# ymxlzgy/commonscenes

Hardware: AMD Instinct MI355X
Metric: DDIM denoise steps/sec (32 objects, 16^3 latent) (higher is better)
Workload: dtype f32 (operands as fp16 hi+lo pairs, fp32 accumulate)

## Files before the change

commonscenes_amd/build.py:

```python
from __future__ import annotations

import os
import shutil
import subprocess
import sys
from pathlib import Path

PKG_DIR = Path(__file__).resolve().parent
CSRC = PKG_DIR / "csrc"
LIB_NAME = "libcommonscenes_hip.so"
LIB_PATH = PKG_DIR / LIB_NAME
SOURCES = ["cs_plan.hip", "cs_gemm.hip", "cs_gemm_f16x3.hip", "cs_gemm_kw.hip", "cs_mesh.hip", "cs_scene.hip", "cs_constraints.hip", "cs_metrics.hip", "cs_pairwise.hip", "cs_norm.hip", "cs_attention.hip", "cs_attention_f16x3.hip", "cs_ops.hip", "cs_unet.hip", "cs_vqvae.hip", "cs_vqenc.hip"]
HEADERS = [CSRC / "cs_common.h", CSRC / "cs_f16x3.h", CSRC / "cs_mc_tables.h", CSRC / "cs_driver.h", CSRC / "cs_vq.h", PKG_DIR.parent / "include" / "commonscenes_hip.h"]
ARCH = "gfx950"
FLAGS = ["-O3", "-std=c++17", "-fPIC", "-ffp-contract=off", f"--offload-arch={ARCH}", "-Wall",
         "-Wno-unused-function"]


def _hipcc() -> str:
    for cand in (os.environ.get("HIPCC"), shutil.which("hipcc"), "/opt/rocm/bin/hipcc"):
        if cand and Path(cand).exists():
            return cand
    raise RuntimeError("hipcc not found: cannot build libcommonscenes_hip.so")


def _flagstr() -> str:
    return " ".join([*FLAGS, *os.environ.get("CS_EXTRA_HIPCC_FLAGS", "").split()])


def _deps(src: Path, seen=None) -> set:
    import re
    seen = set() if seen is None else seen
    src = src.resolve()
    if src in seen or not src.exists():
        return seen
    seen.add(src)
    for m in re.finditer(r'^\s*#\s*include\s+"([^"]+)"', src.read_text(), re.M):
        _deps(src.parent / m.group(1), seen)
    return seen


def needs_build() -> bool:
    if not LIB_PATH.exists():
        return True
    stamp = PKG_DIR / "build" / "flags.txt"
    if stamp.exists() and stamp.read_text() != _flagstr():
        return True
    t = LIB_PATH.stat().st_mtime
    deps = [CSRC / s for s in SOURCES] + HEADERS
    return any(d.stat().st_mtime > t for d in deps)


def build_native(force: bool = False, verbose: bool = True) -> Path:
    if not force and not needs_build():
        return LIB_PATH
    hipcc = _hipcc()
    extra = os.environ.get("CS_EXTRA_HIPCC_FLAGS", "").split()
    objdir = PKG_DIR / "build"
    objdir.mkdir(exist_ok=True)
    import time
    t0 = time.time()
    procs = []
    objs = []
    stamp = objdir / "flags.txt"
    flagstr = _flagstr()
    same_flags = stamp.exists() and stamp.read_text() == flagstr
    for s in SOURCES:
        obj = objdir / (s.replace(".hip", ".o"))
        objs.append(str(obj))
        newest_dep = max(d.stat().st_mtime for d in _deps(CSRC / s))
        if not force and same_flags and obj.exists() and obj.stat().st_mtime > newest_dep:
            continue
        cmd = [hipcc, *FLAGS, *extra, "-c", str(CSRC / s), "-o", str(obj)]
        if verbose:
            print("[build]", " ".join(cmd), flush=True)
        procs.append((s, subprocess.Popen(cmd, stdout=subprocess.PIPE, stderr=subprocess.STDOUT)))
    for s, p in procs:
        out, _ = p.communicate()
        if p.returncode != 0:
            sys.stderr.write(out.decode())
            raise RuntimeError(f"hipcc failed on {s}")
        if verbose and out.strip():
            print(out.decode())
        os.utime(objdir / (s.replace(".hip", ".o")), (t0, t0))
    stamp.write_text(flagstr)
    tmp = LIB_PATH.with_suffix(".so.tmp")
    cmd = [hipcc, "-shared", "-fPIC", f"--offload-arch={ARCH}", *objs, "-o", str(tmp)]
    if verbose:
        print("[build]", " ".join(cmd), flush=True)
    subprocess.check_call(cmd)
    os.replace(tmp, LIB_PATH)
    os.utime(LIB_PATH, (t0, t0))
    return LIB_PATH


if __name__ == "__main__":
    print(build_native(force="--force" in sys.argv))
```

commonscenes_amd/csrc/cs_gemm.hip:

```cpp
#include <cstdlib>
#include <atomic>
#include <cstring>
#include "cs_f16x3.h"

namespace {

constexpr int BK = 16;

template <int WMB, int WNB, int WAVES_M, int WAVES_N>
__global__ __launch_bounds__(256) void conv_gemm_f32_kernel(const CsConvGemm p, int M,
                                                            int tiles_n, int taps_hw, int kw_) {
  constexpr int BM = 32 * WMB * WAVES_M;
  constexpr int BN = 32 * WNB * WAVES_N;
  constexpr int LDAS = BM + 4;
  constexpr int LDBS = BN + 4;
  constexpr int RPT = (BM + 63) / 64;
  constexpr int BUNITS = BK * BN / 4;
  constexpr int BPT = (BUNITS + 255) / 256;
  constexpr int A_SZ = BK * LDAS;
  constexpr int B_SZ = BK * LDBS;
  __shared__ __attribute__((aligned(16))) float smem[2 * A_SZ + 2 * B_SZ];
  float* As = smem;
  float* Bs = smem + 2 * A_SZ;

// ... 467 lines not shown
    }
    if (opair) {
      h4 hi, lo;
#pragma unroll
      for (int k = 0; k < 4; ++k) {
        const float o = v[k] * p.out_scale;
        oamax = fmaxf(oamax, fabsf(o));
        hi[k] = (_Float16)o;
        lo[k] = (_Float16)(o - (float)hi[k]);
      }
      const u32x2 H = __builtin_bit_cast(u32x2, hi), Lw = __builtin_bit_cast(u32x2, lo);
      const bool odd = cl & 1;
      const u32x2 send = odd ? H : Lw;
      u32x2 recv;
      recv[0] = (unsigned)__builtin_amdgcn_update_dpp(0, (int)send[0], 0xB1, 0xF, 0xF, true);
      recv[1] = (unsigned)__builtin_amdgcn_update_dpp(0, (int)send[1], 0xB1, 0xF, 0xF, true);
      u32x4 r;
      r[0] = odd ? recv[0] : H[0];
      r[1] = odd ? recv[1] : H[1];
      r[2] = odd ? Lw[0] : recv[0];
      r[3] = odd ? Lw[1] : recv[1];
      if (tok) {
        char* row = reinterpret_cast<char*>(p.out + m * p.ldo);
        *reinterpret_cast<u32x4*>(row + (n >> 4) * 64 + ((n & 8) ? 32 : 0) + ((n & 4) ? 16 : 0)) = r;
      }
    } else if (tok) {
      *reinterpret_cast<f32x4*>(p.out + m * p.ldo + n) = v;
    }
  }
  if (opair && p.status && oamax >= 65504.f) atomicOr(p.status, CS_STATUS_F16X3_OVERFLOW);
  if (gstat) {
    double tot[2][4];
#pragma unroll
    for (int which = 0; which < 2; ++which) {
      __syncthreads();
#pragma unroll
      for (int k = 0; k < 4; ++k) sc[tl][cl * 4 + k] = which ? sq[k] : s[k];
      __syncthreads();
      if (tl == 0) {
#pragma unroll
        for (int k = 0; k < 4; ++k) {
          double a = 0.0;
          for (int r2 = 0; r2 < 16; ++r2) a += sc[r2][cl * 4 + k];
          tot[which][k] = a;
        }
      }
    }
    if (tl == 0 && nok) {
      double* o = p.gn_part + ((int64_t)rb * p.gn_ld + n) * 2;
#pragma unroll
      for (int k = 0; k < 4; ++k) {
        o[2 * k] = tot[0][k];
        o[2 * k + 1] = tot[1][k];
      }
    }
  }
}

void tile_dims(int tile, int& bm, int& bn) {
  switch (tile) {
    case 1: bm = 128; bn = 128; break;
    case 2: bm = 128; bn = 224; break;
    case 3: bm = 64; bn = 64; break;
    case 4: bm = 256; bn = 224; break;
    case 6: bm = 256; bn = 128; break;
    case 7: bm = 256; bn = 64; break;
    case 10: bm = 64; bn = 64; break;
    default: bm = 0; bn = 0; break;
  }
}

}

static int auto_tile(const CsConvGemm& p, int M, bool f16x3);
static bool up2_direct_batched(const CsConvGemm& d, int64_t m1, int ncls);
static int up2_batched_tile(const CsConvGemm& d, int64_t m1, int ncls);

extern "C" int cs_conv_gemm_epilogue_caps(const CsConvGemm* d, int32_t* gn_rows, int32_t* pair_ok) {
  if (!d) return CS_EINVAL;
  if (gn_rows) *gn_rows = 0;
  if (pair_ok) *pair_ok = 0;
  const CsConvGemm& p = *d;
  if (p.math != CS_MATH_F16X3 || p.nb <= 0 || p.cout <= 0 || p.dout <= 0 || p.hout <= 0 || p.wout <= 0) return CS_OK;
  const int64_t M64 = (int64_t)p.nb * p.dout * p.hout * p.wout;
  if (M64 > 0x7fffffffLL) return CS_OK;
  const int M = (int)M64;
  auto al16 = [](const void* q) { return ((uintptr_t)q & 15) == 0; };
  const int ocols = p.act == CS_ACT_GEGLU ? p.cout / 2 : p.cout;
  const bool vec = (p.cout % 4 == 0) && (p.ldo % 4 == 0) && al16(p.out) && (!p.bias || al16(p.bias)) &&
                   (!p.scale || (al16(p.scale) && al16(p.shift))) && (!p.rowvec || (p.ldrv % 4 == 0 && al16(p.rowvec))) &&
                   (!p.res || (p.ldr % 4 == 0 && al16(p.res)));
  if (!vec) return CS_OK;
  const bool pair_geom = (ocols % 8 == 0) && (p.ldo % 16 == 0) && (((uintptr_t)p.out & 63) == 0);
  int64_t rps = (int64_t)p.dout * p.hout * p.wout;
  int bm = 0, bn = 0;
  if (p.ud | p.uh | p.uw) {
    const int64_t m1 = (int64_t)p.nb * p.din * p.hin * p.win;
    const int ncls = (p.ud ? 2 : 1) * (p.uh ? 2 : 1) * (p.uw ? 2 : 1);
    if (p.splitk > 1 || !up2_direct_batched(p, m1, ncls)) return CS_OK;
    CsConvGemm q = p;
    q.kd = p.ud ? 2 : 3; q.kh = p.uh ? 2 : 3; q.kw = p.uw ? 2 : 3;
    q.ud = q.uh = q.uw = 0;
    q.dout = p.din; q.hout = p.hin; q.wout = p.win;
    q.tile = 0;
    tile_dims(up2_batched_tile(p, m1, ncls), bm, bn);
    rps = (int64_t)p.din * p.hin * p.win;
    if (!bm || !p.bias) return CS_OK;
    if (p.scale) return CS_OK;
    const int64_t ospan = ((int64_t)bm + 2LL * p.hin * p.win + 2LL * p.win + 2) * ncls;
    if (ospan * p.ldo * 4 >= 0x7FF00000LL) return CS_OK;
    if (gn_rows && rps % bm == 0 && p.act != CS_ACT_GEGLU) *gn_rows = bm;
    return CS_OK;
  }
  if (p.a_format == 3 || p.a_format == 4) {
    const int wr = p.a_format == 4 ? 64 : 32;
    if (gn_rows && rps % wr == 0 && p.act != CS_ACT_GEGLU) *gn_rows = wr;
    if (pair_ok && pair_geom && p.act != CS_ACT_GEGLU) *pair_ok = 1;
    return CS_OK;
  }
  if (p.splitk > 1) {
    if (gn_rows && rps % SKR == 0 && p.act != CS_ACT_GEGLU) *gn_rows = SKR;
    if (pair_ok && pair_geom && p.act != CS_ACT_GEGLU) *pair_ok = 1;
    return CS_OK;
  }
  int tile = p.tile ? p.tile : auto_tile(p, M, true);
  if (tile == 5) return CS_OK;
  tile_dims(tile, bm, bn);
  if (!bm) return CS_OK;
  if (tile == 10) {
    if (!cs_kw_gemm_applicable(p, M)) return CS_OK;
    if (gn_rows && rps % bm == 0) *gn_rows = bm;
    if (pair_ok && pair_geom) *pair_ok = 1;
    return CS_OK;
  }
  const bool piped = (p.res || p.bias || p.rowvec) && !p.scale && (p.act != CS_ACT_GEGLU || p.cout % bn == 0) &&
                     (!p.rowvec || p.rv_rows % bm == 0) &&
                     (int64_t)bm * p.ldo * 4 < 0x7FF00000LL && (!p.res || (int64_t)bm * p.ldr * 4 < 0x7FF00000LL);
  if (!piped) return CS_OK;
  if (gn_rows && rps % bm == 0 && p.act != CS_ACT_GEGLU) *gn_rows = bm;
  if (pair_ok && pair_geom) *pair_ok = 1;
  return CS_OK;
}

extern "C" int cs_conv_gemm_plan(const CsConvGemm* d, int32_t* splitk, int64_t* ws_bytes) {
  if (!d || !splitk) return CS_EINVAL;
  const int64_t M = (int64_t)d->nb * d->dout * d->hout * d->wout;
  if (M <= 0 || d->cout <= 0) return CS_EINVAL;
  const int s = plan_splitk(*d, M);
  *splitk = s;
  if (ws_bytes) *ws_bytes = s > 1 ? (int64_t)s * M * d->cout * 4 : 0;
  return CS_OK;
}

static int64_t kwave_max_tiles() {
  static const int64_t v = [] {
    const char* e = getenv("CS_KWAVE_MAX_TILES");
    return (e && *e) ? atoll(e) : (long long)-1;
  }();
  return v >= 0 ? v : 4LL * device_cus();
}

static int tok_t2_maxk() {
  static const int v = [] {
    const char* e = getenv("CS_TOK_T2_MAXK");
    return (e && *e) ? atoi(e) : 128;
  }();
  return v;
}

static int auto_tile(const CsConvGemm& p, int M, bool f16x3) {
  int tile = 0;
  {
    const int64_t mt = (M + 127) / 128;
    if (f16x3 && p.cout % 224 == 0 && ((M + 255) / 256) * (int64_t)(p.cout / 224) >= 192)
      tile = 4;
    else if (f16x3 && p.cout % 128 == 0 && ((M + 255) / 256) * (int64_t)(p.cout / 128) >= 192)
      tile = 6;
    else if (f16x3 && p.cout <= 64 && (p.cout == 64 || p.cout <= 4) && (M + 255) / 256 >= 192)
      tile = 7;
    else if (p.cout % 224 == 0 && mt * (p.cout / 224) >= 256)
      tile = 2;
    else if (p.cout > 64 && mt * ((p.cout + 127) / 128) >= 256)
      tile = 1;
    else
      tile = 3;
    {
      const bool t512on = cs_debug()->tile512 != 0;
      const bool conv3 = p.kd == 3 && p.kh == 3 && p.kw == 3 && p.sd == 1 && p.sh == 1 && p.sw == 1 &&
                         !(p.ud | p.uh | p.uw) && p.pd == 1 && p.ph == 1 && p.pw == 1;
      const int64_t t512 = (M + 511) / 512;
      if (t512on && conv3 && tile == 7 && p.cout == 64 && p.win <= 64 && t512 >= 512) tile = 8;
      if (t512on && conv3 && tile == 6 && p.win <= 32 && t512 * (p.cout / 128) >= 512) tile = 9;
    }
    if (f16x3 && tile == 4 && p.kd * p.kh * p.kw == 1 && p.act != CS_ACT_GEGLU && !cs_debug()->no_tok_rules) {
      const int64_t t4 = ((M + 255) / 256) * (int64_t)(p.cout / 224);
      const int64_t rounds = (t4 + 255) / 256;
      if (t4 > 256 && rounds * 256 * 4 >= t4 * 5)
        tile = 1;
      else if (p.a_format == 2 && (p.cin + 15) / 16 <= 32)
        tile = 2;
      else if (t4 <= 256 && (p.cin + 15) / 16 <= 84)
        tile = 2;
      else if ((p.cin + 15) / 16 <= tok_t2_maxk())
        tile = 2;
    }
    if (p.act == CS_ACT_GEGLU) tile = 2;
    if (f16x3 && tile == 3 && !cs_debug()->no_kwave && (p.cin + 15) / 16 >= 8 && p.cout % 224 == 0 &&
        cs_kw_gemm_applicable(p, M) && (int64_t)((M + 63) / 64) * ((p.cout + 63) / 64) <= kwave_max_tiles())
      tile = 10;
  }
  return tile;
}

static int sliced_tile(const CsConvGemm& p, int M) {
  if (p.tile == 6 || p.tile == 7) return p.tile;
  const bool slab3 = !cs_debug()->slice_tile2 && p.kd == 3 && p.kh == 3 && p.kw == 3 && p.sd == 1 && p.sh == 1 &&
                     p.sw == 1 && p.pd == 1 && p.ph == 1 && p.pw == 1 && !(p.ud | p.uh | p.uw) && p.din == p.dout &&
                     p.hin == p.hout && p.win == p.wout && p.win <= 32;
  return (split4_large(p, M) || p.tile == 4 || slab3) ? 4 : 2;
}

static int device_cus() {
  static std::atomic<int> cached{-1};
  int v = cached.load(std::memory_order_relaxed);
  if (v >= 0) return v;
  int dev = 0, n = 0;
  if (hipGetDevice(&dev) != hipSuccess || hipDeviceGetAttribute(&n, hipDeviceAttributeMultiprocessorCount, dev) != hipSuccess)
    n = 0;
  (void)hipGetLastError();
  cached.store(n, std::memory_order_relaxed);
  return n;
}

static int fused_reduce_plan(const CsConvGemm& p, int M, int stile) {
  if (!p.splitk_sync || cs_debug()->no_fused_reduce || p.splitk < 2 || (stile != 2 && stile != 4)) return 0;
  if (p.cout % 224 || ((uintptr_t)p.splitk_sync & 3)) return 0;
  const int bm = stile == 4 ? 256 : 128;
  const int64_t tiles = (int64_t)((M + bm - 1) / bm) * (p.cout / 224);
  const int64_t slots = (int64_t)device_cus() * (stile == 4 ? 1 : 2);
  if (tiles * p.splitk > slots || 2 * tiles > p.splitk_sync_words) return 0;
  if ((int64_t)p.splitk * M * p.cout * 4 >= 0xFFE00000LL) return 0;
  int r = 1;
  while (2 * r <= p.splitk && 2 * r <= bm / 16) r *= 2;
  return r;
}

static int wino_tile(int cout) { return cout % 224 == 0 ? 4 : cout % 128 == 0 ? 6 : cout == 64 ? 7 : 0; }

static int wino_variant(const CsConvGemm& p);
static bool wino_ok(const CsConvGemm& p) { return wino_variant(p) != 0; }
static bool wino23_ok(const CsConvGemm& p) {
  const CsDebug* dbg = cs_debug();
  if (dbg->no_wino || p.math != CS_MATH_F16X3 || p.act == CS_ACT_GEGLU) return false;
  if (!(p.kd == 3 && p.kh == 3 && p.kw == 3 && p.sd == 1 && p.sh == 1 && p.sw == 1 && p.pd == 1 && p.ph == 1 && p.pw == 1) ||
      (p.ud | p.uh | p.uw) || p.din != p.dout || p.hin != p.hout || p.win != p.wout)
    return false;
  if ((p.win & 1) || p.win < 4 || p.win / 2 > 32 || !wino_tile(p.cout) || (p.cin & 7) || p.cin < 16) return false;
  if (p.cout % 224 && (int64_t)p.din * p.hin * p.win > 4096) return false;
  const int64_t M = (int64_t)p.nb * p.dout * p.hout * p.wout;
  const int64_t min_rows = dbg->wino_min_rows > 0 ? dbg->wino_min_rows : 1024;
  if (M < min_rows || M > 0x3fffffffLL || (M / 2) % 256) return false;
  if ((512 + 2LL * p.hin * (p.win / 2) + p.win + 32) * p.lda * 4 >= 0x7FF00000LL) return false;
  return true;
}
static int wino_variant(const CsConvGemm& p) {
  if (!wino23_ok(p)) return 0;
  const CsDebug* dbg = cs_debug();
  const int64_t M = (int64_t)p.nb * p.dout * p.hout * p.wout;
  const int64_t min43 = dbg->wino43_min_rows > 0 ? dbg->wino43_min_rows : 2048;
  const int64_t rdec = p.cout % 224 ? (int64_t)p.din * p.hin * p.win : M;
  if (!dbg->no_wino43 && p.win % 4 == 0 && (M / 4) % 256 == 0 && (rdec / 4) % 256 == 0 && rdec >= min43) return 4;
  return 2;
}
static inline int wino_pos(int variant) { return variant + 2; }

struct WinoPlan {
  int slices;
  int units_main;
};
static int wino_splits(const CsConvGemm& p, int variant, double* cost_us = nullptr);

static WinoPlan wino_plan(const CsConvGemm& p, int variant) {
  WinoPlan pl;
  double t_uni = 0;
  pl.slices = wino_splits(p, variant, &t_uni);
  pl.units_main = 0;
  static const bool forced = [] { const char* e = getenv("CS_WINO_SPLITS"); return e && *e && atoi(e) > 0; }();
  if (forced || cs_debug()->no_wino_tail || p.cout % 224) return pl;
  const int64_t M = (int64_t)p.nb * p.dout * p.hout * p.wout;
  const int64_t R = M / variant / 256, tiles_n = p.cout / 224;
  const int64_t units = wino_pos(variant) * tiles_n;
  const int64_t cus = device_cus() > 0 ? device_cus() : 256;
  if (R < 1) return pl;
  const int64_t rounds = units * R / cus;
  if (rounds < 1) return pl;
  const int64_t units_main = rounds * cus / R;
  const int64_t tail_tiles = (units - units_main) * R;
  if (units_main < 1 || tail_tiles < 1) return pl;
  const int64_t nsc = 3LL * ((p.cin + 15) / 16);
  int best = 0;
  for (int sp = 2; sp <= 16 && tail_tiles * sp <= cus; ++sp) {
    const int64_t per = (nsc + sp - 1) / sp;
    if (per < 2 || per * sp * 10 > nsc * 11 || (nsc + per - 1) / per != sp) continue;
    best = sp;
  }
  if (!best) return pl;
  const int64_t per = (nsc + best - 1) / best;
  const double mb_tail = (double)tail_tiles * 256.0 * 224.0 * 4.0 / 1e6;
  double seam = (best - 1) * mb_tail * 0.46;
  if (seam < 2.0 * (best - 1)) seam = 2.0 * (best - 1);
  const double main_rounds = (double)((units_main * R + cus - 1) / cus);
  const double t_tail = main_rounds * ((double)nsc * 3.0 * 0.95 + 10.0) + ((double)per * 3.0 * 0.95 + 10.0) + seam + 5.0;
  if (t_tail < t_uni * 0.97) {
    pl.slices = best;
    pl.units_main = (int)units_main;
  }
  return pl;
}

static int wino_splits(const CsConvGemm& p, int variant, double* cost_us) {
  if (cost_us) *cost_us = 0.0;
  if (p.cout % 224) return 1;
  static const int forced = [] {
    const char* e = getenv("CS_WINO_SPLITS");
    return (e && *e) ? atoi(e) : 0;
  }();
  const int64_t M = (int64_t)p.nb * p.dout * p.hout * p.wout;
  const int64_t tiles = wino_pos(variant) * (M / variant / 256) * (p.cout / 224);
  if (forced > 0) {
    const int64_t nsc0 = 3LL * ((p.cin + 15) / 16), per0 = (nsc0 + forced - 1) / forced;
    if (forced == 1 || (per0 >= 2 && per0 * forced * 10 <= nsc0 * 11 && (nsc0 + per0 - 1) / per0 == forced)) return forced;
  }
  const int64_t cus = device_cus() > 0 ? device_cus() : 256;
  const int64_t nsc = 3LL * ((p.cin + 15) / 16);
  const double mb = (double)wino_pos(variant) / variant * (double)M * p.cout * 4.0 / 1e6;
  int best = 1;
  double best_t = 0;
  for (int sp = 1; sp <= 16; ++sp) {
    const int64_t per = (nsc + sp - 1) / sp;
    if (sp > 1 && (per < 2 || per * sp * 10 > nsc * 11 || (nsc + per - 1) / per != sp)) continue;
    const int64_t rounds = (tiles * sp + cus - 1) / cus;
    double seam = (sp - 1) * mb * 0.46;
    if (sp > 1 && seam < 2.0 * (sp - 1)) seam = 2.0 * (sp - 1);
    const double t = (double)rounds * ((double)per * 3.0 * 0.95 + 10.0) + seam;
    if (sp == 1 || t < best_t * 0.97) {
      best = sp;
      best_t = t;
    }
  }
  if (cost_us) *cost_us = best_t;
  return best;
}

extern "C" int cs_conv_wino_ok(const CsConvGemm* d) { return (d && d->nb > 0 && d->cout > 0) ? wino_variant(*d) : 0; }

static int wino_asked(const CsConvGemm& p) {
  const int v = p.a_format == 4 ? 4 : 2;
  const int best = wino_variant(p);
  return (best == 0 || v > best) ? 0 : v;
}

extern "C" int cs_conv_wino_plan(const CsConvGemm* d, int32_t* splitk, int64_t* ws_bytes) {
  if (!d || !splitk) return CS_EINVAL;
  const int v = wino_asked(*d);
  if (!v) return CS_EINVAL;
  const int sp = wino_plan(*d, v).slices;
  *splitk = sp;
  const int64_t M = (int64_t)d->nb * d->dout * d->hout * d->wout;
  if (ws_bytes) *ws_bytes = (int64_t)sp * wino_pos(v) * (M / v) * d->cout * 4;
  return CS_OK;
}

extern "C" int cs_conv_wino_plan_info(const CsConvGemm* d, int32_t* slices, int32_t* units_main, int32_t* units) {
  if (!d) return CS_EINVAL;
  const int v = wino_asked(*d);
  if (!v) return CS_EINVAL;
  const WinoPlan pl = wino_plan(*d, v);
  if (slices) *slices = pl.slices;
  if (units_main) *units_main = pl.units_main;
  if (units) *units = (int32_t)(wino_pos(v) * ((d->cout + 223) / 224));
  return CS_OK;
}

static int conv_wino(const CsConvGemm& p, int M, hipStream_t s, int phases = 3) {
  auto al16 = [](const void* q) { return ((uintptr_t)q & 15) == 0; };
  const int v = wino_asked(p), np = wino_pos(v);
  if (!v || !p.x_lo || !al16(p.x_lo) || !p.w_lo || !al16(p.w_lo) || (p.lda & 7) || !p.splitk_ws || !al16(p.splitk_ws) ||
      p.a_bound || !(p.acc_scale > 0.f))
    return CS_EINVAL;
  if ((p.ldo & 3) || !al16(p.out) || (p.bias && !al16(p.bias)) || (p.scale && (!al16(p.scale) || !al16(p.shift))) ||
      (p.rowvec && ((p.ldrv & 3) || !al16(p.rowvec))) || (p.res && ((p.ldr & 3) || !al16(p.res))))
    return CS_EINVAL;
  const int sp = p.splitk > 1 ? p.splitk : 1;
  if (sp > 16) return CS_EINVAL;
  CsConvGemm q = p;
  q.nb = np * p.nb;
  q.win = q.wout = p.win / v;
  q.kw = 1;
  q.pw = 0;
  q.a_format = 1;
  q.out = reinterpret_cast<float*>(p.splitk_ws);
  q.ldo = p.cout;
  q.bias = q.scale = q.shift = q.rowvec = q.res = nullptr;
  q.act = CS_ACT_NONE;
  q.gn_part = nullptr;
  q.out_format = 0;
  q.splitk = 0;
  q.tile = wino_tile(p.cout);
  const WinoPlan pl = wino_plan(p, v);
  const bool tail = pl.units_main > 0 && pl.slices == sp;
  const int units = np * (p.cout / 224);
  if (phases & 1) {
    int rc;
    if (tail) {
      rc = cs_conv_gemm_f16x3_dispatch(q, np * (M / v), q.tile, 1, s, 16, np, nullptr, nullptr, nullptr, 0, nullptr, 0, pl.units_main);
      if (rc == CS_OK)
        rc = cs_conv_gemm_f16x3_dispatch(q, np * (M / v), q.tile, sp, s, 16, np, nullptr, nullptr, nullptr, 0, nullptr, pl.units_main,
                                         units - pl.units_main);
    } else {
      rc = cs_conv_gemm_f16x3_dispatch(q, np * (M / v), q.tile, sp, s, 16, np, nullptr, nullptr, nullptr, 0, nullptr);
    }
    if (rc != CS_OK) return rc;
  }
  if (!(phases & 2)) return CS_OK;
  const int tail_unit0 = tail ? pl.units_main : 0x7fffffff;
  const int sp_main = tail ? 1 : sp;
  const int64_t nblk = (int64_t)((M / v + 15) / 16) * ((p.cout + 63) / 64);
  if (nblk > 0x7fffffffLL || (p.gn_part && p.gn_rows != 16 * v)) return CS_EINVAL;
  if (v == 4) {
    CS_LAUNCH(wino_out_kernel<4>, dim3((unsigned)nblk), dim3(256), 0, s, p, reinterpret_cast<const float*>(p.splitk_ws), M, sp_main,
              tail_unit0, sp, 224);
  } else {
    CS_LAUNCH(wino_out_kernel<2>, dim3((unsigned)nblk), dim3(256), 0, s, p, reinterpret_cast<const float*>(p.splitk_ws), M, sp_main,
              tail_unit0, sp, 224);
  }
// ... 537 lines not shown
```

commonscenes_amd/csrc/cs_norm.hip:

```cpp
#include <cstdlib>

#include "cs_common.h"

namespace {

constexpr int GN_MIN_SPLIT_ROWS = 16;
constexpr int GN_MAX_SPLITS = 256;
constexpr int64_t GN_SMALL_BYTES = 16 << 20;
constexpr int64_t GN_SMALL_GROUP = 11264;

__global__ __launch_bounds__(256) void gn_partial_kernel(const float* __restrict__ x, int rows, int c,
                                                         int ldx, int groups, int nsplit, int rps,
                                                         double* __restrict__ partial) {
  extern __shared__ __attribute__((aligned(16))) double sm[];
  const int n = blockIdx.x / nsplit;
  const int split = blockIdx.x % nsplit;
  const int ch4 = c >> 2;
  const int tpr = ch4 < 256 ? ch4 : 256;
  const int rowlanes = 256 / tpr;
  const int tid = threadIdx.x;
  const int rl = tid / tpr;
  const int cl = tid - rl * tpr;
  const int r0 = split * rps;
  const int r1 = min(rows, r0 + rps);
  const float* xb = x + (int64_t)n * rows * ldx;
  if (rl < rowlanes) {
    for (int c4 = cl; c4 < ch4; c4 += tpr) {
      double s0 = 0, s1 = 0, s2 = 0, s3 = 0, q0 = 0, q1 = 0, q2 = 0, q3 = 0;
      for (int r = r0 + rl; r < r1; r += 4 * rowlanes) {
        float4 v[4];
#pragma unroll
        for (int u = 0; u < 4; ++u) {
          const int rr = r + u * rowlanes;
          v[u] = rr < r1 ? *reinterpret_cast<const float4*>(xb + (int64_t)rr * ldx + c4 * 4)
                         : make_float4(0.f, 0.f, 0.f, 0.f);
        }
#pragma unroll
        for (int u = 0; u < 4; ++u) {
          if (r + u * rowlanes < r1) {
            s0 += v[u].x; q0 += (double)v[u].x * v[u].x;
            s1 += v[u].y; q1 += (double)v[u].y * v[u].y;
            s2 += v[u].z; q2 += (double)v[u].z * v[u].z;
            s3 += v[u].w; q3 += (double)v[u].w * v[u].w;
          }
        }
      }
      double* d = sm + ((int64_t)rl * c + c4 * 4) * 2;
      d[0] = s0; d[1] = q0; d[2] = s1; d[3] = q1; d[4] = s2; d[5] = q2; d[6] = s3; d[7] = q3;
    }
  }
  __syncthreads();
  if (tid < groups) {
    const int cpg = c / groups;
    double s = 0, q = 0;
    for (int l = 0; l < rowlanes; ++l)
      for (int k = 0; k < cpg; ++k) {
        const double* d = sm + ((int64_t)l * c + tid * cpg + k) * 2;
        s += d[0];
        q += d[1];
      }
    double* o = partial + (((int64_t)n * nsplit + split) * groups + tid) * 2;
    o[0] = s;
    o[1] = q;
  }
}

__device__ __forceinline__ void gn_bound_max(float* bound, double mean, double var, double count);

__global__ __launch_bounds__(256) void gn_finalize_kernel(const double* __restrict__ partial, int nsplit, int groups,
                                                          double count, float eps, float* __restrict__ stats,
                                                          int total, float* __restrict__ bound = nullptr) {
  const int lane = threadIdx.x & 63;
  const int i = blockIdx.x * 4 + (threadIdx.x >> 6);
  if (i >= total) return;
  const int n = i / groups, g = i - n * groups;
  double s = 0, q = 0;
  for (int k = lane; k < nsplit; k += 64) {
    const double* d = partial + (((int64_t)n * nsplit + k) * groups + g) * 2;
    s += d[0];
    q += d[1];
  }
#pragma unroll
  for (int o = 32; o > 0; o >>= 1) {
    s += __shfl_xor(s, o, 64);
    q += __shfl_xor(q, o, 64);
  }
  if (lane == 0) {
    const double mean = s / count;
    double var = q / count - mean * mean;
    if (var < 0) var = 0;
    stats[2 * i] = (float)mean;
    stats[2 * i + 1] = (float)(1.0 / sqrt(var + (double)eps));
    if (bound) gn_bound_max(bound, mean, var, count);
  }
}

struct GnSegs {
  CsGnSeg s[4];
  int n;
};
__device__ __forceinline__ void gn_group_parts(const GnSegs& sg, int n, int g, int cpg, int lane, int nlanes, double& s,
                                               double& q) {
  s = 0;
  q = 0;
  const int c_lo = g * cpg, c_hi = c_lo + cpg;
#pragma unroll
  for (int si = 0; si < 4; ++si) {
    if (si >= sg.n) break;
    const CsGnSeg& sp = sg.s[si];
    const int lo = max(c_lo, sp.ch0), hi = min(c_hi, sp.ch0 + sp.nch);
    if (hi <= lo) continue;
    const int tps = sp.tiles_per_sample, nt = sp.ncls * tps, items = (hi - lo) * nt;
    const int64_t cls_stride = (int64_t)sp.nb_src * tps;
    const int64_t t0 = (int64_t)(n % sp.nb_src) * tps;
    for (int j = lane; j < items; j += 4 * nlanes) {
      double2 v[4];
#pragma unroll
      for (int u = 0; u < 4; ++u) {
        const int ju = j + u * nlanes;
        v[u] = make_double2(0.0, 0.0);
        if (ju < items) {
          const int k = ju / nt, r = ju - k * nt;
          const int cls = r / tps, t = r - cls * tps;
          v[u] = *reinterpret_cast<const double2*>(sp.part +
                                                   ((cls * cls_stride + t0 + t) * sp.ld + sp.col0 + (lo + k - sp.ch0)) * 2);
        }
      }
#pragma unroll
      for (int u = 0; u < 4; ++u)
        if (j + u * nlanes < items) {
          s += v[u].x;
          q += v[u].y;
        }
    }
  }
}

__device__ __forceinline__ float gn_bound_value(double mean, double var, double count) {
  const double b = fabs(mean) + sqrt(var * (count > 1.0 ? count - 1.0 : 1.0));
  float bf = (float)b;
  if ((double)bf < b) bf = __uint_as_float(__float_as_uint(bf) + 1u);
  return (bf == bf && bf > 0.f) ? bf : 0.f;
}
__device__ __forceinline__ void gn_bound_commit(float* bound, float bf) {
  if (bf > 0.f) atomicMax(reinterpret_cast<unsigned int*>(bound), __float_as_uint(bf));
}
__device__ __forceinline__ void gn_bound_max(float* bound, double mean, double var, double count) {
  gn_bound_commit(bound, gn_bound_value(mean, var, count));
}

constexpr int GN_FIN_WAVES = 16;
template <int WPG>
__global__ __launch_bounds__(64 * GN_FIN_WAVES) void gn_finalize_parts_kernel(const GnSegs sg, int groups, int cpg,
                                                                              double count, float eps,
                                                                              float* __restrict__ stats,
// ... 261 lines not shown
  const int tid = threadIdx.x;
  const int ll = tid / tpr;
  const int cl = tid - ll * tpr;
  if (ll >= linelanes) return;
  const int n = blockIdx.y;
  const int l0 = blockIdx.x * lines_per_block;
  const int l1 = min(lines, l0 + lines_per_block);
  const int w4n = w >> 2;
  const float* xb = x + (int64_t)n * lines * w * ldx;
  const int64_t vrow0 = (int64_t)n * lines * w4n;
  const float* st = stats + (int64_t)n * groups * 2;
  float amax = 0.f;
  for (int cv = cl; cv < chv; cv += tpr) {
    float gg[V], bb[V], mean[V], rstd[V];
#pragma unroll
    for (int k4 = 0; k4 < V / 4; ++k4) {
      const float4 g = *reinterpret_cast<const float4*>(gamma + cv * V + 4 * k4);
      const float4 b = *reinterpret_cast<const float4*>(beta + cv * V + 4 * k4);
      gg[4 * k4] = g.x; gg[4 * k4 + 1] = g.y; gg[4 * k4 + 2] = g.z; gg[4 * k4 + 3] = g.w;
      bb[4 * k4] = b.x; bb[4 * k4 + 1] = b.y; bb[4 * k4 + 2] = b.z; bb[4 * k4 + 3] = b.w;
    }
#pragma unroll
    for (int k = 0; k < V; ++k) {
      const int grp = (ch0 + cv * V + k) / cpg;
      mean[k] = st[grp * 2];
      rstd[k] = st[grp * 2 + 1];
    }
    auto actv = [&](const float* px, bool in, float (&o)[V]) {
      if (!in) {
#pragma unroll
        for (int k = 0; k < V; ++k) o[k] = 0.f;
        return;
      }
#pragma unroll
      for (int k4 = 0; k4 < V / 4; ++k4) {
        const float4 v = *reinterpret_cast<const float4*>(px + 4 * k4);
        const float iv[4] = {v.x, v.y, v.z, v.w};
#pragma unroll
        for (int k = 0; k < 4; ++k)
          o[4 * k4 + k] = cs_act((iv[k] - mean[4 * k4 + k]) * rstd[4 * k4 + k] * gg[4 * k4 + k] + bb[4 * k4 + k], act) * a_scale;
      }
    };
    for (int line = l0 + ll; line < l1; line += linelanes) {
      const float* xl = xb + (int64_t)line * w * ldx + cv * V;
      float d[6][V];
#pragma unroll
      for (int k = 0; k < V; ++k) d[0][k] = 0.f;
      actv(xl, true, d[1]);
      for (int t = 0; t < w4n; ++t) {
#pragma unroll
        for (int j = 2; j < 6; ++j) {
          const int wi = 4 * t - 1 + j;
          actv(xl + (int64_t)wi * ldx, wi < w, d[j]);
        }
        const int64_t off = (vrow0 + (int64_t)line * w4n + t) * ldv + cv * V;
#pragma unroll
        for (int q = 0; q < 6; ++q) {
          hv hi, lo;
#pragma unroll
          for (int k = 0; k < V; ++k) {
            float o;
            if (q == 0) o = 4.f * d[0][k] - 5.f * d[2][k] + d[4][k];
            else if (q == 1) o = (d[4][k] + d[3][k]) - 4.f * (d[1][k] + d[2][k]);
            else if (q == 2) o = 4.f * (d[1][k] - d[2][k]) + (d[4][k] - d[3][k]);
            else if (q == 3) o = 2.f * (d[3][k] - d[1][k]) + (d[4][k] - d[2][k]);
            else if (q == 4) o = 2.f * (d[1][k] - d[3][k]) + (d[4][k] - d[2][k]);
            else o = 4.f * d[1][k] - 5.f * d[3][k] + d[5][k];
            amax = fmaxf(amax, fabsf(o));
            const _Float16 hh = (_Float16)o;
            hi[k] = hh;
            lo[k] = (_Float16)(o - (float)hh);
          }
          *reinterpret_cast<hv*>(vh + q * pos_stride + off) = hi;
          *reinterpret_cast<hv*>(vl + q * pos_stride + off) = lo;
        }
#pragma unroll
        for (int k = 0; k < V; ++k) {
          d[0][k] = d[4][k];
          d[1][k] = d[5][k];
        }
      }
    }
  }
  if (status && amax >= 65504.f) atomicOr(status, CS_STATUS_F16X3_OVERFLOW);
}

template <int MAXV>
__global__ __launch_bounds__(256) void ln_kernel(const float* __restrict__ x,
                                                 const float* __restrict__ gamma,
                                                 const float* __restrict__ beta,
                                                 float* __restrict__ y, int m, int c, int ldx,
                                                 int ldy, float eps) {
  const int lane = threadIdx.x & 63;
  const int wave = threadIdx.x >> 6;
  const int ch4 = c >> 2;
  for (int64_t row = (int64_t)blockIdx.x * 4 + wave; row < m; row += (int64_t)gridDim.x * 4) {
    float4 v[MAXV];
    float s = 0.f;
#pragma unroll
    for (int k = 0; k < MAXV; ++k) {
      const int c4 = lane + 64 * k;
      v[k] = make_float4(0.f, 0.f, 0.f, 0.f);
      if (c4 < ch4) v[k] = *reinterpret_cast<const float4*>(x + row * ldx + c4 * 4);
      s += (v[k].x + v[k].y) + (v[k].z + v[k].w);
    }
    const float mean = wave_sum(s) / (float)c;
    float q = 0.f;
#pragma unroll
    for (int k = 0; k < MAXV; ++k) {
      const int c4 = lane + 64 * k;
      if (c4 < ch4) {
        const float a = v[k].x - mean, b = v[k].y - mean, cc = v[k].z - mean, d = v[k].w - mean;
        q += (a * a + b * b) + (cc * cc + d * d);
      }
    }
    const float var = wave_sum(q) / (float)c;
    const float rstd = 1.0f / sqrtf(var + eps);
#pragma unroll
    for (int k = 0; k < MAXV; ++k) {
      const int c4 = lane + 64 * k;
      if (c4 < ch4) {
        const float4 g = *reinterpret_cast<const float4*>(gamma + c4 * 4);
        const float4 b = *reinterpret_cast<const float4*>(beta + c4 * 4);
        float4 o;
        o.x = (v[k].x - mean) * rstd * g.x + b.x;
        o.y = (v[k].y - mean) * rstd * g.y + b.y;
        o.z = (v[k].z - mean) * rstd * g.z + b.z;
        o.w = (v[k].w - mean) * rstd * g.w + b.w;
        *reinterpret_cast<float4*>(y + row * ldy + c4 * 4) = o;
      }
    }
  }
}

template <int MAXV>
__global__ __launch_bounds__(256) void ln_pair_kernel(const float* __restrict__ x, const float* __restrict__ gamma,
                                                      const float* __restrict__ beta, _Float16* __restrict__ y, int m,
                                                      int c, int ldx, int ldy, float eps, float a_scale,
                                                      int32_t* __restrict__ status) {
  const int lane = threadIdx.x & 63;
  const int wave = threadIdx.x >> 6;
  const int ch4 = c >> 2;
  float amax = 0.f;
  for (int64_t row = (int64_t)blockIdx.x * 4 + wave; row < m; row += (int64_t)gridDim.x * 4) {
    float4 v[MAXV];
    float s = 0.f;
#pragma unroll
    for (int k = 0; k < MAXV; ++k) {
      const int c4 = lane + 64 * k;
      v[k] = make_float4(0.f, 0.f, 0.f, 0.f);
      if (c4 < ch4) v[k] = *reinterpret_cast<const float4*>(x + row * ldx + c4 * 4);
      s += (v[k].x + v[k].y) + (v[k].z + v[k].w);
    }
    const float mean = wave_sum(s) / (float)c;
    float q = 0.f;
#pragma unroll
    for (int k = 0; k < MAXV; ++k) {
      const int c4 = lane + 64 * k;
      if (c4 < ch4) {
        const float a = v[k].x - mean, b = v[k].y - mean, cc = v[k].z - mean, d = v[k].w - mean;
        q += (a * a + b * b) + (cc * cc + d * d);
      }
    }
    const float var = wave_sum(q) / (float)c;
    const float rstd = 1.0f / sqrtf(var + eps);
#pragma unroll
    for (int k = 0; k < MAXV; ++k) {
      const int c4 = lane + 64 * k;
      if (c4 < ch4) {
        const float4 g = *reinterpret_cast<const float4*>(gamma + c4 * 4);
        const float4 b = *reinterpret_cast<const float4*>(beta + c4 * 4);
        const float o[4] = {((v[k].x - mean) * rstd * g.x + b.x) * a_scale, ((v[k].y - mean) * rstd * g.y + b.y) * a_scale,
                            ((v[k].z - mean) * rstd * g.z + b.z) * a_scale, ((v[k].w - mean) * rstd * g.w + b.w) * a_scale};
        h4v hi, lo;
#pragma unroll
        for (int e = 0; e < 4; ++e) {
          amax = fmaxf(amax, fabsf(o[e]));
          const _Float16 h = (_Float16)o[e];
          hi[e] = h;
          lo[e] = (_Float16)(o[e] - (float)h);
        }
        const int cch = c4 >> 2, j = (c4 & 3) * 4;
        _Float16* dst = y + row * (int64_t)ldy * 2 + cch * 32 + (j < 8 ? 0 : 16) + (j & 7);
        *reinterpret_cast<h4v*>(dst) = hi;
        *reinterpret_cast<h4v*>(dst + 8) = lo;
      }
    }
  }
  if (status && amax >= 65504.f) atomicOr(status, CS_STATUS_F16X3_OVERFLOW);
}

__global__ __launch_bounds__(256) void gn_small_kernel(const float* __restrict__ x, const float* __restrict__ gamma,
                                                       const float* __restrict__ beta, float* __restrict__ y,
                                                       float* __restrict__ stats, int rows, int c, int ldx, int ldy,
                                                       int groups, float eps, int act) {
  __shared__ double red[2][256];
  const int n = blockIdx.x / groups, g = blockIdx.x - n * groups;
  const int cpg = c / groups;
  const int tid = threadIdx.x;
  const float* xb = x + (int64_t)n * rows * ldx + g * cpg;
  float* yb = y + (int64_t)n * rows * ldy + g * cpg;
  const int dr = 256 / cpg, dk = 256 - dr * cpg;
  auto next = [&](int& r, int& k) {
    r += dr;
    k += dk;
    if (k >= cpg) {
      k -= cpg;
      ++r;
    }
  };
  double s = 0, q = 0;
  {
    int r = tid / cpg, k = tid - r * cpg;
    while (r < rows) {
      float v[4];
      int rr[4];
#pragma unroll
      for (int u = 0; u < 4; ++u) {
        rr[u] = r;
        v[u] = r < rows ? xb[(int64_t)r * ldx + k] : 0.f;
        next(r, k);
      }
#pragma unroll
      for (int u = 0; u < 4; ++u)
        if (rr[u] < rows) {
          s += v[u];
          q += (double)v[u] * v[u];
        }
    }
  }
  red[0][tid] = s;
  red[1][tid] = q;
  __syncthreads();
#pragma unroll
  for (int o = 128; o > 0; o >>= 1) {
    if (tid < o) {
      red[0][tid] += red[0][tid + o];
      red[1][tid] += red[1][tid + o];
    }
    __syncthreads();
  }
  const double count = (double)rows * cpg;
  const double mean_d = red[0][0] / count;
  double var = red[1][0] / count - mean_d * mean_d;
  if (var < 0) var = 0;
  const float mean = (float)mean_d;
  const float rstd = (float)(1.0 / sqrt(var + (double)eps));
  if (tid == 0 && stats) {
    stats[2 * blockIdx.x] = mean;
    stats[2 * blockIdx.x + 1] = rstd;
  }
  {
    int r = tid / cpg, k = tid - r * cpg;
    while (r < rows) {
      float v[4], ga[4], be[4];
      int rr[4], kk[4];
#pragma unroll
      for (int u = 0; u < 4; ++u) {
        rr[u] = r;
        kk[u] = k;
        if (r < rows) {
          v[u] = xb[(int64_t)r * ldx + k];
          ga[u] = gamma[g * cpg + k];
          be[u] = beta[g * cpg + k];
        }
        next(r, k);
      }
#pragma unroll
      for (int u = 0; u < 4; ++u)
        if (rr[u] < rows) yb[(int64_t)rr[u] * ldy + kk[u]] = cs_act((v[u] - mean) * rstd * ga[u] + be[u], act);
    }
  }
}

__global__ __launch_bounds__(256) void gn_small_parts_kernel(const float* __restrict__ x, const GnSegs sg,
                                                             const float* __restrict__ gamma,
                                                             const float* __restrict__ beta, float* __restrict__ y,
                                                             float* __restrict__ stats, float* __restrict__ bound, int rows,
                                                             int c, int ldx, int ldy, int groups, float eps, int act,
                                                             int rsplit) {
  __shared__ double red[2][256];
  const int sgi = blockIdx.x / rsplit, rs = blockIdx.x - sgi * rsplit;
  const int n = sgi / groups, g = sgi - n * groups;
  const int cpg = c / groups;
  const int tid = threadIdx.x;
  double s, q;
  gn_group_parts(sg, n, g, cpg, tid, 256, s, q);
  red[0][tid] = s;
  red[1][tid] = q;
  __syncthreads();
#pragma unroll
  for (int o = 128; o > 0; o >>= 1) {
    if (tid < o) {
      red[0][tid] += red[0][tid + o];
      red[1][tid] += red[1][tid + o];
    }
    __syncthreads();
  }
  const double count = (double)rows * cpg;
  const double mean_d = red[0][0] / count;
  double var = red[1][0] / count - mean_d * mean_d;
  if (var < 0) var = 0;
  const float mean = (float)mean_d;
  const float rstd = (float)(1.0 / sqrt(var + (double)eps));
  if (tid == 0 && stats && rs == 0) {
    stats[2 * sgi] = mean;
    stats[2 * sgi + 1] = rstd;
  }
  if (tid == 0 && bound && rs == 0) gn_bound_max(bound, mean_d, var, count);
  const int rper = (rows + rsplit - 1) / rsplit;
  const int rbeg = rs * rper, rend = min(rows, rbeg + rper);
  const float* xb = x + (int64_t)n * rows * ldx + g * cpg;
  float* yb = y + (int64_t)n * rows * ldy + g * cpg;
  const int dr = 256 / cpg, dk = 256 - dr * cpg;
  int r = rbeg + tid / cpg, k = tid - (tid / cpg) * cpg;
  rows = rend;
  while (r < rows) {
    float v[4], ga[4], be[4];
    int rr[4], kk[4];
#pragma unroll
    for (int u = 0; u < 4; ++u) {
      rr[u] = r;
      kk[u] = k;
      if (r < rows) {
        v[u] = xb[(int64_t)r * ldx + k];
        ga[u] = gamma[g * cpg + k];
        be[u] = beta[g * cpg + k];
      }
      r += dr;
      k += dk;
      if (k >= cpg) {
        k -= cpg;
        ++r;
      }
    }
#pragma unroll
    for (int u = 0; u < 4; ++u)
      if (rr[u] < rows) yb[(int64_t)rr[u] * ldy + kk[u]] = cs_act((v[u] - mean) * rstd * ga[u] + be[u], act);
  }
}
// ... 319 lines not shown
```

commonscenes_amd/csrc/cs_plan.hip:

```cpp
#include <cmath>
#include <cstdlib>
#include <cstring>
#include <mutex>

#include "cs_common.h"

namespace {

CsDebug g_dbg;
std::once_flag g_once;

bool flag(const char* name) {
  const char* e = getenv(name);
  return e && *e && !(e[0] == '0' && e[1] == 0);
}
long long num(const char* name, long long dflt) {
  const char* e = getenv(name);
  return (e && *e) ? atoll(e) : dflt;
}

void parse_env(CsDebug& d) {
  memset(&d, 0, sizeof(d));
  d.no_split16 = flag("CS_NO_SPLIT16");
  d.split16_min_rows = num("CS_SPLIT16_MIN_ROWS", 8192);
  d.no_pair16 = flag("CS_NO_PAIR16");
  d.no_upfold = flag("CS_NO_UPFOLD");
  d.no_splitk = flag("CS_NO_SPLITK");
  d.no_fused_geglu = flag("CS_NO_FUSED_GEGLU");
  d.no_tapcol = flag("CS_NO_TAPCOL");
  d.tapcol_tile = (int32_t)num("CS_TAPCOL_TILE", 0);
  d.no_cfg_split = flag("CS_NO_CFG_SPLIT");
  d.cfg_split_min_rows = num("CS_CFG_SPLIT_MIN_ROWS", 65536);
  d.concat_copy = flag("CS_CONCAT_COPY");
  d.gn_small_group = num("CS_GN_SMALL_GROUP", 11264);
  d.tile512 = flag("CS_TILE512");
  d.no_pw = flag("CS_NO_PW");
  d.no_slab4 = flag("CS_NO_SLAB4");
  d.no_attn_img = flag("CS_NO_ATTN_IMG");
  d.attn_nw8 = flag("CS_ATTN_NW8");
  d.no_up2_direct = flag("CS_NO_UP2_DIRECT");
  d.no_up2_batch = flag("CS_NO_UP2_BATCH");
  d.plan_pow2 = flag("CS_PLAN_POW2");
  d.slice_tile2 = flag("CS_SLICE_TILE2");
  d.no_gn_parts = flag("CS_NO_GN_PARTS");
  d.no_pair_epilogue = flag("CS_NO_PAIR_EPILOGUE");
  d.no_dyn_scale = flag("CS_NO_DYN_SCALE");
  d.no_tok_rules = flag("CS_NO_TOK_RULES");
  d.no_fused_reduce = flag("CS_NO_FUSED_REDUCE");
  d.no_gn_fold = flag("CS_NO_GN_FOLD");
  d.no_kwave = flag("CS_NO_KWAVE");
  d.no_static_scales = flag("CS_NO_STATIC_SCALES");
  d.no_wino = flag("CS_NO_WINO");
  d.wino_min_rows = (int32_t)num("CS_WINO_MIN_ROWS", 1024);
  d.no_wino43 = flag("CS_NO_WINO43");
  d.wino43_min_rows = (int32_t)num("CS_WINO43_MIN_ROWS", 2048);
  d.no_wino_tail = flag("CS_NO_WINO_TAIL");
}

}

extern "C" const CsDebug* cs_debug(void) {
  std::call_once(g_once, [] { parse_env(g_dbg); });
  return &g_dbg;
}

extern "C" void cs_debug_set(const CsDebug* d) {
  (void)cs_debug();
  if (d)
    g_dbg = *d;
  else
    parse_env(g_dbg);
}

extern "C" float cs_norm_a_scale(float gmax, float bmax, int64_t n) {
  const double bound = (double)gmax * std::sqrt((double)(n > 1 ? n - 1 : 1)) + (double)bmax;
  if (!(bound > 0.0) || !std::isfinite(bound)) return (float)std::ldexp(1.0, 40);
  int ex = 0;
  (void)std::frexp(65000.0 / bound, &ex);
  int k = ex - 1;
  if (k < -8) k = -8;
  if (k > 40) k = 40;
  return (float)std::ldexp(1.0, k);
}

extern "C" float cs_bound_a_scale(float bound) {
  if (!(bound > 0.f) || !std::isfinite(bound)) return (float)std::ldexp(1.0, 40);
  int ex = 0;
  (void)std::frexp(65000.0 / (double)bound, &ex);
  int k = ex - 1;
  if (k < -24) k = -24;
  if (k > 40) k = 40;
  return (float)std::ldexp(1.0, k);
}

extern "C" int cs_attnblock_static_scales(float gmax, float bmax, int64_t n, int c, float w_l2max, float b_absmax, float qk_scale,
                                          float* out4) {
  if (!out4 || n < 1 || c < 1 || !(qk_scale > 0.f) || !(gmax >= 0.f) || !(bmax >= 0.f) || !(w_l2max >= 0.f) || !(b_absmax >= 0.f))
    return CS_EINVAL;
  const double e = (double)gmax * std::sqrt((double)(n > 1 ? n - 1 : 1)) + (double)bmax;
  const double b = (double)w_l2max * std::sqrt((double)c) * e + (double)b_absmax;
  auto S = [](double v) { return cs_bound_a_scale(v < 3.0e38 ? (float)(v * (1.0 + 1e-6)) : 3.0e38f); };
  out4[0] = S(b * (double)qk_scale);
  out4[1] = S(b);
  out4[2] = S(b);
  out4[3] = S(b);
  return CS_OK;
}

extern "C" int cs_transformer_static_scales(const CsTransformerStats* st, int c, int64_t n_tokens, int heads, float gn_gmax,
                                            float gn_bmax, float ctx_max, float* out12) {
  if (!st || !out12 || c <= 0 || heads <= 0 || c % heads || n_tokens <= 0) return CS_EINVAL;
  const double rc = std::sqrt((double)c);
  const double dh = (double)(c / heads);
  const double y1 = (double)st->g1 * rc + (double)st->be1;
  const double bq = (double)st->rq * y1, bk = (double)st->rk * y1, bv = (double)st->rv * y1;
  const double ngrp = (double)n_tokens * (double)(c / 32 > 0 ? c / 32 : 1);
  const double egn = (double)gn_gmax * std::sqrt(ngrp > 1.0 ? ngrp - 1.0 : 1.0) + (double)gn_bmax;
  const double bt0 = (double)st->rpi * rc * egn + (double)st->bpi;
  const double bt1 = (double)st->ro * rc * bv + (double)st->bo + bt0 + (double)(ctx_max > 0.f ? ctx_max : 0.f);
  const double y3 = (double)st->g3 * rc + (double)st->be3;
  const double bgg = ((double)st->rx * y3 + (double)st->bx) * ((double)st->rg * y3 + (double)st->bg);
  const double bt2 = (double)st->r2 * std::sqrt(4.0 * c) * bgg + (double)st->b2 + bt1;
  auto S = [](double b) { return cs_bound_a_scale(b < 3.0e38 ? (float)(b * (1.0 + 1e-6)) : 3.0e38f); };
  out12[0] = S(bq / std::sqrt(dh));
  out12[1] = S(bk);
  out12[2] = S(bv);
  out12[3] = S(bv);
  out12[4] = S(bgg);
  out12[5] = S(bt2);
  out12[6] = (float)bq; out12[7] = (float)bk; out12[8] = (float)bv; out12[9] = (float)bt1; out12[10] = (float)bgg;
  out12[11] = (float)bt2;
  return CS_OK;
}

extern "C" int cs_conv_wants_split16(int64_t m, int cin, int cout, int k, int plain, int math) {
  const CsDebug* d = cs_debug();
  if (d->no_split16 || math != CS_MATH_F16X3 || !plain || k != 3 || (cin & 7)) return 0;
  const int64_t t256 = (m + 255) / 256;
  if (cout % 224 == 0) return t256 * (cout / 224) >= 192 || (d->split16_min_rows > 0 && m >= d->split16_min_rows);
  if (cout % 128 == 0) return t256 * (cout / 128) >= 192;
  return (cout == 64 || cout <= 4) && t256 >= 192;
}

extern "C" int cs_tapcol_tile(int64_t m, int ncolp) {
  const CsDebug* d = cs_debug();
  if (d->tapcol_tile) return d->tapcol_tile;
  if ((m + 255) / 256 < 192) return 0;
  return ncolp <= 64 ? 7 : 6;
}

extern "C" int cs_tapcol_ok(int cout, int cin, int k, int math) {
  return !cs_debug()->no_tapcol && math == CS_MATH_F16X3 && k == 3 && cout <= 4 && (cin & 3) == 0;
}
```

commonscenes_amd/csrc/cs_unet.hip:

```cpp
#include "cs_driver.h"

namespace {

enum Kind { CONV_IN, RES, ATTN, ATTNBLOCK, DOWN, UP };

struct Layer {
  Kind kind;
  int cin, cout;
  int g[8];
  int n[4];
  int emb_lo = 0;
  int ks = 0, ch_h = 0;
  int gsp[2] = {-1, -1};
  int ctx_off = 0;
  bool fused_geglu = false;
  int stat_slot = -1;
  CsTransformerStats ts;
  bool has_ts = false;
  float ctx_max = 0.f;
  int ab_w = -1, ab_b = -1;
  float ab_l2max = 0.f, ab_bmax = 0.f;
};

}
// ... 178 lines not shown
      ds *= 2;
    }
  }
  u.mid.push_back(make_res(u, P + "middle_block.0", ch, ch, ted, emb));
  u.mid.push_back(attn_layer(P + "middle_block.1", ch));
  u.mid.push_back(make_res(u, P + "middle_block.2", ch, ch, ted, emb));
  int oi = 0;
  for (int level = c.n_mult - 1; level >= 0; --level) {
    const int m = c.channel_mult[level];
    for (int i = 0; i <= nres; ++i) {
      const int ich = chans.back();
      chans.pop_back();
      const std::string bp = P + "output_blocks." + std::to_string(oi++);
      std::vector<Layer> layers;
      layers.push_back(make_res(u, bp + ".0", ch + ich, mc * m, ted, emb));
      ch = mc * m;
      if (in_list(c.attention_resolutions, c.n_attn_res, ds))
        layers.push_back(attn_layer(bp + ".1", ch));
      if (level && i == nres) {
        Layer l{};
        l.kind = UP;
        l.cin = l.cout = ch;
        l.g[0] = add_layer_gemm(u, bp + "." + std::to_string(layers.size()) + ".conv", ch, ch, 3, true, 0,
                                c.dims == 3 ? 3 : 7);
        layers.push_back(l);
        ds /= 2;
      }
      u.out.push_back(layers);
    }
  }
  if (c.use_spatial_transformer && !cs_debug()->no_cfg_split) {
    size_t n_prefix = 0;
    while (n_prefix < u.inp.size() && !has_attn(u.inp[n_prefix])) ++n_prefix;
    for (size_t j = 0; j < u.out.size(); ++j) {
      const size_t src = u.inp.size() - 1 - j;
      Layer& l = u.out[j][0];
      if (src >= n_prefix || l.kind != RES || l.g[2] < 0) continue;
      const int ch_s = u.inp[src].back().cout, C = l.cin, ch_h = C - ch_s, cpg = C / 32;
      if (C % 32) continue;
      int ks = 0;
      for (int k = (ch_h + 15) / 16 * 16; k < C; k += 16)
        if ((k / cpg) * cpg >= ch_h) {
          ks = k;
          break;
        }
      if (!ks || (C - ks) % 16) continue;
      const int gi = l.g[0];
      const int wp = u.gemms[gi].w[0].param, bp = u.gemms[gi].b.empty() ? -1 : u.gemms[gi].b[0].param;
      const int k = u.gemms[gi].k;
      l.gsp[0] = add_gemm_cin_range(u, wp, bp, l.cout, C, k, 0, ks);
      l.gsp[1] = add_gemm_cin_range(u, wp, -1, l.cout, C, k, ks, C);
      l.ks = ks;
      l.ch_h = ch_h;
    }
  }
  u.split_min_rows = cs_debug()->cfg_split_min_rows;
  u.ch_final = ch;
  u.n_out = add_norm(u, P + "out.0", ch);
  u.g_out = add_layer_gemm(u, P + "out.2", c.out_channels, mc, 3, true, 0, 0, true);
  u.g_emb_all = add_gemm(u, emb.w, emb.b, emb.total, ted, 0);
  u.emb_total = emb.total;

  int nblk = 0, nab = 0;
  for_each_layer(u, [&](const Layer& l) {
    nblk += l.kind == ATTN;
    nab += l.kind == ATTNBLOCK;
  });
  u.extra_slots = (c.math == CS_MATH_F16X3) ? 34 * nblk + 4 * nab : 0;
  layout_arena(u);
  if (u.extra_slots) {
    int k = 0, k2 = 0;
    for_each_layer(u, [&](Layer& l) {
      if (l.kind == ATTN) l.stat_slot = u.extra_slot0 + 34 * k++;
      if (l.kind == ATTNBLOCK) l.stat_slot = u.extra_slot0 + 34 * nblk + 4 * k2++;
    });
  }
  return CS_OK;
}

struct Exec : ExecBase {
  const cs_unet& u;
  Exec(const cs_unet& u_, const void* arena_, void* ws_, int64_t ws_bytes_, bool dry_, hipStream_t st_)
      : ExecBase(u_, arena_, ws_, ws_bytes_, dry_, st_), u(u_) {}
  int64_t in_bound_off = -1;

  Act res_block(const Layer& l, const Act& x, const Buf& semb) {
    const int rows = x.d * x.h * x.w;
    const bool own_skip = l.g[2] >= 0;
    int64_t xb = -1;
    Buf hn = groupnorm(x.b, l.n[0], x.nb, 1e-5f, CS_ACT_SILU, 32, l.g[0], own_skip ? &xb : nullptr, x.d, x.h, x.w);
    Buf h1 = gemm(hn, l.g[0], x.nb, x.d, x.h, x.w, GemmOpts().row_vector(at(semb, l.emb_lo), semb.c, rows).stats());
    release(hn);
    Buf hn2 = groupnorm(h1, l.n[1], x.nb, 1e-5f, CS_ACT_SILU, 32, l.g[1], nullptr, x.d, x.h, x.w);
    release(h1);
    Buf skip;
    if (own_skip) skip = gemm(x.b, l.g[2], x.nb, x.d, x.h, x.w, GemmOpts().bound(xb));
    Act o = x;
    const Buf& sk = own_skip ? skip : x.b;
    o.b = gemm(hn2, l.g[1], x.nb, x.d, x.h, x.w, GemmOpts().residual(sk, sk.c).stats());
    release(hn2);
    release(skip);
    return o;
  }

  Act res_block_split(const Layer& l, const Act& x, const Act& sk, const Buf& semb) {
    const int rows = x.d * x.h * x.w, C = x.b.c, ks = l.ks, cs = C - ks, off = ks - l.ch_h, cpg = C / 32;
    const int nb = x.nb, nbs = sk.nb, ch_s = sk.b.c, cout = l.cout;
    Act o = x;
    if (nbs <= 0 || nb % nbs || ch_s != C - l.ch_h) {
      chk(CS_EINVAL);
      return o;
    }
    const Norm& n0 = pl.norms[l.n[0]];
    GnStats s = gn_stats_alloc(x.b, nb, 32, true);
    gn_stats_run(x.b, nb, 1e-5f, 32, s);
    release(s.wsb);
    auto gn_range = [&](const float* xp, int ldx, int nbr, int64_t sample0, int ch0, int c, int conv_gi, int wn) {
      Buf y = gn_out(n0, (int64_t)nbr * rows, c, nbr, cpg, wn, conv_gi, (int64_t)nbs * rows);
      gn_emit(xp, ldx, at(s.stats, sample0 * 32 * 2), n0, y, nbr, rows, x.d, x.h, x.w, 32, cpg, ch0, CS_ACT_SILU);
      return y;
    };
    const int wn_h = wants_wino(l.gsp[0], nbs, x.d, x.h, x.w), wn_s = wants_wino(l.gsp[1], nbs, x.d, x.h, x.w);
    Buf a_h;
    if (!wn_h) a_h = gn_range(at(x.b), C, nb, 0, 0, ks, l.gsp[0], 0);
    Buf a_s = gn_range(at(sk.b, off), ch_s, nbs, 0, ks, cs, l.gsp[1], wn_s);
    Buf y_s = alloc(sk.b.rows, cout);
    if (ok()) gemm_view(view(a_s), l.gsp[1], nbs, x.d, x.h, x.w, at(y_s), cout);
    release(a_s);
    Buf h1 = alloc(x.b.rows, cout);
    for (int g = 0; g < nb / nbs && ok(); ++g) {
      const int64_t s0 = (int64_t)g * nbs, r0 = s0 * rows;
      GemmOpts opt;
      opt.row_vector(at(semb, s0 * semb.c + l.emb_lo), semb.c, rows).residual(y_s, cout);
      if (wn_h) {
        Buf a_g = gn_range(at(x.b, r0 * C), C, nbs, s0, 0, ks, l.gsp[0], wn_h);
        if (ok()) gemm_view(view(a_g), l.gsp[0], nbs, x.d, x.h, x.w, at(h1, r0 * cout), cout, opt);
        release(a_g);
      } else {
        gemm_view(view(a_h, r0), l.gsp[0], nbs, x.d, x.h, x.w, at(h1, r0 * cout), cout, opt);
      }
    }
    release(s.stats);
    release(a_h);
    release(y_s);
    Buf skc = gemm(x.b, l.g[2], nb, x.d, x.h, x.w, GemmOpts().bound(s.bound));
    Buf hn2 = groupnorm(h1, l.n[1], nb, 1e-5f, CS_ACT_SILU, 32, l.g[1], nullptr, x.d, x.h, x.w);
    release(h1);
    o.b = gemm(hn2, l.g[1], nb, x.d, x.h, x.w, GemmOpts().residual(skc, cout).stats());
    release(hn2);
    release(skc);
    return o;
  }

  Act attn_block(const Layer& l, const Act& x, const float* ctxvec) {
    const int c = l.cin, heads = u.cfg.num_heads, dh = c / heads;
    const int n = x.d * x.h * x.w;
    const int64_t rows = (int64_t)x.nb * n;
    Buf xn = groupnorm(x.b, l.n[0], x.nb, 1e-6f, CS_ACT_NONE);
    Buf t0 = linear(xn, l.g[0]);
    release(xn);
    Buf n1 = layernorm(t0, l.n[1]);
    Buf qkv = linear(n1, l.g[1]);
    release(n1);
    Buf a = alloc(rows, c);
    float ss[12];
    const Norm& gnn = pl.norms[l.n[0]];
    const bool stat = l.has_ts && u.cfg.math == CS_MATH_F16X3 && !cs_debug()->no_static_scales && ctxvec &&
                      cs_transformer_static_scales(&l.ts, c, n, heads, gnn.gmax, gnn.bmax, l.ctx_max, ss) == CS_OK;
    self_attention(qkv, a, x.nb, n, heads, dh, c, (float)std::pow((double)dh, -0.5), stat ? ss : nullptr);
    if (stat) a.a_scale = ss[3];
    release(qkv);
    Buf t1 = linear(a, l.g[2], GemmOpts().row_vector(ctxvec ? ctxvec + l.ctx_off : nullptr, u.ctx_total, n).residual(t0, c));
    release(a);
    release(t0);
    Buf n3 = layernorm(t1, l.n[3]);
    Buf gg;
    const float pairs = u.cfg.math == CS_MATH_F16X3 ? 16.f : 0.f;
    const float pair_gg = (pairs > 0.f && stat) ? ss[4] : pairs, pair_t2 = (pairs > 0.f && stat) ? ss[5] : pairs;
    if (l.fused_geglu) {
      gg = linear(n3, l.g[5], GemmOpts().activation(CS_ACT_GEGLU).pair(pair_gg));
    } else {
      Buf ff = linear(n3, l.g[5]);
      gg = alloc(rows, 4 * c);
      if (ok() && !dry) chk(cs_geglu(p(ff), p(gg), (int)rows, 4 * c, 8 * c, 4 * c, st));
      release(ff);
    }
    if (stat && !gg.pair) gg.a_scale = ss[4];
    release(n3);
    Buf t2 = linear(gg, l.g[6], GemmOpts().residual(t1, c).pair(pair_t2));
    if (stat && !t2.pair) t2.a_scale = ss[5];
    release(gg);
    release(t1);
    Act o = x;
    o.b = gemm(t2, l.g[7], x.nb, n, 1, 1, GemmOpts().residual(x.b, c).stats());
    release(t2);
    return o;
  }

  Act attnblock(const Layer& l, const Act& x) {
    const int c = l.cin, heads = u.cfg.num_heads, dh = c / heads;
    const int n = x.d * x.h * x.w;
    const int64_t rows = (int64_t)x.nb * n;
    Buf xn = groupnorm(x.b, l.n[0], x.nb, 1e-5f, CS_ACT_NONE);
    Buf qkv = linear(xn, l.g[0]);
    release(xn);
    Buf a = alloc(rows, c);
    float ss[4];
    const float qks = (float)std::pow((double)dh, -0.5);
    const bool stat = attnblock_scales(l.n[0], (int64_t)n * (c / 32), c, l.ab_l2max, l.ab_bmax, qks, ss);
    self_attention(qkv, a, x.nb, n, heads, dh, c, qks, stat ? ss : nullptr);
    if (stat) a.a_scale = ss[3];
    release(qkv);
    Act o = x;
    o.b = gemm(a, l.g[1], x.nb, n, 1, 1, GemmOpts().residual(x.b, c).stats());
    release(a);
    return o;
  }

  Act run(const std::vector<Layer>& layers, Act h, const Buf& semb, const float* ctxvec, bool keep_in,
          const Act* split_skip = nullptr) {
    bool owned = !keep_in;
    for (const Layer& l : layers) {
      Act o;
      if (l.kind == RES && l.ks > 0 && split_skip && &l == &layers[0]) {
        o = res_block_split(l, h, *split_skip, semb);
        if (owned) release(h.b);
        h = o;
        owned = true;
        continue;
      }
      switch (l.kind) {
        case CONV_IN:
          o = h;
          o.b = gemm(h.b, l.g[0], h.nb, h.d, h.h, h.w, GemmOpts().stats().bound(in_bound_off));
          break;
        case RES:
          o = res_block(l, h, semb);
          break;
        case ATTN:
          o = attn_block(l, h, ctxvec);
          break;
        case ATTNBLOCK:
          o = attnblock(l, h);
          break;
        case DOWN: {
          const int sd = u.cfg.dims == 3 ? 1 : 2;
          o = h;
          o.b = gemm(h.b, l.g[0], h.nb, h.d, h.h, h.w, GemmOpts().stride(2, sd).stats().bound(range_bound(h.b, h.nb)));
          o.d = h.d / sd;
          o.h = h.h / 2;
          o.w = h.w / 2;
          break;
        }
        case UP: {
          const int ud = u.cfg.dims == 3 ? 0 : 1;
          o = h;
          o.b = gemm(h.b, l.g[0], h.nb, h.d, h.h, h.w, GemmOpts().upsample(1, ud).stats().bound(range_bound(h.b, h.nb)));
          o.d = h.d << ud;
          o.h = h.h * 2;
          o.w = h.w * 2;
          break;
        }
      }
      if (owned) release(h.b);
      h = o;
      owned = true;
    }
    return h;
  }

  Buf duplicate(const Buf& a) {
    Buf o = alloc(2 * a.rows, a.c);
    if (a.nseg == 1 && a.seg[0].valid()) {
      o.seg[0] = dup_stat(a.seg[0]);
      o.nseg = o.seg[0].valid() ? 1 : 0;
    }
    if (ok() && !dry) {
      const size_t bytes = (size_t)a.rows * a.c * 4;
      if (hipMemcpyAsync(p(o), p(a), bytes, hipMemcpyDeviceToDevice, st) != hipSuccess ||
          hipMemcpyAsync((char*)p(o) + bytes, p(a), bytes, hipMemcpyDeviceToDevice, st) != hipSuccess)
        chk(CS_EINVAL);
    }
    return o;
  }
};

int forward(Exec& e, const float* x_ncdhw, const int64_t* t, const float* ctxvec, float* eps_ncdhw, int nbx,
            int cfg_pairs) {
  const cs_unet& u = e.u;
  const CsUnetConfig& c = u.cfg;
  const int S = c.d * c.h * c.w;
  e.sync_begin();
  e.amax_begin(64);
  Buf temb = e.alloc(nbx, c.model_channels);
  if (e.ok() && !e.dry) e.chk(cs_timestep_embedding(t, e.p(temb), nbx, c.model_channels, 10000.0f, e.st));
  Buf e1 = e.linear(temb, u.g_te0, GemmOpts().activation(CS_ACT_SILU));
  e.release(temb);
  Buf e2 = e.linear(e1, u.g_te2, GemmOpts().activation(CS_ACT_SILU));
  e.release(e1);
  Buf semb = e.linear(e2, u.g_emb_all);
  e.release(e2);
  Act h;
  h.nb = nbx; h.d = c.d; h.h = c.h; h.w = c.w;
  h.b = e.alloc((int64_t)nbx * S, u.cpad_in);
  if (e.ok() && !e.dry) e.chk(cs_nchw_to_ndhwc(x_ncdhw, e.p(h.b), nbx, c.in_channels, S, u.cpad_in, e.st));
  e.in_bound_off = e.amax_slot();
  if (e.in_bound_off >= 0 && e.ok() && !e.dry)
    e.chk(cs_absmax(e.p(h.b), (int64_t)nbx * S * u.cpad_in, e.bound_ptr(e.in_bound_off), e.st));
  bool shared = cfg_pairs != 0;
  auto split = [&](bool h_retained) {
    Buf h2 = e.duplicate(h.b);
    if (!h_retained) e.release(h.b);
    h.b = h2;
    h.nb *= 2;
    Buf s2 = e.duplicate(semb);
    e.release(semb);
    semb = s2;
    shared = false;
  };
  std::vector<Act> hs;
  bool first = true;
  for (const auto& layers : u.inp) {
    bool keep = !first;
    if (shared && has_attn(layers)) {
      split(!first);
      keep = false;
    }
    h = e.run(layers, h, semb, ctxvec, keep);
    hs.push_back(h);
    first = false;
    if (!e.ok()) return e.rc;
  }
  bool keep_mid = true;
  if (shared) {
    split(true);
    keep_mid = false;
  }
  h = e.run(u.mid, h, semb, ctxvec, keep_mid);
  for (const auto& layers : u.out) {
    Act sk = hs.back();
    hs.pop_back();
    Act cat = h;
    cat.b = e.alloc(h.b.rows, h.b.c + sk.b.c);
    if (e.ok() && !e.dry) {
      e.chk(cs_copy_rows(e.p(h.b), e.p(cat.b), h.b.rows, h.b.c, h.b.c, cat.b.c, e.st));
      const int groups = h.nb / sk.nb;
      if (groups * sk.nb != h.nb) e.chk(CS_EINVAL);
      for (int g = 0; g < groups && e.ok(); ++g)
        e.chk(cs_copy_rows(e.p(sk.b), e.p(cat.b) + (int64_t)g * sk.b.rows * cat.b.c + h.b.c, sk.b.rows, sk.b.c,
                           sk.b.c, cat.b.c, e.st));
    }
    cat.b.nseg = 0;
    if (h.b.nseg == 1 && sk.b.nseg == 1 && h.b.seg[0].valid() && sk.b.seg[0].valid()) {
      cat.b.seg[0] = h.b.seg[0];
      cat.b.seg[1] = sk.b.seg[0];
      cat.b.nseg = 2;
      h.b.seg[0] = Stat();
      sk.b.seg[0] = Stat();
      h.b.nseg = sk.b.nseg = 0;
    }
    e.release(h.b);
    if (layers[0].kind == RES && layers[0].ks > 0 && cat.b.rows >= u.split_min_rows) {
      h = e.run(layers, cat, semb, ctxvec, false, &sk);
      e.release(sk.b);
    } else {
      e.release(sk.b);
      h = e.run(layers, cat, semb, ctxvec, false);
    }
    if (!e.ok()) return e.rc;
  }
  Buf hn = e.groupnorm(h.b, u.n_out, h.nb, 1e-5f, CS_ACT_SILU, 32, u.g_out);
  e.release(h.b);
  Buf eps = e.gemm(hn, u.g_out, h.nb, h.d, h.h, h.w);
  e.release(hn);
  if (e.ok() && !e.dry) e.chk(cs_ndhwc_to_nchw(e.p(eps), eps_ncdhw, h.nb, c.out_channels, S, eps.c, e.st));
  e.release(eps);
  e.release(semb);
  e.release(e.amax_arena);
  return e.rc;
}

}

extern "C" int cs_unet_create(const CsUnetConfig* cfg, cs_unet** out) {
  if (!cfg || !out) return CS_EINVAL;
  cs_unet* u = new (std::nothrow) cs_unet();
  if (!u) return CS_ENOMEM;
  u->cfg = *cfg;
  u->math = cfg->math;
  const int rc = build(*u);
  if (rc != CS_OK) {
    delete u;
    return rc;
  }
  *out = u;
  return CS_OK;
}

extern "C" void cs_unet_destroy(cs_unet* u) { delete u; }

extern "C" int cs_unet_param_count(const cs_unet* u) { return u ? (int)u->params.size() : 0; }

extern "C" int cs_unet_param_info(const cs_unet* u, int i, const char** name, int64_t shape5[5], int* ndim,
                                  int64_t* raw_offset_bytes) {
  return plan_param_info(u, i, name, shape5, ndim, raw_offset_bytes);
}

extern "C" int64_t cs_unet_raw_bytes(const cs_unet* u) { return u ? u->raw_bytes : 0; }
extern "C" int64_t cs_unet_arena_bytes(const cs_unet* u) { return u ? u->arena_bytes : 0; }
extern "C" int64_t cs_unet_context_floats(const cs_unet* u) { return u ? u->ctx_total : 0; }

extern "C" int cs_unet_pack(cs_unet* u, const void* raw_dev, void* arena_dev, cs_stream_t stream) {
  const int rc = pack_plan(u, raw_dev, arena_dev, stream);
  if (rc != CS_OK || !u || u->math != CS_MATH_F16X3) return rc;
  hipStream_t st = (hipStream_t)stream;
  const char* raw = reinterpret_cast<const char*>(raw_dev);
  float* d_amax = reinterpret_cast<float*>(reinterpret_cast<char*>(arena_dev) + u->amax_off);
  auto src = [&](int param) { return reinterpret_cast<const float*>(raw + u->params[param].raw_off); };
  struct Job {
    const float* w;
    int rows, cols;
  };
  for (Kind kind : {ATTNBLOCK, ATTN}) {
    std::vector<Layer*> blocks;
    for_each_layer(*u, [&](Layer& l) {
      if (l.kind == kind && l.stat_slot >= 0) blocks.push_back(&l);
    });
    if (blocks.empty()) continue;
    const int njobs = kind == ATTN ? 17 : 2;
    for (const Layer* lp : blocks) {
      const Layer& l = *lp;
      const int c = l.cin;
      std::vector<Job> jobs;
      if (kind == ATTNBLOCK) {
        jobs = {{src(l.ab_w), 3 * c, c}, {src(l.ab_b), 1, 3 * c}};
      } else {
        const Gemm& qkv = u->gemms[l.g[1]];
        const Gemm& to = u->gemms[l.g[2]];
        const Gemm& ff = u->gemms[l.g[5]];
        const Gemm& f2 = u->gemms[l.g[6]];
        const Gemm& pi = u->gemms[l.g[0]];
        const Norm& n1 = u->norms[l.n[1]];
        const Norm& n3 = u->norms[l.n[3]];
        if (qkv.w.size() != 3 || to.w.empty() || to.b.empty() || ff.w.empty() || ff.b.empty() || f2.w.empty() || f2.b.empty() ||
            pi.w.empty() || pi.b.empty())
          return CS_EINVAL;
        const float* wff = src(ff.w[0].param);
        const float* bff = src(ff.b[0].param);
        jobs = {
            {src(qkv.w[0].param), c, c}, {src(qkv.w[1].param), c, c}, {src(qkv.w[2].param), c, c},
            {src(to.w[0].param), c, c}, {src(to.b[0].param), 1, c},
            {wff, 4 * c, c}, {bff, 1, 4 * c}, {wff + (int64_t)4 * c * c, 4 * c, c}, {bff + 4 * c, 1, 4 * c},
            {src(f2.w[0].param), c, 4 * c}, {src(f2.b[0].param), 1, c},
            {src(pi.w[0].param), c, c}, {src(pi.b[0].param), 1, c},
            {src(n1.gp), 1, c}, {src(n1.bp), 1, c}, {src(n3.gp), 1, c}, {src(n3.bp), 1, c}};
      }
      if ((int)jobs.size() != njobs) return CS_EINVAL;
      for (int j = 0; j < njobs; ++j) {
        const int r2 = cs_weight_rowstats(jobs[j].w, jobs[j].rows, jobs[j].cols, d_amax + l.stat_slot + 2 * j, stream);
        if (r2 != CS_OK) return r2;
      }
    }
    std::vector<float> host((size_t)2 * njobs * blocks.size());
    if (hipMemcpyAsync(host.data(), d_amax + blocks[0]->stat_slot, host.size() * 4, hipMemcpyDeviceToHost, st) != hipSuccess ||
        hipStreamSynchronize(st) != hipSuccess)
      return CS_EINVAL;
    for (size_t b = 0; b < blocks.size(); ++b) {
      const float* h = host.data() + 2 * njobs * b;
      if (kind == ATTNBLOCK) {
        blocks[b]->ab_l2max = h[0];
        blocks[b]->ab_bmax = h[3];
        continue;
      }
      static const int which[17] = {0, 0, 0, 0, 1, 0, 1, 0, 1, 0, 1, 0, 1, 1, 0, 1, 0};
      float v[17];
      for (int j = 0; j < 17; ++j) v[j] = h[2 * j + which[j]];
      CsTransformerStats& t = blocks[b]->ts;
      t.rq = v[0]; t.rk = v[1]; t.rv = v[2]; t.ro = v[3]; t.bo = v[4]; t.rx = v[5]; t.bx = v[6]; t.rg = v[7]; t.bg = v[8];
      t.r2 = v[9]; t.b2 = v[10]; t.rpi = v[11]; t.bpi = v[12]; t.g1 = v[13]; t.be1 = v[14]; t.g3 = v[15]; t.be3 = v[16];
      blocks[b]->has_ts = true;
    }
// ... 81 lines not shown
```

commonscenes_amd/lib.py:

```python
from __future__ import annotations

import ctypes as C
import os
from pathlib import Path

import torch

from .build import LIB_PATH

ABI_VERSION = 18
CS_OK = 0
CS_EINVAL = -22
CS_ENOMEM = -12
ACT_NONE, ACT_RELU, ACT_SILU, ACT_GELU, ACT_GEGLU = 0, 1, 2, 3, 4
MATH_FP32, MATH_F16X3 = 0, 1
VQ_ST_ROWS = 256
MATH_F16 = 2
DEFAULT_MATH = MATH_FP32 if os.environ.get("CS_MATH", "f16x3").lower() == "fp32" else MATH_F16X3

_f = C.c_void_p
_i = C.c_int
_l = C.c_int64
_s = C.c_void_p
_fl = C.c_float


class CsConvGemm(C.Structure):
    _fields_ = [
        ("x", C.c_void_p), ("w", C.c_void_p), ("out", C.c_void_p), ("bias", C.c_void_p),
        ("scale", C.c_void_p), ("shift", C.c_void_p), ("rowvec", C.c_void_p), ("res", C.c_void_p),
        ("nb", C.c_int32), ("din", C.c_int32), ("hin", C.c_int32), ("win", C.c_int32),
        ("dout", C.c_int32), ("hout", C.c_int32), ("wout", C.c_int32),
        ("cin", C.c_int32), ("cout", C.c_int32),
        ("lda", C.c_int32), ("ldw", C.c_int32), ("ldo", C.c_int32), ("ldr", C.c_int32),
        ("ldrv", C.c_int32),
        ("kd", C.c_int32), ("kh", C.c_int32), ("kw", C.c_int32),
        ("sd", C.c_int32), ("sh", C.c_int32), ("sw", C.c_int32),
        ("pd", C.c_int32), ("ph", C.c_int32), ("pw", C.c_int32),
        ("ud", C.c_int32), ("uh", C.c_int32), ("uw", C.c_int32),
        ("act", C.c_int32), ("rv_rows", C.c_int32), ("math", C.c_int32), ("tile", C.c_int32),
        ("w_lo", C.c_void_p), ("acc_scale", C.c_float), ("a_scale", C.c_float),
        ("x_lo", C.c_void_p), ("a_format", C.c_int32), ("splitk", C.c_int32),
        ("splitk_ws", C.c_void_p), ("status", C.c_void_p),
        ("gn_part", C.c_void_p), ("gn_ld", C.c_int32), ("gn_rows", C.c_int32), ("out_format", C.c_int32),
        ("out_scale", C.c_float), ("a_bound", C.c_void_p),
        ("splitk_sync", C.c_void_p), ("splitk_sync_words", C.c_int32),
    ]


class CsTransformerStats(C.Structure):
    _fields_ = [(n, C.c_float) for n in ("rq", "rk", "rv", "ro", "bo", "rx", "bx", "rg", "bg", "r2", "b2", "rpi", "bpi", "g1",
                                        "be1", "g3", "be3")]


class CsGnSeg(C.Structure):
    _fields_ = [("part", C.c_void_p), ("ld", C.c_int32), ("col0", C.c_int32), ("ch0", C.c_int32), ("nch", C.c_int32),
                ("tiles_per_sample", C.c_int32), ("ncls", C.c_int32), ("nb_src", C.c_int32), ("reserved", C.c_int32)]


class CsDebug(C.Structure):
    _fields_ = [(n, C.c_int32) for n in (
        "no_split16", "no_pair16", "no_upfold", "no_splitk", "no_fused_geglu", "no_tapcol", "tapcol_tile", "no_cfg_split",
        "concat_copy", "tile512", "no_pw", "no_slab4", "no_attn_img", "attn_nw8", "no_up2_direct", "no_up2_batch",
        "plan_pow2", "slice_tile2", "no_gn_parts", "no_pair_epilogue", "no_dyn_scale", "no_tok_rules", "no_fused_reduce",
        "no_gn_fold", "no_kwave", "no_static_scales", "no_wino", "wino_min_rows", "no_wino43", "wino43_min_rows",
        "no_wino_tail")] + [
        ("split16_min_rows", C.c_int64), ("cfg_split_min_rows", C.c_int64), ("gn_small_group", C.c_int64)]


class CsUnetConfig(C.Structure):
    _fields_ = [
        ("in_channels", C.c_int32), ("out_channels", C.c_int32), ("model_channels", C.c_int32),
        ("num_res_blocks", C.c_int32), ("n_mult", C.c_int32), ("channel_mult", C.c_int32 * 8),
        ("n_attn_res", C.c_int32), ("attention_resolutions", C.c_int32 * 8),
        ("num_heads", C.c_int32), ("context_dim", C.c_int32),
        ("d", C.c_int32), ("h", C.c_int32), ("w", C.c_int32), ("math", C.c_int32),
        ("use_spatial_transformer", C.c_int32), ("dims", C.c_int32),
    ]


class CsVqvaeConfig(C.Structure):
    _fields_ = [
        ("ch", C.c_int32), ("out_ch", C.c_int32), ("n_mult", C.c_int32), ("ch_mult", C.c_int32 * 8),
        ("num_res_blocks", C.c_int32), ("z_channels", C.c_int32), ("resolution", C.c_int32),
        ("n_embed", C.c_int32), ("embed_dim", C.c_int32), ("math", C.c_int32),
    ]


_pp = C.POINTER(C.c_void_p)

SIGNATURES = {
    "cs_conv_gemm": (_i, [C.POINTER(CsConvGemm), _s]),
    "cs_conv_gemm_plan": (_i, [C.POINTER(CsConvGemm), C.POINTER(C.c_int32), C.POINTER(C.c_int64)]),
    "cs_conv_gemm_epilogue_caps": (_i, [C.POINTER(CsConvGemm), C.POINTER(C.c_int32), C.POINTER(C.c_int32)]),
    "cs_conv_wino_ok": (_i, [C.POINTER(CsConvGemm)]),
    "cs_conv_wino_plan": (_i, [C.POINTER(CsConvGemm), C.POINTER(C.c_int32), C.POINTER(C.c_int64)]),
    "cs_conv_wino_plan_info": (_i, [C.POINTER(CsConvGemm), C.POINTER(C.c_int32), C.POINTER(C.c_int32), C.POINTER(C.c_int32)]),
    "cs_conv_wino_positions": (_i, [C.POINTER(CsConvGemm), _s]),
    "cs_conv_wino_output": (_i, [C.POINTER(CsConvGemm), _s]),
    "cs_conv_gemm_launch_info": (_i, [C.POINTER(CsConvGemm), C.POINTER(C.c_int32), C.POINTER(C.c_int32)]),
    "cs_debug": (C.POINTER(CsDebug), []),
    "cs_debug_set": (None, [C.POINTER(CsDebug)]),
    "cs_norm_a_scale": (_fl, [_fl, _fl, _l]),
    "cs_bound_a_scale": (_fl, [_fl]),
    "cs_weight_rowstats": (_i, [_f, _i, _i, _f, _s]),
    "cs_transformer_static_scales": (_i, [C.POINTER(CsTransformerStats), _i, _l, _i, _fl, _fl, _fl, _f]),
    "cs_conv_wants_split16": (_i, [_l, _i, _i, _i, _i, _i]),
    "cs_tapcol_ok": (_i, [_i, _i, _i, _i]),
    "cs_tapcol_tile": (_i, [_l, _i]),
    "cs_groupnorm_finalize_parts": (_i, [C.POINTER(CsGnSeg), _i, _i, _i, _i, _i, _fl, _f, _f, _s]),
    "cs_groupnorm_parts": (_i, [_f, C.POINTER(CsGnSeg), _i, _f, _f, _f, _i, _i, _i, _i, _i, _i, _fl, _i, _f, _f, _s]),
    "cs_conv_up2_info": (_i, [_i, _i, _i, C.POINTER(C.c_int32), C.POINTER(C.c_int32), C.POINTER(C.c_int32),
                              C.POINTER(C.c_int32)]),
    "cs_fold_upsample_weight": (_i, [_f, _f, _i, _i, _i, _i, _i, _s]),
    "cs_conv_gemm_up2_ws_bytes": (_l, [C.POINTER(CsConvGemm)]),
    "cs_conv_gemm_up2": (_i, [C.POINTER(CsConvGemm), _pp, _pp, C.POINTER(C.c_float), C.c_void_p, _s]),
    "cs_conv3d_3x3x3_s111": (_i, [_f, _f, _f, _f, _i, _i, _i, _i, _i, _i, _s]),
    "cs_conv3d_3x3x3_s122": (_i, [_f, _f, _f, _f, _i, _i, _i, _i, _i, _i, _s]),
    "cs_gemm_tokens": (_i, [_f, _f, _f, _f, _f, _i, _i, _i, _i, _s]),
    "cs_relayout_weight": (_i, [_f, _f, _i, _i, _i, _i, _i, _s]),
    "cs_pack_weight_f16x3": (_i, [_f, _f, _f, _i, _i, _i, _fl, _s]),
    "cs_pack_weight_f16x3_tapcol": (_i, [_f, _f, _f, _i, _i, _i, _fl, _s]),
    "cs_pack_weight_f16x3_wino": (_i, [_f, _f, _f, _i, _i, _fl, _s]),
    "cs_pack_weight_f16x3_wino_v": (_i, [_f, _f, _f, _i, _i, _fl, _i, _i, _i, _s]),
    "cs_tapsum27": (_i, [_f, _f, _f, _i, _i, _i, _i, _i, _i, _i, _s]),
    "cs_groupnorm_ws_bytes": (_l, [_i, _i]),
    "cs_groupnorm_stats": (_i, [_f, _i, _i, _i, _i, _i, _fl, _f, _f, _s]),
    "cs_groupnorm_stats_bound": (_i, [_f, _i, _i, _i, _i, _i, _fl, _f, _f, _f, _s]),
    "cs_groupnorm_apply": (_i, [_f, _f, _f, _f, _f, _i, _i, _i, _i, _i, _i, _i, _s]),
    "cs_groupnorm_apply_split16": (_i, [_f, _f, _f, _f, _f, _f, _i, _i, _i, _i, _i, _i, _i, _fl, _f, _s]),
    "cs_groupnorm_apply_wino16": (_i, [_f, _f, _f, _f, _f, _f, _i, _i, _i, _i, _i, _i, _i, _i, _i, _fl, _f, _s]),
    "cs_groupnorm_apply_wino16_range": (_i, [_f, _f, _f, _f, _f, _f, _i, _i, _i, _i, _i, _i, _i, _i, _i, _i, _i, _fl, _f, _s]),
    "cs_groupnorm_apply_wino_range": (_i, [_f, _f, _f, _f, _f, _f, _i, _i, _i, _i, _i, _i, _i, _i, _i, _i, _i, _fl, _i, _f, _s]),
    "cs_layernorm_pair16": (_i, [_f, _f, _f, _f, _i, _i, _i, _i, _fl, _fl, _f, _s]),
    "cs_groupnorm_apply_range": (_i, [_f, _f, _f, _f, _f, _i, _i, _i, _i, _i, _i, _i, _i, _i, _s]),
    "cs_groupnorm_apply_split16_range": (_i, [_f, _f, _f, _f, _f, _f, _i, _i, _i, _i, _i, _i, _i, _i, _i, _fl, _f, _s]),
    "cs_groupnorm": (_i, [_f, _f, _f, _f, _i, _i, _i, _i, _i, _i, _fl, _i, _f, _f, _s]),
    "cs_groupnorm_silu_ndhwc": (_i, [_f, _f, _f, _f, _i, _i, _i, _i, _fl, _f, _f, _s]),
    "cs_layernorm": (_i, [_f, _f, _f, _f, _i, _i, _i, _i, _fl, _s]),
    "cs_attn_selfattn": (_i, [_f, _f, _f, _f, _i, _i, _i, _i, _i, _i, _i, _i, _i, _fl, _s]),
    "cs_attn_selfattn_f16x3": (_i, [_f, _f, _f, _f, _i, _i, _i, _i, _i, _i, _i, _i, _i, _fl, _f, _s]),
    "cs_attn_selfattn_f16x3_scaled": (_i, [_f, _f, _f, _f, _i, _i, _i, _i, _i, _i, _i, _i, _i, _fl, _fl, _fl, _fl, _f, _s]),
    "cs_attn_f16x3_ws_bytes": (_l, [_i, _i, _i, _i, _i]),
    "cs_attn_selfattn_f16x3_ws": (_i, [_f, _f, _f, _f, _i, _i, _i, _i, _i, _i, _i, _i, _i, _fl, _f, _f, _s]),
    "cs_attn_selfattn_f16x3_ws_scaled": (_i, [_f, _f, _f, _f, _i, _i, _i, _i, _i, _i, _i, _i, _i, _fl, _fl, _fl, _fl, _f, _f, _s]),
    "cs_attnblock_static_scales": (_i, [_fl, _fl, _l, _i, _fl, _fl, _fl, _f]),
    "cs_attn_selfattn_f16": (_i, [_f, _f, _f, _f, _i, _i, _i, _i, _i, _i, _i, _i, _i, _fl, _f, _s]),
    "cs_geglu": (_i, [_f, _f, _i, _i, _i, _i, _s]),
    "cs_copy_rows": (_i, [_f, _f, _l, _i, _i, _i, _s]),
    "cs_add_rowvec": (_i, [_f, _f, _l, _i, _i, _i, _i, _s]),
    "cs_nchw_to_ndhwc": (_i, [_f, _f, _i, _i, _i, _i, _s]),
    "cs_absmax": (_i, [_f, _l, _f, _s]),
    "cs_ndhwc_to_nchw": (_i, [_f, _f, _i, _i, _i, _i, _s]),
    "cs_timestep_embedding": (_i, [_f, _f, _i, _i, _fl, _s]),
    "cs_ddim_cfg_update": (_i, [_f, _f, _f, _f, _f, _l, _l, _fl, _fl, _fl, _fl, _fl, _i, _s]),
    "cs_ddim_coefficients": (_i, [_fl, _fl, _fl, _fl, _f]),
    "cs_ddim_cfg_update_dev": (_i, [_f, _f, _f, _f, _f, _l, _l, _f, _fl, _i, _s]),
    "cs_plms_update": (_i, [_f, _f, _f, _f, _f, _f, _f, _f, _l, _l, _i, _fl, _fl, _fl, _fl, _i, _s]),
    "cs_chamfer_backward": (_i, [_f, _f, _f, _f, _f, _f, _f, _f, _i, _i, _i, _s]),
    "cs_emd_approxmatch": (_i, [_f, _f, _f, _f, _i, _i, _i, _s]),
    "cs_emd_matchcost": (_i, [_f, _f, _f, _f, _i, _i, _i, _s]),
    "cs_emd_matchcost_grad": (_i, [_f, _f, _f, _f, _f, _i, _i, _i, _s]),
    "cs_chamfer_pairwise": (_i, [_f, _f, _f, _i, _i, _i, _i, _i, _s]),
    "cs_emd_pairwise_cost": (_i, [_f, _f, _f, _i, _i, _i, _i, _s]),
    "cs_occupancy_histogram": (_i, [_f, _f, _f, _f, _f, _i, _i, _i, _s]),
    "cs_mc_blocks_per_object": (_i, [_i]),
    "cs_mc_count": (_i, [_f, _i, _i, _fl, _i, _f, _s]),
    "cs_mc_emit": (_i, [_f, _i, _i, _fl, _i, _f, _f, _f, _f, _f, _f, _fl, _fl, _s]),
    "cs_scene_fit_boxes": (_i, [_f, _l, _f, _f, _f, _i, _i, _f, _f, _s]),
    "cs_scene_apply": (_i, [_f, _l, _f, _l, _f, _f, _f, _f, _f, _f, _f, _f, _f, _i, _i, _f, _f, _l, _f, _f, _l, _s]),
    "cs_scene_raster_topdown": (_i, [_f, _l, _f, _l, _i, _fl, _f, _f, _s]),
    "cs_scene_resolve": (_i, [_f, _f, _l, _f, _l, _f, _f, _i, _f, _f, _f, _s]),
    "cs_scene_constraints": (_i, [_f, _l, _i, _i, _f, _l, _f, _f, _i, _f, _i, _f, _i, _f, C.c_double, _i, C.c_double, _f, _f, _f,
                                  _s]),
    "cs_box3d_iou_pairs": (_i, [_f, _f, _l, _i, _i, _i, _f, _f, _s]),
    "cs_chamfer_nm_distance": (_i, [_f, _f, _f, _f, _i, _i, _i, _s]),
    "cs_unet_create": (_i, [C.POINTER(CsUnetConfig), _pp]),
    "cs_unet_destroy": (None, [C.c_void_p]),
    "cs_unet_param_count": (_i, [C.c_void_p]),
    "cs_unet_param_info": (_i, [C.c_void_p, _i, C.POINTER(C.c_char_p), C.POINTER(C.c_int64 * 5), C.POINTER(C.c_int),
                                C.POINTER(C.c_int64)]),
    "cs_unet_raw_bytes": (_l, [C.c_void_p]),
    "cs_unet_arena_bytes": (_l, [C.c_void_p]),
    "cs_unet_context_floats": (_l, [C.c_void_p]),
    "cs_unet_set_context_bounds": (_i, [C.c_void_p, C.POINTER(C.c_float), _i]),
    "cs_unet_pack": (_i, [C.c_void_p, _f, _f, _s]),
    "cs_unet_workspace_bytes": (_l, [C.c_void_p, _i, _i]),
    "cs_unet_context": (_i, [C.c_void_p, _f, _f, _i, _f, _f, _f, _l, _s]),
    "cs_unet_step": (_i, [C.c_void_p, _f, _f, _f, _f, _f, _i, _i, _f, _f, _l, _s]),
    "cs_vq_argmin_lookup": (_i, [_f, _f, _f, _f, _l, _i, _i, _i, _i, _s]),
    "cs_vq_quantize_st": (_i, [_f, _f, _f, _f, _f, _f, _l, _i, _i, _i, _i, _i, _s]),
    "cs_vqenc_conv_in": (_i, [_f, _f, _f, _f, _i, _i, _i, _i, _i, _i, _s]),
    "cs_gcn_gather_cat": (_i, [_f, _f, _f, _f, _i, _i, _i, _i, _f, _s]),
    "cs_gcn_segment_mean": (_i, [_f, _f, _f, _i, _i, _i, _i, _i, _f, _s]),
    "cs_gcn_csr_ints": (_l, [_i, _i]),
    "cs_gcn_csr_build": (_i, [_f, _f, _i, _i, _f, _s]),
    "cs_gcn_segment_mean_csr": (_i, [_f, _f, _f, _i, _i, _i, _i, _s]),
    "cs_embedding": (_i, [_f, _f, _f, _i, _i, _i, _i, _f, _s]),
    "cs_log_softmax": (_i, [_f, _f, _i, _i, _i, _i, _s]),
    "cs_synth_fill": (_i, [_f, _l, C.c_uint64, C.c_double, C.c_double, _s]),
    "cs_vqvae_create": (_i, [C.POINTER(CsVqvaeConfig), _pp]),
    "cs_vqvae_destroy": (None, [C.c_void_p]),
    "cs_vqvae_param_count": (_i, [C.c_void_p]),
    "cs_vqvae_param_info": (_i, [C.c_void_p, _i, C.POINTER(C.c_char_p), C.POINTER(C.c_int64 * 5), C.POINTER(C.c_int),
                                 C.POINTER(C.c_int64)]),
    "cs_vqvae_raw_bytes": (_l, [C.c_void_p]),
    "cs_vqvae_arena_bytes": (_l, [C.c_void_p]),
    "cs_vqvae_pack": (_i, [C.c_void_p, _f, _f, _s]),
    "cs_vqvae_workspace_bytes": (_l, [C.c_void_p, _i]),
    "cs_vqvae_decode": (_i, [C.c_void_p, _f, _f, _f, _f, _i, _i, _f, _f, _l, _s]),
    "cs_abi_version": (_i, []),
}

_LIB = None


class NativeLibraryMissing(RuntimeError):
    pass


def load(path: Path | None = None) -> C.CDLL:
    global _LIB
    if _LIB is not None and path is None:
        return _LIB
    alt = os.environ.get("CS_LIB_PATH")
    p = Path(path) if path else (Path(alt) if alt else LIB_PATH)
    if not p.exists():
        raise NativeLibraryMissing(
            f"{p} not found. Build it with `python -m commonscenes_amd.build` "
            "(hipcc --offload-arch=gfx950); there is no CPU fallback.")
    lib = C.CDLL(str(p))
    for name, (res, args) in SIGNATURES.items():
        try:
            fn = getattr(lib, name)
        except AttributeError as e:
            raise NativeLibraryMissing(f"{p} does not export {name}") from e
        fn.restype = res
        fn.argtypes = args
    got = lib.cs_abi_version()
    if got != ABI_VERSION:
        raise NativeLibraryMissing(f"{p} has ABI version {got}, this package expects {ABI_VERSION}: rebuild it "
                                   "(`python -m commonscenes_amd.build --force`)")
    if path is None:
        _LIB = lib
    return lib


class CsError(RuntimeError):
    pass


class CsOverflowError(CsError):
    """A CS_MATH_F16X3 kernel met an activation beyond the fp16 range (CS_STATUS_F16X3_OVERFLOW)."""


class CsSplitKTimeout(CsError):
    """A reducer of a fused split-K launch gave up waiting for a slice that never reached a CU (CS_STATUS_SPLITK_TIMEOUT):
    the launch was not resident.  The host classes re-run with the two-kernel form."""


STATUS_F16X3_OVERFLOW = 1
STATUS_INTERNAL = 2
STATUS_SPLITK_TIMEOUT = 4
STATUS_CONSTRAINT_RANGE = 8


def check(rc: int, what: str) -> None:
    if rc != CS_OK:
        kind = {CS_EINVAL: "invalid argument", CS_ENOMEM: "workspace too small"}.get(rc, f"hipError_t {rc}")
        raise CsError(f"{what} failed: {kind}")


def debug() -> CsDebug:
    return load().cs_debug().contents


def debug_set(**fields) -> None:
    new = CsDebug.from_buffer_copy(debug())
    for k, v in fields.items():
        if not hasattr(new, k):
            raise AttributeError(f"CsDebug has no field {k!r}")
        setattr(new, k, int(v))
    load().cs_debug_set(C.byref(new))


class debug_override:

# ... 18 lines not shown
```

commonscenes_amd/ops.py:

```python
from __future__ import annotations

import ctypes as C
import dataclasses
from dataclasses import dataclass
from typing import Optional, Sequence, Tuple

import os

import torch

from . import lib as L

Tensor = torch.Tensor


def _stream() -> C.c_void_p:
    return C.c_void_p(torch.cuda.current_stream().cuda_stream)


def _ptr(t: Optional[Tensor]) -> Optional[int]:
    return None if t is None else t.data_ptr()


_STATUS: dict = {}
# ... 815 lines not shown
                                                      yh.data_ptr(), yl.data_ptr(), nb, int(x.shape[1]), int(x.shape[2]),
                                                      int(x.shape[3]), c, ldx, c, groups, c // groups, 0, act, a_sc, wino,
                                                      status_word(x.device).data_ptr(), _stream()),
                    "cs_groupnorm_apply_wino_range")
            return Wino16(yh, yl, a_sc, (nb, int(x.shape[1]), int(x.shape[2]), int(x.shape[3])), wino)
        a_sc = float(a_scale or A_SCALE)
        L.check(lib.cs_groupnorm_apply_split16(x.data_ptr(), stats.data_ptr(), gamma.data_ptr(), beta.data_ptr(),
                                               yh.data_ptr(), yl.data_ptr(), nb, rows, c, ldx, c, groups, act,
                                               a_sc, status_word(x.device).data_ptr(), _stream()),
                "cs_groupnorm_apply_split16")
        return Split16(yh, yl, a_sc)

    if segs is not None and not (split16 and _sw("SPLIT16_PRODUCERS")):
        if out is None:
            out = torch.empty(x.shape, dtype=torch.float32, device=x.device)
        om, oc, ldy = rows_ld(out, "out")
        if om != m or oc != c:
            raise L.CsError("groupnorm out shape mismatch")
        stats = torch.empty((nb, groups, 2), dtype=torch.float32, device=x.device)
        if not _sw("DYN_SCALE"):
            bound = None
        L.check(lib.cs_groupnorm_parts(x.data_ptr(), _seg_array(segs), len(segs), gamma.data_ptr(), beta.data_ptr(),
                                       out.data_ptr(), nb, rows, c, ldx, ldy, groups, eps, act, stats.data_ptr(),
                                       _ptr(bound), _stream()), "cs_groupnorm_parts")
        if bound is not None:
            x.cs_bound = bound
        return out
    if segs is not None:
        if not _sw("DYN_SCALE"):
            bound = None
        stats = groupnorm_stats_from_parts(segs, nb, rows, c, groups, eps, x.device, bound)
        if bound is not None:
            x.cs_bound = bound
        if split16 and _sw("SPLIT16_PRODUCERS"):
            return _emit(stats)
        if out is None:
            out = torch.empty(x.shape, dtype=torch.float32, device=x.device)
        om, oc, ldy = rows_ld(out, "out")
        if om != m or oc != c:
            raise L.CsError("groupnorm out shape mismatch")
        L.check(lib.cs_groupnorm_apply(x.data_ptr(), stats.data_ptr(), gamma.data_ptr(), beta.data_ptr(), out.data_ptr(),
                                       nb, rows, c, ldx, ldy, groups, act, _stream()), "cs_groupnorm_apply")
        return out
    ws = torch.empty(lib.cs_groupnorm_ws_bytes(nb, groups) // 8, dtype=torch.float64, device=x.device)
    stats = torch.empty((nb, groups, 2), dtype=torch.float32, device=x.device)
    want_bound = bound is not None and _sw("DYN_SCALE")

    def _stats():
        if want_bound:
            L.check(lib.cs_groupnorm_stats_bound(x.data_ptr(), nb, rows, c, ldx, groups, eps, ws.data_ptr(), stats.data_ptr(),
                                                 bound.data_ptr(), _stream()), "cs_groupnorm_stats_bound")
            x.cs_bound = bound
        else:
            L.check(lib.cs_groupnorm_stats(x.data_ptr(), nb, rows, c, ldx, groups, eps, ws.data_ptr(),
                                           stats.data_ptr(), _stream()), "cs_groupnorm_stats")
    if split16 and _sw("SPLIT16_PRODUCERS"):
        _stats()
        return _emit(stats)
    if out is None:
        out = torch.empty(x.shape, dtype=torch.float32, device=x.device)
    om, oc, ldy = rows_ld(out, "out")
    if om != m or oc != c:
        raise L.CsError("groupnorm out shape mismatch")
    if want_bound:
        _stats()
        L.check(lib.cs_groupnorm_apply(x.data_ptr(), stats.data_ptr(), gamma.data_ptr(), beta.data_ptr(), out.data_ptr(),
                                       nb, rows, c, ldx, ldy, groups, act, _stream()), "cs_groupnorm_apply")
        return out
    L.check(lib.cs_groupnorm(x.data_ptr(), gamma.data_ptr(), beta.data_ptr(), out.data_ptr(), nb, rows, c, ldx, ldy,
                             groups, eps, act, ws.data_ptr(), stats.data_ptr(), _stream()), "cs_groupnorm")
    return out


def groupnorm_stats(x: Tensor, groups: int, eps: float, bound: Optional[Tensor] = None) -> Tensor:
    _chk(x, "x")
    nb = x.shape[0]
    m, c, ldx = rows_ld(x, "x")
    lib = L.load()
    segs = stats_segments(x)
    if segs is not None:
        if bound is not None and _sw("DYN_SCALE"):
            x.cs_bound = bound
        else:
            bound = None
        return groupnorm_stats_from_parts(segs, nb, m // nb, c, groups, eps, x.device, bound)
    ws = torch.empty(lib.cs_groupnorm_ws_bytes(nb, groups) // 8, dtype=torch.float64, device=x.device)
    stats = torch.empty((nb, groups, 2), dtype=torch.float32, device=x.device)
    if bound is not None and _sw("DYN_SCALE"):
        L.check(lib.cs_groupnorm_stats_bound(x.data_ptr(), nb, m // nb, c, ldx, groups, eps, ws.data_ptr(), stats.data_ptr(),
                                             bound.data_ptr(), _stream()), "cs_groupnorm_stats_bound")
        x.cs_bound = bound
        return stats
    L.check(lib.cs_groupnorm_stats(x.data_ptr(), nb, m // nb, c, ldx, groups, eps, ws.data_ptr(), stats.data_ptr(),
                                   _stream()), "cs_groupnorm_stats")
    return stats


def groupnorm_apply_range(x: Tensor, stats: Tensor, gamma: Tensor, beta: Tensor, cpg: int, ch0: int,
                          act: int = L.ACT_NONE, split16: bool = False, a_scale: Optional[float] = None, wino: bool = False):
    _chk(x, "x"); _chk(stats, "stats")
    nb = x.shape[0]
    m, c, ldx = rows_ld(x, "x")
    groups = stats.shape[1]
    if stats.shape[0] < nb or not stats.is_contiguous() or gamma.numel() != c or beta.numel() != c:
        raise L.CsError("groupnorm_apply_range: stats / gamma / beta do not match x")
    lib = L.load()
    if wino and _sw("SPLIT16_PRODUCERS"):
        v = 4 if wino == 4 else 2
        if x.dim() != 5 or int(x.shape[3]) % v or c % 8:
            raise L.CsError("groupnorm_apply_range(wino=v) needs x as [nb, d, h, w, c] with w % v == 0 and c % 8 == 0")
        d_, h_, w_ = int(x.shape[1]), int(x.shape[2]), int(x.shape[3])
        yh = torch.empty((v + 2, nb, d_, h_, w_ // v, c), dtype=torch.float16, device=x.device)
        yl = torch.empty_like(yh)
        a_sc = float(a_scale or A_SCALE) * (0.5 if v == 2 else 0.0625)
        L.check(lib.cs_groupnorm_apply_wino_range(x.data_ptr(), stats.data_ptr(), gamma.data_ptr(), beta.data_ptr(),
                                                  yh.data_ptr(), yl.data_ptr(), nb, d_, h_, w_, c, ldx, c, groups, cpg,
                                                  ch0, act, a_sc, v, status_word(x.device).data_ptr(), _stream()),
                "cs_groupnorm_apply_wino_range")
        return Wino16(yh, yl, a_sc, (nb, d_, h_, w_), v)
    if split16 and _sw("SPLIT16_PRODUCERS"):
        yh = torch.empty(x.shape, dtype=torch.float16, device=x.device)
        yl = torch.empty(x.shape, dtype=torch.float16, device=x.device)
        a_sc = float(a_scale or A_SCALE)
        L.check(lib.cs_groupnorm_apply_split16_range(x.data_ptr(), stats.data_ptr(), gamma.data_ptr(), beta.data_ptr(),
                                                     yh.data_ptr(), yl.data_ptr(), nb, m // nb, c, ldx, c, groups, cpg,
                                                     ch0, act, a_sc, status_word(x.device).data_ptr(), _stream()),
                "cs_groupnorm_apply_split16_range")
        return Split16(yh, yl, a_sc)
    y = torch.empty(x.shape, dtype=torch.float32, device=x.device)
    L.check(lib.cs_groupnorm_apply_range(x.data_ptr(), stats.data_ptr(), gamma.data_ptr(), beta.data_ptr(), y.data_ptr(),
                                         nb, m // nb, c, ldx, c, groups, cpg, ch0, act, _stream()),
            "cs_groupnorm_apply_range")
    return y


def layernorm(x: Tensor, gamma: Tensor, beta: Tensor, eps: float = 1e-5, out: Optional[Tensor] = None,
              pair_scale: Optional[float] = None):
    _chk(x, "x")
    m, c, ldx = rows_ld(x, "x")
    if pair_scale is not None and _sw("PAIR16_PRODUCERS") and c % 16 == 0:
        y = torch.empty(x.shape, dtype=torch.float32, device=x.device)
        L.check(L.load().cs_layernorm_pair16(x.data_ptr(), gamma.data_ptr(), beta.data_ptr(), y.data_ptr(), m, c, ldx, c,
                                             eps, float(pair_scale), status_word(x.device).data_ptr(), _stream()),
                "cs_layernorm_pair16")
        return Pair16(y, float(pair_scale))
    if out is None:
        out = torch.empty(x.shape, dtype=torch.float32, device=x.device)
    _, _, ldy = rows_ld(out, "out")
    L.check(L.load().cs_layernorm(x.data_ptr(), gamma.data_ptr(), beta.data_ptr(), out.data_ptr(), m, c,
                                  ldx, ldy, eps, _stream()), "cs_layernorm")
    return out


def bound_a_scale(bound: float) -> float:
    return float(L.load().cs_bound_a_scale(float(bound)))


def attention(q: Tensor, k: Tensor, v: Tensor, heads: int, scale: float, out: Optional[Tensor] = None,
              math: int = L.MATH_FP32, scales: Optional[Tuple[float, float, float]] = None) -> Tensor:
    for t, n in ((q, "q"), (k, "k"), (v, "v")):
        _chk(t, n)
        if t.dim() != 3:
            raise L.CsError(f"{n} must be [nb, n, c]")
    nb, nq, cq = q.shape
    nk = k.shape[1]
    dh = cq // heads
    _, _, ldq = rows_ld(q, "q")
    _, _, ldk = rows_ld(k, "k")
    _, _, ldv = rows_ld(v, "v")
    if out is None:
        out = torch.empty((nb, nq, cq), dtype=torch.float32, device=q.device)
    _, _, ldo = rows_ld(out, "out")
    lib = L.load()
    if math == L.MATH_F16X3 and scales is not None:
        wsb = lib.cs_attn_f16x3_ws_bytes(nb, nq, nk, heads, dh)
        if wsb > 0:
            ws = torch.empty((wsb // 4,), dtype=torch.float32, device=q.device)
            L.check(lib.cs_attn_selfattn_f16x3_ws_scaled(q.data_ptr(), k.data_ptr(), v.data_ptr(), out.data_ptr(), nb, nq, nk,
                                                         heads, dh, ldq, ldk, ldv, ldo, scale, float(scales[0]),
                                                         float(scales[1]), float(scales[2]),
                                                         status_word(q.device).data_ptr(), ws.data_ptr(), _stream()),
                    "cs_attn_selfattn_f16x3_ws_scaled")
        else:
            L.check(lib.cs_attn_selfattn_f16x3_scaled(q.data_ptr(), k.data_ptr(), v.data_ptr(), out.data_ptr(), nb, nq, nk,
                                                      heads, dh, ldq, ldk, ldv, ldo, scale, float(scales[0]), float(scales[1]),
                                                      float(scales[2]), status_word(q.device).data_ptr(), _stream()),
                    "cs_attn_selfattn_f16x3_scaled")
    elif math == L.MATH_F16X3:
        wsb = lib.cs_attn_f16x3_ws_bytes(nb, nq, nk, heads, dh)
        ws = torch.empty((wsb // 4,), dtype=torch.float32, device=q.device) if wsb > 0 else None
        L.check(lib.cs_attn_selfattn_f16x3_ws(q.data_ptr(), k.data_ptr(), v.data_ptr(), out.data_ptr(), nb, nq, nk, heads,
                                              dh, ldq, ldk, ldv, ldo, scale, status_word(q.device).data_ptr(), _ptr(ws),
                                              _stream()), "cs_attn_selfattn_f16x3_ws")
    elif math == L.MATH_F16:
        L.check(lib.cs_attn_selfattn_f16(q.data_ptr(), k.data_ptr(), v.data_ptr(), out.data_ptr(), nb, nq, nk, heads, dh,
                                         ldq, ldk, ldv, ldo, scale, status_word(q.device).data_ptr(), _stream()),
                "cs_attn_selfattn_f16")
    else:
        L.check(lib.cs_attn_selfattn(q.data_ptr(), k.data_ptr(), v.data_ptr(), out.data_ptr(), nb, nq, nk, heads, dh,
                                     ldq, ldk, ldv, ldo, scale, _stream()), "cs_attn_selfattn")
    return out


def weight_rowstats(mats: Sequence[Tensor]) -> Tuple[float, float]:
    if not mats:
        return 0.0, 0.0
    lib = L.load()
    slot = torch.zeros((2,), dtype=torch.float32, device=mats[0].device)
    for m in mats:
        m = m.contiguous()
        L.check(lib.cs_weight_rowstats(m.data_ptr(), int(m.shape[0]), int(m.shape[1]), slot.data_ptr(), _stream()),
                "cs_weight_rowstats")
    v = slot.cpu().tolist()
    return float(v[0]), float(v[1])


def attnblock_static_scales(gmax: float, bmax: float, n: int, c: int, w_l2max: float, b_absmax: float,
                            qk_scale: float) -> Optional[Tuple[float, float, float, float]]:
    if not _sw("STATIC_SCALES") or not w_l2max > 0.0:
        return None
    o = (C.c_float * 4)()
    L.check(L.load().cs_attnblock_static_scales(float(gmax), float(bmax), int(n), int(c), float(w_l2max), float(b_absmax),
                                                float(qk_scale), o), "cs_attnblock_static_scales")
    return float(o[0]), float(o[1]), float(o[2]), float(o[3])


def geglu(x: Tensor, out: Optional[Tensor] = None) -> Tensor:
    _chk(x, "x")
    m, c2, ldx = rows_ld(x, "x")
    h = c2 // 2
    if out is None:
        out = torch.empty((*x.shape[:-1], h), dtype=torch.float32, device=x.device)
    _, _, ldo = rows_ld(out, "out")
    L.check(L.load().cs_geglu(x.data_ptr(), out.data_ptr(), m, h, ldx, ldo, _stream()), "cs_geglu")
    return out


def copy_rows(src: Tensor, dst: Tensor) -> Tensor:
    _chk(src, "src"); _chk(dst, "dst")
    m, c, lds = rows_ld(src, "src")
    dm, dc, ldd = rows_ld(dst, "dst")
    if dm != m or dc != c:
        raise L.CsError("copy_rows shape mismatch")
    L.check(L.load().cs_copy_rows(src.data_ptr(), dst.data_ptr(), m, c, lds, ldd, _stream()), "cs_copy_rows")
    return dst


def concat_channels(a: Tensor, b: Tensor) -> Tensor:
    ca, cb = a.shape[-1], b.shape[-1]
    out = torch.empty((*a.shape[:-1], ca + cb), dtype=torch.float32, device=a.device)
    copy_rows(a, out[..., :ca])
    if b.shape[0] == a.shape[0]:
        copy_rows(b, out[..., ca:])
    elif a.shape[0] % b.shape[0] == 0:
        nb = b.shape[0]
        for g in range(a.shape[0] // nb):
            copy_rows(b, out[g * nb:(g + 1) * nb, ..., ca:])
    else:
        raise L.CsError("concat_channels: batch mismatch")
    return out


def add_rowvec_(x: Tensor, v: Tensor, rows: int) -> Tensor:
    _chk(x, "x"); _chk(v, "v")
    m, c, ldx = rows_ld(x, "x")
    _, vc, ldv = rows_ld(v, "v")
    if vc != c:
        raise L.CsError("add_rowvec shape mismatch")
    L.check(L.load().cs_add_rowvec(x.data_ptr(), v.data_ptr(), m, c, ldx, ldv, rows, _stream()), "cs_add_rowvec")
    return x


def absmax_bound(x: Tensor, slot: Optional[Tensor]) -> Optional[Tensor]:
    if slot is None or not _sw("DYN_SCALE"):
        return None
    _chk(x, "x")
    if not x.is_contiguous():
        raise L.CsError("absmax_bound: contiguous tensor expected")
    L.check(L.load().cs_absmax(x.data_ptr(), x.numel(), slot.data_ptr(), _stream()), "cs_absmax")
    x.cs_bound = slot
    return slot


def nchw_to_ndhwc(x: Tensor, cpad: Optional[int] = None) -> Tensor:
    _chk(x, "x")
    x = x.contiguous()
    nb, c = x.shape[:2]
    sp = tuple(x.shape[2:])
    s = 1
    for v in sp:
        s *= v
    cp = cpad if cpad is not None else c
    y = torch.empty((nb, *sp, cp), dtype=torch.float32, device=x.device)
    L.check(L.load().cs_nchw_to_ndhwc(x.data_ptr(), y.data_ptr(), nb, c, s, cp, _stream()), "cs_nchw_to_ndhwc")
    return y


def ndhwc_to_nchw(x: Tensor, c: Optional[int] = None) -> Tensor:
    _chk(x, "x")
    m, cx, ldx = rows_ld(x, "x")
    nb = x.shape[0]
    sp = tuple(x.shape[1:-1])
    cc = c if c is not None else cx
    y = torch.empty((nb, cc, *sp), dtype=torch.float32, device=x.device)
    L.check(L.load().cs_ndhwc_to_nchw(x.data_ptr(), y.data_ptr(), nb, cc, m // nb, ldx, _stream()),
            "cs_ndhwc_to_nchw")
# ... 201 lines not shown
```

commonscenes_amd/unet.py:

```python
from __future__ import annotations

from collections import OrderedDict
from typing import Dict, List, Optional, Sequence, Tuple

import ctypes as C

import torch

from . import lib as L
from . import ops

Tensor = torch.Tensor


def _cfg(unet_params) -> dict:
    g = (lambda k, d=None: unet_params.get(k, d)) if isinstance(unet_params, dict) else (
        lambda k, d=None: getattr(unet_params, k, d))
    cfg = dict(
        image_size=int(g("image_size", 16)), in_channels=int(g("in_channels", 3)),
        out_channels=int(g("out_channels", 3)), model_channels=int(g("model_channels")),
        num_res_blocks=int(g("num_res_blocks")), attention_resolutions=tuple(g("attention_resolutions")),
        channel_mult=tuple(g("channel_mult")), num_heads=int(g("num_heads", -1)),
        context_dim=g("context_dim"), dims=int(g("dims", 3)),
        use_spatial_transformer=bool(g("use_spatial_transformer", True)),
# ... 379 lines not shown
                for l in layers:
                    if l["kind"] != "attn":
                        continue
                    p = f"{bp}.{l['idx']}"
                    wq, bq = sd[p + ".qkv.weight"], sd[p + ".qkv.bias"]
                    l2, _ = ops.weight_rowstats([wq.reshape(wq.shape[0], -1)])
                    _, bm = ops.weight_rowstats([bq.reshape(1, -1)])
                    self._abstat[p] = (l2, bm)
        self._packed = pk
        self._blocks = (inp, mid, out)
        self._ctx_cache = None

    def _nas(self, norm: str, n: int) -> Optional[float]:
        gb = self._ngb.get(norm)
        return ops.norm_a_scale(gb[0], gb[1], n) if gb is not None else None

    def _static_scales(self, p: str, t: str, c: int, n_tokens: int, ctx) -> Optional[Dict[str, object]]:
        st = self._tstat.get(t)
        if st is None or self.math != L.MATH_F16X3 or not ops._sw("STATIC_SCALES") or not isinstance(ctx, tuple):
            return None
        key = (t, n_tokens, id(ctx))
        cache = self.__dict__.setdefault("_sscache", {})
        hit = cache.get(key)
        if hit is not None:
            return hit
        gb = self._ngb.get(p + ".norm", (1.0, 0.0))
        cmax = float(ctx[3].get(t, 0.0)) if len(ctx) > 3 else 0.0
        o = (C.c_float * 12)()
        L.check(L.load().cs_transformer_static_scales(C.byref(st), int(c), int(n_tokens), int(self.cfg["num_heads"]),
                                                      float(gb[0]), float(gb[1]), cmax, o), "cs_transformer_static_scales")
        out = dict(attn=(float(o[0]), float(o[1]), float(o[2])), a=float(o[3]), gg=float(o[4]), t2=float(o[5]),
                   bounds=dict(q=float(o[6]), k=float(o[7]), v=float(o[8]), t1=float(o[9]), gg=float(o[10]), t2=float(o[11]),
                               ctx=cmax))
        cache[key] = out
        return out

    def _slot(self):
        a = getattr(self, "_amax", None)
        if a is None or self._amax_i >= a.numel():
            return None
        self._amax_i += 1
        return a[self._amax_i - 1:self._amax_i]

    def _res(self, p: str, l: dict, x: Tensor, semb: Tensor, out_fn=None) -> Tensor:
        sd, pk = self._sd, self._packed
        nb = x.shape[0]
        rows = x.shape[1] * x.shape[2] * x.shape[3]
        s1 = self._nas(p + ".in_layers.0", rows * (l["cin"] // 32))
        vol = (nb, int(x.shape[1]), int(x.shape[2]), int(x.shape[3]))
        hn = ops.groupnorm(x, sd[p + ".in_layers.0.weight"], sd[p + ".in_layers.0.bias"], 32, 1e-5, L.ACT_SILU,
                           split16=ops.wants_split16(nb * rows, pk[p + ".in_layers.2"]), a_scale=s1,
                           bound=self._slot() if l["cin"] != l["cout"] else None,
                           wino=ops.wants_wino(*vol, pk[p + ".in_layers.2"]))
        lo, hi = self._emb_slices[p]
        embo = semb[:, lo:hi]
        h = ops.conv_gemm(hn, pk[p + ".in_layers.2"], rowvec=embo, rv_rows=rows, math=self.math, a_scale=s1, stats=True)
        s2 = self._nas(p + ".out_layers.0", rows * (l["cout"] // 32))
        hn2 = ops.groupnorm(h, sd[p + ".out_layers.0.weight"], sd[p + ".out_layers.0.bias"], 32, 1e-5, L.ACT_SILU,
                            split16=ops.wants_split16(nb * rows, pk[p + ".out_layers.3"]), a_scale=s2,
                            wino=ops.wants_wino(*vol, pk[p + ".out_layers.3"]))
        skip = x if l["cin"] == l["cout"] else ops.conv_gemm(x, pk[p + ".skip_connection"], math=self.math,
                                                             x_bound=getattr(x, "cs_bound", None))
        return ops.conv_gemm(hn2, pk[p + ".out_layers.3"], res=skip, math=self.math, out_fn=out_fn, a_scale=s2,
                             stats=True)

    def _res_split(self, p: str, l: dict, x: Tensor, skip: Tensor, semb: Tensor, out_fn=None) -> Tensor:
        sd, pk = self._sd, self._packed
        ks, ch_h = self._split_info[p]
        nb, d, h, w, C = x.shape
        nbs = skip.shape[0]
        rows, cpg, off = d * h * w, C // 32, ks - ch_h
        if nb % nbs or skip.shape[-1] != C - ch_h:
            raise L.CsError("channel-split ResBlock: skip tensor does not match the concatenation")
        gam, bet = sd[p + ".in_layers.0.weight"], sd[p + ".in_layers.0.bias"]
        wh, ws = pk[p + ".in_layers.2:h"], pk[p + ".in_layers.2:s"]
        stats = ops.groupnorm_stats(x, 32, 1e-5, bound=self._slot())
        s1 = self._nas(p + ".in_layers.0", rows * cpg)
        wn_h, wn_s = ops.wants_wino(nbs, d, h, w, wh), ops.wants_wino(nbs, d, h, w, ws)
        a_h = None if wn_h else ops.groupnorm_apply_range(x[..., :ks], stats, gam[:ks], bet[:ks], cpg, 0, L.ACT_SILU,
                                                          split16=ops.wants_split16(nbs * rows, wh), a_scale=s1)
        a_s = ops.groupnorm_apply_range(skip[..., off:], stats, gam[ks:], bet[ks:], cpg, ks, L.ACT_SILU,
                                        split16=ops.wants_split16(nbs * rows, ws), a_scale=s1, wino=wn_s)
        y_s = ops.conv_gemm(a_s, ws, math=self.math, a_scale=s1)
        lo, hi = self._emb_slices[p]
        cout = l["cout"]
        h1 = torch.empty((nb, d, h, w, cout), dtype=torch.float32, device=x.device)
        for g in range(nb // nbs):
            sl = slice(g * nbs, (g + 1) * nbs)
            a_g = a_h[sl] if a_h is not None else ops.groupnorm_apply_range(
                x[sl][..., :ks], stats[sl], gam[:ks], bet[:ks], cpg, 0, L.ACT_SILU, a_scale=s1, wino=wn_h)
            ops.conv_gemm(a_g, wh, rowvec=semb[sl, lo:hi], rv_rows=rows, res=y_s, out=h1[sl], math=self.math,
                          a_scale=s1)
        sk = ops.conv_gemm(x, pk[p + ".skip_connection"], math=self.math, x_bound=getattr(x, "cs_bound", None))
        s2 = self._nas(p + ".out_layers.0", rows * (cout // 32))
        hn2 = ops.groupnorm(h1, sd[p + ".out_layers.0.weight"], sd[p + ".out_layers.0.bias"], 32, 1e-5, L.ACT_SILU,
                            split16=ops.wants_split16(nb * rows, pk[p + ".out_layers.3"]), a_scale=s2,
                            wino=ops.wants_wino(nb, d, h, w, pk[p + ".out_layers.3"]))
        return ops.conv_gemm(hn2, pk[p + ".out_layers.3"], res=sk, math=self.math, out_fn=out_fn, a_scale=s2,
                             stats=True)

    def _context_vectors(self, ctx: Tensor):
        if ctx.shape[1] != 1:
            return ctx
        key = (ctx.data_ptr(), ctx._version, tuple(ctx.shape), self.math)
        if self._ctx_cache is not None and self._ctx_cache[0] == key:
            return self._ctx_cache[1]
        pk = self._packed
        nb = ctx.shape[0]
        flat = ctx.reshape(nb, -1)
        vecs = {}
        b_ctx = None
        inp, mid, out = self._blocks
        P = self.prefix
        for bp, layers in ([(f"{P}input_blocks.{i}", l) for i, l in enumerate(inp)] + [(P + "middle_block", mid)]
                           + [(f"{P}output_blocks.{i}", l) for i, l in enumerate(out)]):
            for l in layers:
                if l["kind"] == "attn":
                    t = f"{bp}.{l['idx']}.transformer_blocks.0"
                    dyn = self.math == L.MATH_F16X3 and ops._sw("DYN_SCALE") and ops._sw("STATIC_SCALES")
                    if dyn and b_ctx is None:
                        b_ctx = flat.abs().max().reshape(1)
                    v2 = ops.linear(flat, pk[t + ".attn2.to_v"], math=self.math, x_bound=b_ctx if dyn else None)
                    vecs[t] = ops.linear(v2, pk[t + ".attn2.to_out.0"], math=self.math,
                                         x_bound=v2.abs().max().reshape(1) if dyn else None)
        cmax = {}
        if self.math == L.MATH_F16X3 and ops._sw("STATIC_SCALES") and vecs:
            ks = list(vecs)
            host = torch.stack([vecs[k_].abs().max() for k_ in ks]).cpu().tolist()
            cmax = {k_: float(v_) for k_, v_ in zip(ks, host)}
        cached = ("ctxvec", vecs, ctx, cmax)
        self._ctx_cache = (key, cached)
        self.__dict__.pop("_sscache", None)
        return cached

    def _attnblock(self, p: str, l: dict, x: Tensor, out_fn=None) -> Tensor:
        sd, pk = self._sd, self._packed
        heads = self.cfg["num_heads"]
        nb, d, h, w, c = x.shape
        n = d * h * w
        xn = ops.groupnorm(x, sd[p + ".norm.weight"], sd[p + ".norm.bias"], 32, 1e-5, L.ACT_NONE)
        qkv = ops.linear(xn.view(nb, n, c), pk[p + ".qkv"], math=self.math, a_scale=self._nas(p + ".norm", n * (c // 32)))
        amath = self.attn_math if self.attn_math is not None else self.math
        ss = None
        gb, st = self._ngb.get(p + ".norm"), self.__dict__.get("_abstat", {}).get(p)
        if self.math == L.MATH_F16X3 and gb is not None and st is not None:
            ss = ops.attnblock_static_scales(gb[0], gb[1], n * (c // 32), c, st[0], st[1], (c // heads) ** -0.5)
        a = ops.attention(qkv[..., 0:c], qkv[..., c:2 * c], qkv[..., 2 * c:3 * c], heads, (c // heads) ** -0.5, math=amath,
                          scales=ss[:3] if (ss is not None and amath == L.MATH_F16X3) else None)
        dst = out_fn((nb, d, h, w, c)).view(nb, n, c) if out_fn is not None else None
        out = ops.linear(a, pk[p + ".proj_out"], res=x.view(nb, n, c), math=self.math, out=dst, stats=True,
                         spatial=(nb, n, 1, 1), a_scale=ss[3] if ss is not None else None)
        return ops.attach_stats(out.view(nb, d, h, w, c), getattr(out, "cs_stats", None))

    def _attn(self, p: str, l: dict, x: Tensor, ctx, out_fn=None) -> Tensor:
        sd, pk = self._sd, self._packed
        heads = self.cfg["num_heads"]
        nb, d, h, w, c = x.shape
        n = d * h * w
        dh = c // heads
        t = p + ".transformer_blocks.0"
        xn = ops.groupnorm(x, sd[p + ".norm.weight"], sd[p + ".norm.bias"], 32, 1e-6, L.ACT_NONE)
        t0 = ops.linear(xn.view(nb, n, c), pk[p + ".proj_in"], math=self.math, a_scale=self._nas(p + ".norm", n * (c // 32)))
        s1 = self._nas(t + ".norm1", c)
        n1 = ops.layernorm(t0, sd[t + ".norm1.weight"], sd[t + ".norm1.bias"], pair_scale=s1)
        qkv = ops.linear(n1, pk[t + ".attn1.qkv"], math=self.math, a_scale=s1)
        ss = self._static_scales(p, t, c, n, ctx)
        amath = self.attn_math if self.attn_math is not None else self.math
        a = ops.attention(qkv[..., 0:c], qkv[..., c:2 * c], qkv[..., 2 * c:3 * c], heads, dh ** -0.5, math=amath,
                          scales=ss["attn"] if (ss is not None and amath == L.MATH_F16X3) else None)
        if isinstance(ctx, tuple):
            t1 = ops.linear(a, pk[t + ".attn1.to_out.0"], res=t0, rowvec=ctx[1][t], rv_rows=n, math=self.math,
                            a_scale=ss["a"] if ss is not None else None)
        else:
            t1a = ops.linear(a, pk[t + ".attn1.to_out.0"], res=t0, math=self.math)
            n2 = ops.layernorm(t1a, sd[t + ".norm2.weight"], sd[t + ".norm2.bias"])
            q2 = ops.linear(n2, pk[t + ".attn2.to_q"], math=self.math, a_scale=self._nas(t + ".norm2", c))
            k2 = ops.linear(ctx, pk[t + ".attn2.to_k"], math=self.math)
            vv2 = ops.linear(ctx, pk[t + ".attn2.to_v"], math=self.math)
            a2 = ops.attention(q2, k2, vv2, heads, dh ** -0.5, math=self.attn_math if self.attn_math is not None else self.math)
            t1 = ops.linear(a2, pk[t + ".attn2.to_out.0"], res=t1a, math=self.math)
        s3 = self._nas(t + ".norm3", c)
        n3 = ops.layernorm(t1, sd[t + ".norm3.weight"], sd[t + ".norm3.bias"], pair_scale=s3)
        on = self.math == L.MATH_F16X3 and ops._sw("PAIR_EPILOGUES")
        pair_gg = (ss["gg"] if ss is not None else ops.A_SCALE) if on else None
        pair_t2 = (ss["t2"] if ss is not None else ops.A_SCALE) if on else None
        if (t + ".ff.geglu") in pk:
            gg = ops.linear(n3, pk[t + ".ff.geglu"], act=L.ACT_GEGLU, a_scale=s3, out_pair=pair_gg)
        else:
            ff = ops.linear(n3, pk[t + ".ff.net.0.proj"], math=self.math, a_scale=s3)
            gg = ops.geglu(ff)
        t2 = ops.linear(gg, pk[t + ".ff.net.2"], res=t1, math=self.math, out_pair=pair_t2,
                        a_scale=None if isinstance(gg, ops.Pair16) or ss is None else ss["gg"])
        dst = out_fn((nb, d, h, w, c)).view(nb, n, c) if out_fn is not None else None
        out = ops.linear(t2, pk[p + ".proj_out"], res=x.view(nb, n, c), math=self.math, out=dst, stats=True,
                         spatial=(nb, n, 1, 1), a_scale=None if isinstance(t2, ops.Pair16) or ss is None else ss["t2"])
        return ops.attach_stats(out.view(nb, d, h, w, c), getattr(out, "cs_stats", None))

    def _run(self, bp: str, layers, h: Tensor, semb: Tensor, ctx: Tensor, out_fn=None, split_skip=None) -> Tensor:
        pk = self._packed
        for li, l in enumerate(layers):
            p = f"{bp}.{l['idx']}"
            k = l["kind"]
            of = out_fn if li == len(layers) - 1 else None
            if k == "conv_in":
                h = ops.conv_gemm(h, pk[p], math=self.math, out_fn=of, stats=True, x_bound=getattr(h, "cs_bound", None))
            elif k == "res":
                if li == 0 and split_skip is not None and p in self._split_info:
                    h = self._res_split(p, l, h, split_skip, semb, of)
                else:
                    h = self._res(p, l, h, semb, of)
            elif k == "attn":
                h = (self._attn(p, l, h, ctx, of) if self.cfg["use_spatial_transformer"]
                     else self._attnblock(p, l, h, of))
            elif k == "down":
                h = ops.conv_gemm(h, pk[p + ".op"], stride=(1, 2, 2) if self.cfg["dims"] == 3 else (2, 2, 2),
                                  math=self.math, out_fn=of, stats=True, x_bound=ops.range_bound(h, self._slot()))
            elif k == "up":
                h = ops.conv_gemm(h, pk[p + ".conv"], up=self._up, math=self.math, out_fn=of, stats=True,
                                  x_bound=ops.range_bound(h, self._slot()))
        return h

    @torch.no_grad()
    def forward_ndhwc(self, h: Tensor, t: Tensor, ctx: Tensor, cfg_pairs: bool = False) -> Tensor:
        if self._packed is None:
            self._pack()
        sd, pk, P = self._sd, self._packed, self.prefix
        inp, mid, out = self._blocks
        self._amax = (torch.zeros(64, dtype=torch.float32, device=h.device)
                      if self.math == L.MATH_F16X3 and ops._sw("DYN_SCALE") and ops._sw("GN_PARTS") else None)
        self._amax_i = 0
        if self._amax is not None:
            ops.absmax_bound(h, self._slot())
        temb = ops.timestep_embedding(t, self.cfg["model_channels"])
        e1 = ops.linear(temb, pk[P + "time_embed.0"], act=L.ACT_SILU, math=self.math)
        semb = ops.linear(e1, pk[P + "time_embed.2"], act=L.ACT_SILU, math=self.math)
        semb = ops.linear(semb, pk["emb_all"], math=self.math)
        ctx = self._context_vectors(ctx) if ctx is not None else None
        hs: List[Tensor] = []
        tr = self.trace
        nout = len(out)
        ch_skip = [layers[-1]["cout"] for layers in inp][::-1]
        ch_h = [out[j][0]["cin"] - ch_skip[j] for j in range(nout)]
        cats: List[Optional[Tensor]] = [None] * nout
        nocopy = not L.debug().concat_copy
        split_min_rows = self.split_min_rows
        seg_l: List[Optional[object]] = [None] * nout
        seg_r: List[Optional[object]] = [None] * nout

        def slot(j: int, left: bool):
            def fn(shape):
                want = (*shape[:-1], ch_h[j] + ch_skip[j])
                if cats[j] is None:
                    cats[j] = torch.empty(want, dtype=torch.float32, device=h.device)
                elif tuple(cats[j].shape) != want:
                    raise L.CsError(f"concat buffer {j}: {tuple(cats[j].shape)} vs {want}")
                return cats[j][..., :ch_h[j]] if left else cats[j][..., ch_h[j]:]
            return fn

        shared = cfg_pairs
        for i, layers in enumerate(inp):
            if shared and any(l["kind"] == "attn" for l in layers):
                st = getattr(h, "cs_stats", None)
                h = torch.cat([h, h], dim=0)
                ops.attach_stats(h, st)
                semb = torch.cat([semb, semb], dim=0)
                shared = False
            direct = nocopy and not shared
            h = self._run(f"{P}input_blocks.{i}", layers, h, semb, ctx, slot(nout - 1 - i, False) if direct else None)
            hs.append(None if direct else h)
            seg_r[nout - 1 - i] = getattr(h, "cs_stats", None)
            if tr is not None:
                tr[f"input_blocks.{i}"] = h
        if shared:
            st = getattr(h, "cs_stats", None)
            h = ops.attach_stats(torch.cat([h, h], dim=0), st)
            semb = torch.cat([semb, semb], dim=0)
        h = self._run(P + "middle_block", mid, h, semb, ctx, slot(0, True) if nocopy else None)
        seg_l[0] = getattr(h, "cs_stats", None)
        if tr is not None:
            tr["middle_block"] = h
        for i, layers in enumerate(out):
            skip = hs.pop()
            if not nocopy:
                h = ops.concat_channels(h, skip)
            else:
                if skip is not None:
                    right = slot(i, False)((h.shape[0], *skip.shape[1:]))
                    nbs = skip.shape[0]
                    for g in range(h.shape[0] // nbs):
                        ops.copy_rows(skip, right[g * nbs:(g + 1) * nbs])
                h = cats[i]
                cats[i] = None
                h.cs_segs = [(0, seg_l[i]), (ch_h[i], seg_r[i])]
            split_skip = None
            if (f"{P}output_blocks.{i}.0" in self._split_info
                    and h.shape[0] * h.shape[1] * h.shape[2] * h.shape[3] >= split_min_rows):
                split_skip = skip if skip is not None else h[..., ch_h[i]:]
            h = self._run(f"{P}output_blocks.{i}", layers, h, semb, ctx,
                          slot(i + 1, True) if nocopy and i + 1 < nout else None, split_skip=split_skip)
            if i + 1 < nout:
                seg_l[i + 1] = getattr(h, "cs_stats", None)
            if tr is not None:
                tr[f"output_blocks.{i}"] = h
        so = self._nas(P + "out.0", h.shape[1] * h.shape[2] * h.shape[3] * (h.shape[4] // 32))
        hn = ops.groupnorm(h, sd[P + "out.0.weight"], sd[P + "out.0.bias"], 32, 1e-5, L.ACT_SILU,
                           split16=ops.wants_split16(h.shape[0] * h.shape[1] * h.shape[2] * h.shape[3], pk[P + "out.2"]),
                           a_scale=so)
        return ops.conv_gemm(hn, pk[P + "out.2"], math=self.math, a_scale=so)

    @torch.no_grad()
    def forward_cfg(self, x: Tensor, t: Tensor, c_in: Tensor) -> Tensor:
        if self.conditioning_key == "concat":
            return self.forward(torch.cat([x, x]), torch.cat([t, t]), c_concat=[c_in])
        if self.conditioning_key != "crossattn":
            raise NotImplementedError("forward_cfg: crossattn / concat conditioning only")
        ctx = c_in.to(dtype=torch.float32).contiguous()
        if ctx.shape[0] != 2 * x.shape[0]:
            raise ValueError("c_in must hold [uc; c] for every sample of x")
        h = ops.nchw_to_ndhwc(x.to(torch.float32), cpad=(self.cfg["in_channels"] + 3) // 4 * 4)
        eps = self.forward_ndhwc(h, t.to(torch.int64).contiguous(), ctx, cfg_pairs=True)
        return ops.ndhwc_to_nchw(eps)

    @torch.no_grad()
    def forward(self, x: Tensor, t: Tensor, c_concat: Optional[list] = None,
                c_crossattn: Optional[list] = None) -> Tensor:
        if t.dtype != torch.int64:
            t = t.to(torch.int64)
        cpad = (self.cfg["in_channels"] + 3) // 4 * 4
        if self.conditioning_key == "concat":
            if not c_concat:
                raise ValueError("c_concat is required for conditioning_key='concat'")
            if self.cfg["use_spatial_transformer"]:
                raise NotImplementedError("concat conditioning with SpatialTransformer3D blocks (needs a context)")
            xc = torch.cat([x.to(torch.float32)] + [c.to(device=x.device, dtype=torch.float32) for c in c_concat], dim=1)
            if xc.shape[1] != self.cfg["in_channels"]:
                raise ValueError(f"x + c_concat have {xc.shape[1]} channels, in_channels={self.cfg['in_channels']}")
            return ops.ndhwc_to_nchw(self.forward_ndhwc(ops.nchw_to_ndhwc(xc, cpad=cpad), t.contiguous(), None))
        if self.conditioning_key != "crossattn":
            raise NotImplementedError(f"conditioning_key={self.conditioning_key!r}: 'crossattn' "
                                      "(config/sdfusion-txt2shape.yaml:5) and 'concat' "
                                      "(config/sdfusion-txt2shape_concat.yaml:5) are implemented")
        if not self.cfg["use_spatial_transformer"]:
            raise NotImplementedError("crossattn conditioning needs use_spatial_transformer=True")
        if c_crossattn is None:
            raise ValueError("c_crossattn is required for conditioning_key='crossattn'")
        ctx = c_crossattn[0] if len(c_crossattn) == 1 else torch.cat(c_crossattn, 1)
        ctx = ctx.to(dtype=torch.float32).contiguous()
        if t.dtype != torch.int64:
            t = t.to(torch.int64)
        h = ops.nchw_to_ndhwc(x.to(torch.float32), cpad=(self.cfg["in_channels"] + 3) // 4 * 4)
        eps = self.forward_ndhwc(h, t.contiguous(), ctx)
        return ops.ndhwc_to_nchw(eps)

    __call__ = forward
```

commonscenes_amd/unet_native.py:

```python
from __future__ import annotations

import ctypes as C
from collections import OrderedDict
from typing import Dict, List, Optional, Tuple

import torch

from . import lib as L
from . import ops
from .unet import _cfg

Tensor = torch.Tensor


def _stream() -> int:
    return torch.cuda.current_stream().cuda_stream


class NativeDiffusionUNet:
    def __init__(self, unet_params, vq_conf=None, conditioning_key: Optional[str] = "crossattn",
                 device: str | torch.device = "cuda", math: str | int | None = None, grid: Tuple[int, int, int] = (16, 16, 16)):
        self.cfg = _cfg(unet_params)
        self.conditioning_key = conditioning_key
        self.device = torch.device(device)
        self.math = L.DEFAULT_MATH if math is None else {"fp32": L.MATH_FP32, "f16x3": L.MATH_F16X3}.get(math, math)
        self.grid = tuple(grid)
        self._h = None
        self._arena: Optional[Tensor] = None
        self._sd: Dict[str, Tensor] = {}
        self._ws: Optional[Tensor] = None
        self._ws_key = None
        self._ctx_cache = None
        self._create()

    def _create(self):
        cfg = self.cfg
        c = L.CsUnetConfig()
        c.in_channels, c.out_channels = cfg["in_channels"], cfg["out_channels"]
        c.model_channels, c.num_res_blocks = cfg["model_channels"], cfg["num_res_blocks"]
        mult, ar = list(cfg["channel_mult"]), list(cfg["attention_resolutions"])
        if len(mult) > 8 or len(ar) > 8:
            raise L.CsError("channel_mult / attention_resolutions: at most 8 entries")
        c.n_mult, c.n_attn_res = len(mult), len(ar)
        for i, v in enumerate(mult):
            c.channel_mult[i] = int(v)
        for i, v in enumerate(ar):
            c.attention_resolutions[i] = int(v)
        c.num_heads, c.context_dim = cfg["num_heads"], int(cfg["context_dim"] or 0)
        c.d, c.h, c.w = self.grid
        c.math = self.math
        c.use_spatial_transformer, c.dims = int(cfg["use_spatial_transformer"]), cfg["dims"]
        lib = L.load()
        h = C.c_void_p()
        L.check(lib.cs_unet_create(C.byref(c), C.byref(h)), "cs_unet_create")
        self._h = h
        self.params: "OrderedDict[str, Tuple[Tuple[int, ...], int]]" = OrderedDict()
        name, shape, nd, off = C.c_char_p(), (C.c_int64 * 5)(), C.c_int(), C.c_int64()
        for i in range(lib.cs_unet_param_count(h)):
            L.check(lib.cs_unet_param_info(h, i, C.byref(name), C.byref(shape), C.byref(nd), C.byref(off)),
                    "cs_unet_param_info")
            self.params[name.value.decode()] = (tuple(int(shape[k]) for k in range(nd.value)), int(off.value))
        self.ctx_floats = int(lib.cs_unet_context_floats(h))

    def __del__(self):
        h, self._h = getattr(self, "_h", None), None
        if h:
            try:
                L.load().cs_unet_destroy(h)
            except Exception:
                pass

    @property
    def shapes(self) -> "OrderedDict[str, Tuple[int, ...]]":
        return OrderedDict((k, v[0]) for k, v in self.params.items())

    def state_dict(self) -> "OrderedDict[str, Tensor]":
        return OrderedDict((k, self._sd[k]) for k in self.params if k in self._sd)

    def load_state_dict(self, sd, strict: bool = True):
        if self.device.type != "cuda":
            raise L.CsError("NativeDiffusionUNet: weights must be on the HIP device (no CPU path)")
        missing = [k for k in self.params if k not in sd]
        unexpected = [k for k in sd if k not in self.params]
        if missing or (strict and unexpected):
            raise RuntimeError(f"NativeDiffusionUNet.load_state_dict: missing {missing[:5]} unexpected {unexpected[:5]}")
        lib = L.load()
        raw = torch.empty(int(lib.cs_unet_raw_bytes(self._h)), dtype=torch.uint8, device=self.device)
        for k, (shp, off) in self.params.items():
            t = sd[k]
            if tuple(t.shape) != shp:
                raise RuntimeError(f"size mismatch for {k}: {tuple(t.shape)} vs {shp}")
            n = t.numel()
            dst = raw[off:off + 4 * n].view(torch.float32).view(shp)
            dst.copy_(t.detach().to(device=self.device, dtype=torch.float32))
            self._sd[k] = dst
        self._raw = raw
        self._arena = torch.empty(int(lib.cs_unet_arena_bytes(self._h)), dtype=torch.uint8, device=self.device)
        L.check(lib.cs_unet_pack(self._h, raw.data_ptr(), self._arena.data_ptr(), _stream()), "cs_unet_pack")
        self._ctx_cache = None
        return self

    def set_math(self, mode) -> "NativeDiffusionUNet":
        m = {"fp32": L.MATH_FP32, "f16x3": L.MATH_F16X3}.get(mode, mode)
        if m not in (L.MATH_FP32, L.MATH_F16X3):
            raise ValueError(f"unknown math mode {mode!r}")
        if m != self.math:
            self.math = m
            sd = dict(self._sd)
            self.__del__()
            self._create()
            self._ws_key = None
            if sd:
                self.load_state_dict(sd)
        return self

    def parameters(self):
        return iter(self._sd.values())

    def eval(self):
        return self

    def num_parameters(self) -> int:
        n = 0
        for shp, _ in self.params.values():
            k = 1
            for v in shp:
                k *= v
            n += k
        return n

    def _workspace(self, nb_x: int, cfg_pairs: bool) -> Tensor:
        key = (nb_x, cfg_pairs)
        if self._ws_key != key:
            need = int(L.load().cs_unet_workspace_bytes(self._h, nb_x, 1 if cfg_pairs else 0))
            if need < 0:
                L.check(need, "cs_unet_workspace_bytes")
            if self._ws is None or self._ws.numel() < need:
                self._ws = torch.empty(need, dtype=torch.uint8, device=self.device)
            self._ws_key = key
        return self._ws

    def reset_run_cache(self) -> None:
        self._ctx_cache = None

    def check_overflow(self) -> None:
        ops.check_overflow(self.device, "NativeDiffusionUNet")

    def context_vectors(self, ctx: Tensor, ws: Tensor) -> Tensor:
        if ctx.dim() == 3:
            if ctx.shape[1] != 1:
                raise NotImplementedError("the native driver implements the shipped one-token context (SURVEY F4)")
            ctx = ctx[:, 0]
        key = (ctx.data_ptr(), ctx._version, tuple(ctx.shape))
        if self._ctx_cache is not None and self._ctx_cache[0] == key:
            return self._ctx_cache[1]
        ctx = ctx.to(torch.float32).contiguous()
        vec = torch.empty((ctx.shape[0], self.ctx_floats), dtype=torch.float32, device=self.device)
        L.check(L.load().cs_unet_context(self._h, self._arena.data_ptr(), ctx.data_ptr(), ctx.shape[0], vec.data_ptr(),
                                         ops.status_word(self.device).data_ptr(), ws.data_ptr(), ws.numel(),
                                         _stream()), "cs_unet_context")
        if self.math == L.MATH_F16X3 and self.cfg["use_spatial_transformer"] and not L.debug().no_static_scales:
            from .unet import unet_blocks
            inp, mid, out = unet_blocks(self.cfg)[:3]
            widths = [l["cin"] for layers in (list(inp) + [mid] + list(out)) for l in layers if l["kind"] == "attn"]
            if widths and sum(widths) != self.ctx_floats:
                raise L.CsError(f"cs_unet context row vector has {self.ctx_floats} floats, the attention blocks' widths sum "
                                f"to {sum(widths)}: cannot derive the per-block context bounds")
            if widths:
                mx = torch.stack([seg.abs().max() for seg in torch.split(vec, widths, dim=1)]).cpu().tolist()
                arr = (C.c_float * len(widths))(*[float(v) for v in mx])
                L.check(L.load().cs_unet_set_context_bounds(self._h, arr, len(widths)), "cs_unet_set_context_bounds")
        self._ctx_cache = (key, vec, ctx)
        return vec

    def _step(self, x: Tensor, t: Tensor, ctx: Tensor, cfg_pairs: bool) -> Tensor:
        if self._arena is None:
            raise RuntimeError("NativeDiffusionUNet: weights not loaded")
        x = x.to(torch.float32).contiguous()
        t = t.to(torch.int64).contiguous()
        nb = x.shape[0]
        if tuple(x.shape[1:]) != (self.cfg["in_channels"], *self.grid):
            raise ValueError(f"x must be (B, {self.cfg['in_channels']}, {self.grid}), got {tuple(x.shape)}")
        ws = self._workspace(nb, cfg_pairs)
        nbo = 2 * nb if cfg_pairs else nb
        if ctx is None:
            vec_ptr = None
        else:
            vec = self.context_vectors(ctx, ws)
            if vec.shape[0] != nbo:
                raise ValueError("context batch does not match x")
            vec_ptr = vec.data_ptr()
        out = torch.empty((nbo, self.cfg["out_channels"], *self.grid), dtype=torch.float32, device=self.device)
        L.check(L.load().cs_unet_step(self._h, self._arena.data_ptr(), x.data_ptr(), t.data_ptr(), vec_ptr,
                                      out.data_ptr(), nb, 1 if cfg_pairs else 0,
                                      ops.status_word(self.device).data_ptr(), ws.data_ptr(), ws.numel(), _stream()),
                "cs_unet_step")
        return out

    @torch.no_grad()
    def forward_cfg(self, x: Tensor, t: Tensor, c_in: Tensor) -> Tensor:
        if self.conditioning_key == "concat":
            return self.forward(torch.cat([x, x]), torch.cat([t, t]), c_concat=[c_in])
        return self._step(x, t, c_in, True)

    @torch.no_grad()
    def forward(self, x: Tensor, t: Tensor, c_concat: Optional[list] = None,
                c_crossattn: Optional[list] = None) -> Tensor:
        if self.conditioning_key == "concat":
            if not c_concat or self.cfg["use_spatial_transformer"]:
                raise NotImplementedError("concat conditioning needs c_concat and AttentionBlock blocks")
            xc = torch.cat([x.to(torch.float32)] + [c.to(device=x.device, dtype=torch.float32) for c in c_concat], dim=1)
            return self._step(xc, t, None, False)
        if self.conditioning_key != "crossattn" or not self.cfg["use_spatial_transformer"]:
            raise NotImplementedError(f"conditioning_key={self.conditioning_key!r} with this block type")
        if c_crossattn is None:
            raise ValueError("c_crossattn is required for conditioning_key='crossattn'")
        ctx = c_crossattn[0] if len(c_crossattn) == 1 else torch.cat(c_crossattn, 1)
        return self._step(x, t, ctx, False)

    __call__ = forward
```

include/commonscenes_hip.h:

```cpp
#ifndef COMMONSCENES_HIP_H
#define COMMONSCENES_HIP_H

#include <stdint.h>

#ifdef __cplusplus
extern "C" {
#endif

typedef struct ihipStream_t* cs_stream_t;

#define CS_OK 0
#define CS_ENOMEM (-12)
#define CS_EINVAL (-22)

#define CS_ACT_NONE 0
#define CS_ACT_RELU 1
#define CS_ACT_SILU 2
#define CS_ACT_GELU 3
#define CS_ACT_GEGLU 4

#define CS_STATUS_F16X3_OVERFLOW 1
#define CS_STATUS_INTERNAL 2
#define CS_STATUS_SPLITK_TIMEOUT 4
#define CS_STATUS_CONSTRAINT_RANGE 8

typedef struct CsDebug {
  int32_t no_split16;
  int32_t no_pair16;
  int32_t no_upfold;
  int32_t no_splitk;
  int32_t no_fused_geglu;
  int32_t no_tapcol;
  int32_t tapcol_tile;
  int32_t no_cfg_split;
  int32_t concat_copy;
  int32_t tile512;
  int32_t no_pw;
  int32_t no_slab4;
  int32_t no_attn_img;
  int32_t attn_nw8;
  int32_t no_up2_direct;
  int32_t no_up2_batch;
  int32_t plan_pow2;
  int32_t slice_tile2;
  int32_t no_gn_parts;
  int32_t no_pair_epilogue;
  int32_t no_dyn_scale;
  int32_t no_tok_rules;
  int32_t no_fused_reduce;
  int32_t no_gn_fold;
  int32_t no_kwave;
  int32_t no_static_scales;
  int32_t no_wino;
  int32_t wino_min_rows;
  int32_t no_wino43;
  int32_t wino43_min_rows;
  int32_t no_wino_tail;
  int64_t split16_min_rows;
  int64_t cfg_split_min_rows;
  int64_t gn_small_group;
} CsDebug;
const CsDebug* cs_debug(void);
void cs_debug_set(const CsDebug* d);

float cs_norm_a_scale(float gmax, float bmax, int64_t n);
float cs_bound_a_scale(float bound);
int cs_attnblock_static_scales(float gmax, float bmax, int64_t n, int c, float w_l2max, float b_absmax, float qk_scale,
                               float* out4);
typedef struct CsTransformerStats {
  float rq, rk, rv;
  float ro, bo;
  float rx, bx, rg, bg;
  float r2, b2;
  float rpi, bpi;
  float g1, be1, g3, be3;
} CsTransformerStats;
int cs_weight_rowstats(const float* w, int rows, int cols, float* out2, cs_stream_t stream);
int cs_transformer_static_scales(const CsTransformerStats* st, int c, int64_t n_tokens, int heads, float gn_gmax,
                                 float gn_bmax, float ctx_max, float* out12);
int cs_conv_wants_split16(int64_t m, int cin, int cout, int k, int plain, int math);
int cs_tapcol_ok(int cout, int cin, int k, int math);
int cs_tapcol_tile(int64_t m, int ncolp);

#define CS_MATH_FP32 0
#define CS_MATH_F16X3 1

typedef struct CsConvGemm {
  const float* x;
  const float* w;
  float* out;
  const float* bias;
  const float* scale;
  const float* shift;
  const float* rowvec;
  const float* res;
  int32_t nb, din, hin, win;
  int32_t dout, hout, wout;
  int32_t cin, cout;
  int32_t lda, ldw, ldo, ldr, ldrv;
  int32_t kd, kh, kw;
  int32_t sd, sh, sw;
  int32_t pd, ph, pw;
  int32_t ud, uh, uw;
  int32_t act;
  int32_t rv_rows;
  int32_t math;
  int32_t tile;
  const void* w_lo;
  float acc_scale;
  float a_scale;
  const void* x_lo;
  int32_t a_format;
  int32_t splitk;
  void* splitk_ws;
  int32_t* status;
  double* gn_part;
  int32_t gn_ld;
  int32_t gn_rows;
  int32_t out_format;
  float out_scale;
  const float* a_bound;
  int32_t* splitk_sync;
  int32_t splitk_sync_words;
} CsConvGemm;

int cs_conv_gemm(const CsConvGemm* desc, cs_stream_t stream);

int cs_conv_gemm_epilogue_caps(const CsConvGemm* desc, int32_t* gn_rows, int32_t* pair_ok);

int cs_conv_gemm_launch_info(const CsConvGemm* desc, int32_t* tile, int32_t* slab);

int cs_conv_gemm_plan(const CsConvGemm* desc, int32_t* splitk, int64_t* splitk_ws_bytes);
int cs_conv_wino_ok(const CsConvGemm* desc);
int cs_conv_wino_plan(const CsConvGemm* desc, int32_t* splitk, int64_t* ws_bytes);
int cs_conv_wino_plan_info(const CsConvGemm* desc, int32_t* slices, int32_t* units_main, int32_t* units);
int cs_conv_wino_positions(const CsConvGemm* desc, cs_stream_t stream);
int cs_conv_wino_output(const CsConvGemm* desc, cs_stream_t stream);

int cs_conv_up2_info(int ud, int uh, int uw, int32_t* ncls, int32_t* kd, int32_t* kh, int32_t* kw);
int cs_fold_upsample_weight(const float* w_torch, float* w_folded, int cout, int cin, int ud, int uh, int uw,
                            cs_stream_t stream);
int64_t cs_conv_gemm_up2_ws_bytes(const CsConvGemm* desc);
int cs_conv_gemm_up2(const CsConvGemm* desc, const void* const* w_cls, const void* const* w_lo_cls,
                     const float* acc_scale_cls, void* ws, cs_stream_t stream);

int cs_conv3d_3x3x3_s111(const float* x, const float* w, const float* bias, float* out,
                         int nb, int d, int h, int w_, int cin, int cout, cs_stream_t stream);
int cs_conv3d_3x3x3_s122(const float* x, const float* w, const float* bias, float* out,
                         int nb, int d, int h, int w_, int cin, int cout, cs_stream_t stream);
int cs_gemm_tokens(const float* x, const float* w, const float* bias, const float* res, float* out,
                   int m, int k, int n, int act, cs_stream_t stream);

int cs_relayout_weight(const float* w_torch, float* w_out, int cout, int cin, int taps,
                       int cin_pad, int ldw, cs_stream_t stream);

int cs_pack_weight_f16x3(const float* w_torch, void* w_hi, void* w_lo, int cout, int cin, int taps,
                         float scale, cs_stream_t stream);
int cs_pack_weight_f16x3_wino(const float* w_torch, void* w_hi, void* w_lo, int cout, int cin, float scale,
                              cs_stream_t stream);
int cs_pack_weight_f16x3_wino_v(const float* w_torch, void* w_hi, void* w_lo, int cout, int cin, float scale, int variant,
                                int src_cin, int c0, cs_stream_t stream);

int cs_pack_weight_f16x3_tapcol(const float* w_torch, void* w_hi, void* w_lo, int cout, int cin, int ncolp, float scale,
                                cs_stream_t stream);
int cs_tapsum27(const float* y, const float* bias, float* out, int nb, int d, int h, int w, int cout, int ldy, int ldo,
                cs_stream_t stream);

int64_t cs_groupnorm_ws_bytes(int nb, int groups);
int cs_groupnorm_stats(const float* x, int nb, int rows, int c, int ldx, int groups, float eps,
                       void* ws, float* stats, cs_stream_t stream);
int cs_groupnorm_stats_bound(const float* x, int nb, int rows, int c, int ldx, int groups, float eps, void* ws,
                             float* stats, float* bound, cs_stream_t stream);
int cs_groupnorm_apply(const float* x, const float* stats, const float* gamma, const float* beta,
                       float* y, int nb, int rows, int c, int ldx, int ldy, int groups, int act,
                       cs_stream_t stream);
int cs_groupnorm_apply_split16(const float* x, const float* stats, const float* gamma, const float* beta,
                               void* y_hi, void* y_lo, int nb, int rows, int c, int ldx, int ldy, int groups,
                               int act, float a_scale, int32_t* status, cs_stream_t stream);
int cs_groupnorm_apply_wino16(const float* x, const float* stats, const float* gamma, const float* beta, void* v_hi,
                              void* v_lo, int nb, int d, int h, int w, int c, int ldx, int ldv, int groups, int act,
                              float a_scale, int32_t* status, cs_stream_t stream);
int cs_groupnorm_apply_wino16_range(const float* x, const float* stats, const float* gamma, const float* beta, void* v_hi,
                                    void* v_lo, int nb, int d, int h, int w, int c, int ldx, int ldv, int groups, int cpg,
                                    int ch0, int act, float a_scale, int32_t* status, cs_stream_t stream);
int cs_groupnorm_apply_wino_range(const float* x, const float* stats, const float* gamma, const float* beta, void* v_hi,
                                  void* v_lo, int nb, int d, int h, int w, int c, int ldx, int ldv, int groups, int cpg,
                                  int ch0, int act, float a_scale, int variant, int32_t* status, cs_stream_t stream);
int cs_groupnorm_apply_range(const float* x, const float* stats, const float* gamma, const float* beta, float* y,
                             int nb, int rows, int c, int ldx, int ldy, int groups, int cpg, int ch0, int act,
                             cs_stream_t stream);
int cs_groupnorm_apply_split16_range(const float* x, const float* stats, const float* gamma, const float* beta,
                                     void* y_hi, void* y_lo, int nb, int rows, int c, int ldx, int ldy, int groups,
                                     int cpg, int ch0, int act, float a_scale, int32_t* status, cs_stream_t stream);
int cs_groupnorm(const float* x, const float* gamma, const float* beta, float* y, int nb, int rows, int c, int ldx,
                 int ldy, int groups, float eps, int act, void* ws, float* stats, cs_stream_t stream);
typedef struct CsGnSeg {
  const double* part;
  int32_t ld;
  int32_t col0;
  int32_t ch0;
  int32_t nch;
  int32_t tiles_per_sample;
  int32_t ncls;
  int32_t nb_src;
  int32_t reserved;
} CsGnSeg;
int cs_groupnorm_finalize_parts(const CsGnSeg* segs, int nseg, int nb, int rows, int c, int groups, float eps,
                                float* stats, float* bound, cs_stream_t stream);
int cs_groupnorm_parts(const float* x, const CsGnSeg* segs, int nseg, const float* gamma, const float* beta, float* y,
                       int nb, int rows, int c, int ldx, int ldy, int groups, float eps, int act, float* stats,
                       float* bound, cs_stream_t stream);
int cs_groupnorm_silu_ndhwc(const float* x, const float* gamma, const float* beta, float* y,
                            int nb, int rows, int c, int groups, float eps, void* ws, float* stats,
                            cs_stream_t stream);

int cs_layernorm(const float* x, const float* gamma, const float* beta, float* y, int m, int c,
                 int ldx, int ldy, float eps, cs_stream_t stream);

int cs_layernorm_pair16(const float* x, const float* gamma, const float* beta, void* y, int m, int c, int ldx, int ldy,
                        float eps, float a_scale, int32_t* status, cs_stream_t stream);

int cs_attn_selfattn(const float* q, const float* k, const float* v, float* out, int nb, int nq,
                     int nk, int heads, int dh, int ldq, int ldk, int ldv, int ldo, float scale,
                     cs_stream_t stream);

int cs_attn_selfattn_f16x3(const float* q, const float* k, const float* v, float* out, int nb, int nq,
                           int nk, int heads, int dh, int ldq, int ldk, int ldv, int ldo, float scale,
                           int32_t* status, cs_stream_t stream);

int cs_attn_selfattn_f16x3_scaled(const float* q, const float* k, const float* v, float* out, int nb, int nq, int nk,
                                  int heads, int dh, int ldq, int ldk, int ldv, int ldo, float scale, float q_scale,
                                  float k_scale, float v_scale, int32_t* status, cs_stream_t stream);
int64_t cs_attn_f16x3_ws_bytes(int nb, int nq, int nk, int heads, int dh);
int cs_attn_selfattn_f16x3_ws(const float* q, const float* k, const float* v, float* out, int nb, int nq,
                              int nk, int heads, int dh, int ldq, int ldk, int ldv, int ldo, float scale,
                              int32_t* status, void* ws, cs_stream_t stream);
int cs_attn_selfattn_f16x3_ws_scaled(const float* q, const float* k, const float* v, float* out, int nb, int nq,
                                     int nk, int heads, int dh, int ldq, int ldk, int ldv, int ldo, float scale,
                                     float q_scale, float k_scale, float v_scale, int32_t* status, void* ws,
                                     cs_stream_t stream);

int cs_attn_selfattn_f16(const float* q, const float* k, const float* v, float* out, int nb, int nq,
                         int nk, int heads, int dh, int ldq, int ldk, int ldv, int ldo, float scale,
                         int32_t* status, cs_stream_t stream);

int cs_geglu(const float* x, float* out, int m, int h, int ldx, int ldo, cs_stream_t stream);

int cs_copy_rows(const float* src, float* dst, int64_t m, int c, int lds, int ldd,
                 cs_stream_t stream);

int cs_add_rowvec(float* x, const float* v, int64_t m, int c, int ldx, int ldv, int rows,
                  cs_stream_t stream);

int cs_nchw_to_ndhwc(const float* x, float* y, int nb, int c, int s, int cpad, cs_stream_t stream);
int cs_absmax(const float* x, int64_t n, float* slot, cs_stream_t stream);
int cs_ndhwc_to_nchw(const float* x, float* y, int nb, int c, int s, int ldx, cs_stream_t stream);

int cs_timestep_embedding(const int64_t* t, float* out, int nb, int dim, float max_period,
                          cs_stream_t stream);

int cs_ddim_cfg_update(const float* x, const float* eps, const float* noise, float* x_prev,
                       float* pred_x0, int64_t nb, int64_t per, float a_t, float a_prev,
                       float sigma_t, float sqrt_one_minus_at, float cfg_scale, int cfg,
                       cs_stream_t stream);

int cs_ddim_coefficients(float a_t, float a_prev, float sigma_t, float sqrt_one_minus_at, float* coef5_host);
int cs_ddim_cfg_update_dev(const float* x, const float* eps, const float* noise, float* x_prev,
                           float* pred_x0, int64_t nb, int64_t per, const float* coef5_dev,
                           float cfg_scale, int cfg, cs_stream_t stream);

#define CS_PLMS_PLAIN 0
#define CS_PLMS_AB2 1
#define CS_PLMS_AB3 2
#define CS_PLMS_AB4 3
#define CS_PLMS_EULER_AVG 4
int cs_plms_update(const float* x, const float* eps, const float* h1, const float* h2, const float* h3,
                   float* e_out, float* x_prev, float* pred_x0, int64_t nb, int64_t per, int mode, float a_t,
                   float a_prev, float sqrt_one_minus_at, float cfg_scale, int cfg, cs_stream_t stream);

int cs_vq_argmin_lookup(const float* z, const float* codebook, int64_t* idx, float* zq, int64_t m,
                        int ncode, int edim, int ldz, int ldq, cs_stream_t stream);

#define CS_VQ_ST_ROWS 256
int cs_vq_quantize_st(const float* z, const float* codebook, int64_t* idx, float* zst, double* part, double* loss,
                      int64_t rows, int nb, int ncode, int edim, int ldz, int ldq, cs_stream_t stream);

int cs_vqenc_conv_in(const float* x, const float* w, const float* bias, float* out, int nb, int d, int h, int wd,
                     int cout, int ldo, cs_stream_t stream);

int cs_gcn_gather_cat(const float* obj, const float* pred, const int64_t* edges, float* out,
                      int n_obj, int n_tri, int d_obj, int d_pred, int32_t* err,
                      cs_stream_t stream);
int cs_gcn_segment_mean(const float* new_t, const int64_t* edges, float* pooled, int n_obj,
                        int n_tri, int h, int off_o, int ld_t, int32_t* err, cs_stream_t stream);

int64_t cs_gcn_csr_ints(int n_obj, int n_tri);
int cs_gcn_csr_build(const int64_t* edges, int32_t* csr, int n_obj, int n_tri, int32_t* err, cs_stream_t stream);
int cs_gcn_segment_mean_csr(const float* new_t, const int32_t* csr, float* pooled, int n_obj, int h, int off_o,
                            int ld_t, cs_stream_t stream);

int cs_embedding(const float* table, const int64_t* idx, float* out, int n, int dim, int n_rows,
                 int ldo, int32_t* err, cs_stream_t stream);

int cs_log_softmax(const float* x, float* y, int m, int c, int ldx, int ldy, cs_stream_t stream);

int cs_synth_fill(float* out, int64_t n, uint64_t base, double scale, double offset, cs_stream_t stream);

int cs_chamfer_nm_distance(const float* xyz1, const float* xyz2, float* dist, int32_t* idx, int b, int n, int m,
                           cs_stream_t stream);

int cs_chamfer_backward(const float* xyz1, const float* xyz2, const float* grad_dist1, const float* grad_dist2,
                        const int32_t* idx1, const int32_t* idx2, float* grad_xyz1, float* grad_xyz2, int b, int n,
                        int m, cs_stream_t stream);

int cs_emd_approxmatch(const float* xyz1, const float* xyz2, float* match, float* temp, int b, int n, int m,
                       cs_stream_t stream);
int cs_emd_matchcost(const float* xyz1, const float* xyz2, const float* match, float* out, int b, int n, int m,
                     cs_stream_t stream);
int cs_emd_matchcost_grad(const float* xyz1, const float* xyz2, const float* match, float* grad1, float* grad2, int b,
                          int n, int m, cs_stream_t stream);

#define CS_CHAMFER_PAIRWISE_MAX_Q 32768
#define CS_EMD_PAIRWISE_MAX_POINTS 8192
#define CS_OCCUPANCY_MAX_CELLS 524288
int cs_chamfer_pairwise(const float* a, const float* b, float* out, int na, int nb, int p, int q, int symmetric,
                        cs_stream_t stream);
int cs_emd_pairwise_cost(const float* a, const float* b, float* cost, int na, int nb, int n, int m, cs_stream_t stream);
int cs_occupancy_histogram(const float* clouds, const float* grid, int32_t* idx, int32_t* counters, int32_t* bernoulli,
                           int s, int p, int g, cs_stream_t stream);

int cs_mc_blocks_per_object(int n);
#define CS_MC_TABLE_CLASSIC 0
#define CS_MC_TABLE_WATERTIGHT 1
int cs_mc_count(const float* sdf, int nb, int n, float level, int table, int32_t* block_sums, cs_stream_t stream);
int cs_mc_emit(const float* sdf, int nb, int n, float level, int table, const int32_t* block_sums, const int64_t* vert_base,
               const int64_t* face_base, float* verts, int64_t* faces, int32_t* voxel_ws, float vert_div,
               float vert_shift, cs_stream_t stream);

int cs_scene_fit_boxes(const float* verts, int64_t total_verts, const int64_t* vert_base, const int64_t* vert_count,
                       const float* box7, int n, int degrees, float* xform, float* box_points, cs_stream_t stream);
int cs_scene_apply(const float* verts, int64_t total_verts, const int64_t* faces, int64_t total_faces,
                   const int64_t* vert_base, const int64_t* vert_count, const int64_t* face_base, const int64_t* face_count,
                   const float* xform, const uint8_t* keep, const int64_t* out_vert_base, const int64_t* out_face_base,
                   const float* color, int n, int flip, float* out_verts, float* out_rgb, int64_t out_nverts,
                   int64_t* out_faces, int32_t* face_object, int64_t out_nfaces, cs_stream_t stream);
int cs_scene_raster_topdown(const float* verts, int64_t nverts, const int64_t* faces, int64_t nfaces, int size, float znear,
                            uint64_t* keys, int32_t* dropped, cs_stream_t stream);
int cs_scene_resolve(const uint64_t* keys, const float* verts, int64_t nverts, const int64_t* faces, int64_t nfaces,
                     const float* vert_rgb, const int32_t* face_object, int size, float* depth, int32_t* object_id,
                     uint8_t* rgb, cs_stream_t stream);

int cs_scene_constraints(const float* boxes, int64_t n_boxes, int ld, int params, const int64_t* triples, int64_t n_triples,
                         const int64_t* box_ptr, const int64_t* triple_ptr, int n_scenes, const int32_t* pred_code,
                         int n_preds, const uint8_t* keep, int mode, const double* norm, double scale, int strict,
                         double overlap_threshold, int8_t* verdict, int32_t* counts, int32_t* status, cs_stream_t stream);
int cs_box3d_iou_pairs(const float* box1, const float* box2, int64_t m, int ld, int params, int with_translation, double* iou,
                       double* iou_2d, cs_stream_t stream);

typedef struct CsUnetConfig {
  int32_t in_channels, out_channels, model_channels, num_res_blocks;
  int32_t n_mult;
  int32_t channel_mult[8];
  int32_t n_attn_res;
  int32_t attention_resolutions[8];
  int32_t num_heads, context_dim;
  int32_t d, h, w;
  int32_t math;
  int32_t use_spatial_transformer;
  int32_t dims;
} CsUnetConfig;
typedef struct cs_unet cs_unet;

int cs_unet_create(const CsUnetConfig* cfg, cs_unet** out);
void cs_unet_destroy(cs_unet* u);
// ... 45 lines not shown
```

Baseline: 15.80.

## Defer CFG batch split to the first attention's context-dependent output projection

```diff
diff --git a/commonscenes_amd/build.py b/commonscenes_amd/build.py
--- a/commonscenes_amd/build.py
+++ b/commonscenes_amd/build.py
@@ -10,8 +10,8 @@
 CSRC = PKG_DIR / "csrc"
 LIB_NAME = "libcommonscenes_hip.so"
 LIB_PATH = PKG_DIR / LIB_NAME
-SOURCES = ["cs_plan.hip", "cs_gemm.hip", "cs_gemm_f16x3.hip", "cs_gemm_kw.hip", "cs_mesh.hip", "cs_scene.hip", "cs_constraints.hip", "cs_metrics.hip", "cs_pairwise.hip", "cs_norm.hip", "cs_attention.hip", "cs_attention_f16x3.hip", "cs_ops.hip", "cs_unet.hip", "cs_vqvae.hip", "cs_vqenc.hip"]
-HEADERS = [CSRC / "cs_common.h", CSRC / "cs_f16x3.h", CSRC / "cs_mc_tables.h", CSRC / "cs_driver.h", CSRC / "cs_vq.h", PKG_DIR.parent / "include" / "commonscenes_hip.h"]
+SOURCES = ["cs_plan.hip", "cs_gemm.hip", "cs_gemm_f16x3.hip", "cs_gemm_kw.hip", "cs_mesh.hip", "cs_scene.hip", "cs_constraints.hip", "cs_metrics.hip", "cs_pairwise.hip", "cs_norm.hip", "cs_twin_ln.hip", "cs_attention.hip", "cs_attention_f16x3.hip", "cs_ops.hip", "cs_unet.hip", "cs_vqvae.hip", "cs_vqenc.hip"]
+HEADERS = [CSRC / "cs_common.h", CSRC / "cs_f16x3.h", CSRC / "cs_mc_tables.h", CSRC / "cs_driver.h", CSRC / "cs_vq.h", CSRC / "cs_ln_pair.h", PKG_DIR.parent / "include" / "commonscenes_hip.h"]
 ARCH = "gfx950"
 FLAGS = ["-O3", "-std=c++17", "-fPIC", "-ffp-contract=off", f"--offload-arch={ARCH}", "-Wall",
          "-Wno-unused-function"]
diff --git a/commonscenes_amd/csrc/cs_gemm.hip b/commonscenes_amd/csrc/cs_gemm.hip
--- a/commonscenes_amd/csrc/cs_gemm.hip
+++ b/commonscenes_amd/csrc/cs_gemm.hip
@@ -643,6 +643,19 @@
   return CS_OK;
 }
 
+static thread_local int tl_plan_copies = 1;
+extern "C" int cs_conv_plan_copies(int copies) {
+  if (copies < 1 || copies > 64) return CS_EINVAL;
+  const int prev = tl_plan_copies;
+  tl_plan_copies = copies;
+  return prev;
+}
+static CsConvGemm planned(const CsConvGemm& p) {
+  CsConvGemm q = p;
+  if (tl_plan_copies > 1 && (int64_t)p.nb * tl_plan_copies <= 0x7fffffffLL) q.nb = p.nb * tl_plan_copies;
+  return q;
+}
+
 static int64_t kwave_max_tiles() {
   static const int64_t v = [] {
     const char* e = getenv("CS_KWAVE_MAX_TILES");
@@ -659,8 +672,10 @@
   return v;
 }
 
-static int auto_tile(const CsConvGemm& p, int M, bool f16x3) {
+static int auto_tile(const CsConvGemm& p, int M_launch, bool f16x3) {
   int tile = 0;
+  const int64_t M_all = (int64_t)M_launch * tl_plan_copies;
+  const int M = M_all > 0x7fffffffLL ? 0x7fffffff : (int)M_all;
   {
     const int64_t mt = (M + 127) / 128;
     if (f16x3 && p.cout % 224 == 0 && ((M + 255) / 256) * (int64_t)(p.cout / 224) >= 192)
@@ -754,7 +769,7 @@
   if ((512 + 2LL * p.hin * (p.win / 2) + p.win + 32) * p.lda * 4 >= 0x7FF00000LL) return false;
   return true;
 }
-static int wino_variant(const CsConvGemm& p) {
+static int wino_variant_at(const CsConvGemm& p) {
   if (!wino23_ok(p)) return 0;
   const CsDebug* dbg = cs_debug();
   const int64_t M = (int64_t)p.nb * p.dout * p.hout * p.wout;
@@ -763,6 +778,14 @@
   if (!dbg->no_wino43 && p.win % 4 == 0 && (M / 4) % 256 == 0 && (rdec / 4) % 256 == 0 && rdec >= min43) return 4;
   return 2;
 }
+static int wino_variant(const CsConvGemm& p) {
+  const int v = wino_variant_at(p);
+  if (!v || tl_plan_copies <= 1) return v;
+  const int vq = wino_variant_at(planned(p));
+  const int64_t M = (int64_t)p.nb * p.dout * p.hout * p.wout;
+  if (vq == 4 && v == 2) return (p.win % 4 == 0 && (M / 4) % 256 == 0 && !cs_debug()->no_wino43) ? 4 : 2;
+  return vq ? vq : v;
+}
 static inline int wino_pos(int variant) { return variant + 2; }
 
 struct WinoPlan {
@@ -771,7 +794,8 @@
 };
 static int wino_splits(const CsConvGemm& p, int variant, double* cost_us = nullptr);
 
-static WinoPlan wino_plan(const CsConvGemm& p, int variant) {
+static WinoPlan wino_plan(const CsConvGemm& p_launch, int variant) {
+  const CsConvGemm p = planned(p_launch);
   WinoPlan pl;
   double t_uni = 0;
   pl.slices = wino_splits(p, variant, &t_uni);
diff --git a/commonscenes_amd/csrc/cs_ln_pair.h b/commonscenes_amd/csrc/cs_ln_pair.h
--- /dev/null
+++ b/commonscenes_amd/csrc/cs_ln_pair.h
@@ -0,0 +1,45 @@
+#pragma once
+#include "cs_common.h"
+
+typedef _Float16 cs_h4v __attribute__((ext_vector_type(4)));
+
+template <int MAXV>
+__device__ __forceinline__ float cs_ln_pair_row(const float4 (&v)[MAXV], float s, int lane, int ch4, int c,
+                                                const float* __restrict__ gamma, const float* __restrict__ beta,
+                                                _Float16* __restrict__ yrow, float eps, float a_scale, float amax) {
+  const float mean = wave_sum(s) / (float)c;
+  float q = 0.f;
+#pragma unroll
+  for (int k = 0; k < MAXV; ++k) {
+    const int c4 = lane + 64 * k;
+    if (c4 < ch4) {
+      const float a = v[k].x - mean, b = v[k].y - mean, cc = v[k].z - mean, d = v[k].w - mean;
+      q += (a * a + b * b) + (cc * cc + d * d);
+    }
+  }
+  const float var = wave_sum(q) / (float)c;
+  const float rstd = 1.0f / sqrtf(var + eps);
+#pragma unroll
+  for (int k = 0; k < MAXV; ++k) {
+    const int c4 = lane + 64 * k;
+    if (c4 < ch4) {
+      const float4 g = *reinterpret_cast<const float4*>(gamma + c4 * 4);
+      const float4 b = *reinterpret_cast<const float4*>(beta + c4 * 4);
+      const float o[4] = {((v[k].x - mean) * rstd * g.x + b.x) * a_scale, ((v[k].y - mean) * rstd * g.y + b.y) * a_scale,
+                          ((v[k].z - mean) * rstd * g.z + b.z) * a_scale, ((v[k].w - mean) * rstd * g.w + b.w) * a_scale};
+      cs_h4v hi, lo;
+#pragma unroll
+      for (int e = 0; e < 4; ++e) {
+        amax = fmaxf(amax, fabsf(o[e]));
+        const _Float16 h = (_Float16)o[e];
+        hi[e] = h;
+        lo[e] = (_Float16)(o[e] - (float)h);
+      }
+      const int cch = c4 >> 2, j = (c4 & 3) * 4;
+      _Float16* dst = yrow + cch * 32 + (j < 8 ? 0 : 16) + (j & 7);
+      *reinterpret_cast<cs_h4v*>(dst) = hi;
+      *reinterpret_cast<cs_h4v*>(dst + 8) = lo;
+    }
+  }
+  return amax;
+}
diff --git a/commonscenes_amd/csrc/cs_norm.hip b/commonscenes_amd/csrc/cs_norm.hip
--- a/commonscenes_amd/csrc/cs_norm.hip
+++ b/commonscenes_amd/csrc/cs_norm.hip
@@ -1,6 +1,7 @@
 #include <cstdlib>
 
 #include "cs_common.h"
+#include "cs_ln_pair.h"
 
 namespace {
 
@@ -568,40 +569,7 @@
       if (c4 < ch4) v[k] = *reinterpret_cast<const float4*>(x + row * ldx + c4 * 4);
       s += (v[k].x + v[k].y) + (v[k].z + v[k].w);
     }
-    const float mean = wave_sum(s) / (float)c;
-    float q = 0.f;
-#pragma unroll
-    for (int k = 0; k < MAXV; ++k) {
-      const int c4 = lane + 64 * k;
-      if (c4 < ch4) {
-        const float a = v[k].x - mean, b = v[k].y - mean, cc = v[k].z - mean, d = v[k].w - mean;
-        q += (a * a + b * b) + (cc * cc + d * d);
-      }
-    }
-    const float var = wave_sum(q) / (float)c;
-    const float rstd = 1.0f / sqrtf(var + eps);
-#pragma unroll
-    for (int k = 0; k < MAXV; ++k) {
-      const int c4 = lane + 64 * k;
-      if (c4 < ch4) {
-        const float4 g = *reinterpret_cast<const float4*>(gamma + c4 * 4);
-        const float4 b = *reinterpret_cast<const float4*>(beta + c4 * 4);
-        const float o[4] = {((v[k].x - mean) * rstd * g.x + b.x) * a_scale, ((v[k].y - mean) * rstd * g.y + b.y) * a_scale,
-                            ((v[k].z - mean) * rstd * g.z + b.z) * a_scale, ((v[k].w - mean) * rstd * g.w + b.w) * a_scale};
-        h4v hi, lo;
-#pragma unroll
-        for (int e = 0; e < 4; ++e) {
-          amax = fmaxf(amax, fabsf(o[e]));
-          const _Float16 h = (_Float16)o[e];
-          hi[e] = h;
-          lo[e] = (_Float16)(o[e] - (float)h);
-        }
-        const int cch = c4 >> 2, j = (c4 & 3) * 4;
-        _Float16* dst = y + row * (int64_t)ldy * 2 + cch * 32 + (j < 8 ? 0 : 16) + (j & 7);
-        *reinterpret_cast<h4v*>(dst) = hi;
-        *reinterpret_cast<h4v*>(dst + 8) = lo;
-      }
-    }
+    amax = cs_ln_pair_row<MAXV>(v, s, lane, ch4, c, gamma, beta, y + row * (int64_t)ldy * 2, eps, a_scale, amax);
   }
   if (status && amax >= 65504.f) atomicOr(status, CS_STATUS_F16X3_OVERFLOW);
 }
diff --git a/commonscenes_amd/csrc/cs_plan.hip b/commonscenes_amd/csrc/cs_plan.hip
--- a/commonscenes_amd/csrc/cs_plan.hip
+++ b/commonscenes_amd/csrc/cs_plan.hip
@@ -55,6 +55,7 @@
   d.no_wino43 = flag("CS_NO_WINO43");
   d.wino43_min_rows = (int32_t)num("CS_WINO43_MIN_ROWS", 2048);
   d.no_wino_tail = flag("CS_NO_WINO_TAIL");
+  d.no_cfg_late_split = flag("CS_NO_CFG_LATE_SPLIT");
 }
 
 }
diff --git a/commonscenes_amd/csrc/cs_twin_ln.hip b/commonscenes_amd/csrc/cs_twin_ln.hip
--- /dev/null
+++ b/commonscenes_amd/csrc/cs_twin_ln.hip
@@ -0,0 +1,85 @@
+#include "cs_common.h"
+#include "cs_ln_pair.h"
+
+namespace {
+
+template <int MAXV>
+__global__ __launch_bounds__(256) void twin_ln_pair_kernel(const float* __restrict__ y, const float* __restrict__ rowvec,
+                                                           const float* __restrict__ res, const float* __restrict__ gamma,
+                                                           const float* __restrict__ beta, float* __restrict__ t1,
+                                                           _Float16* __restrict__ pair, int m, int c, int ldy, int ldrv,
+                                                           int rv_rows, int ldr, int ldt, int ldp, float eps, float a_scale,
+                                                           int32_t* __restrict__ status) {
+  const int lane = threadIdx.x & 63;
+  const int wave = threadIdx.x >> 6;
+  const int ch4 = c >> 2;
+  float amax = 0.f;
+  for (int64_t row = (int64_t)blockIdx.x * 4 + wave; row < m; row += (int64_t)gridDim.x * 4) {
+    float4 a[MAXV], r[MAXV];
+#pragma unroll
+    for (int k = 0; k < MAXV; ++k) {
+      const int c4 = lane + 64 * k;
+      a[k] = r[k] = make_float4(0.f, 0.f, 0.f, 0.f);
+      if (c4 < ch4) {
+        a[k] = *reinterpret_cast<const float4*>(y + row * ldy + c4 * 4);
+        r[k] = *reinterpret_cast<const float4*>(res + row * ldr + c4 * 4);
+      }
+    }
+#pragma unroll
+    for (int g = 0; g < 2; ++g) {
+      const int64_t orow = (int64_t)g * m + row;
+      const float* rv = rowvec + orow / rv_rows * ldrv;
+      float4 v[MAXV];
+      float s = 0.f;
+#pragma unroll
+      for (int k = 0; k < MAXV; ++k) {
+        const int c4 = lane + 64 * k;
+        v[k] = make_float4(0.f, 0.f, 0.f, 0.f);
+        if (c4 < ch4) {
+          const float4 w = *reinterpret_cast<const float4*>(rv + c4 * 4);
+          v[k].x = (a[k].x + w.x) + r[k].x;
+          v[k].y = (a[k].y + w.y) + r[k].y;
+          v[k].z = (a[k].z + w.z) + r[k].z;
+          v[k].w = (a[k].w + w.w) + r[k].w;
+          *reinterpret_cast<float4*>(t1 + orow * ldt + c4 * 4) = v[k];
+        }
+        s += (v[k].x + v[k].y) + (v[k].z + v[k].w);
+      }
+      amax = cs_ln_pair_row<MAXV>(v, s, lane, ch4, c, gamma, beta, pair + orow * (int64_t)ldp * 2, eps, a_scale, amax);
+    }
+  }
+  if (status && amax >= 65504.f) atomicOr(status, CS_STATUS_F16X3_OVERFLOW);
+}
+
+}
+
+extern "C" int cs_twin_layernorm_pair16(const float* y, const float* rowvec, const float* res, const float* gamma,
+                                        const float* beta, float* t1, void* pair, int m, int c, int ldy, int ldrv, int rv_rows,
+                                        int ldr, int ldt, int ldp, float eps, float a_scale, int32_t* status,
+                                        cs_stream_t stream) {
+  if (!y || !rowvec || !res || !gamma || !beta || !t1 || !pair || m <= 0 || c <= 0 || rv_rows <= 0 || !(a_scale > 0.f))
+    return CS_EINVAL;
+  if ((c & 15) || (ldy & 3) || (ldrv & 3) || (ldr & 3) || (ldt & 3) || (ldp & 15) || ldy < c || ldrv < c || ldr < c || ldt < c ||
+      ldp < c)
+    return CS_EINVAL;
+  if (((uintptr_t)y & 15) || ((uintptr_t)rowvec & 15) || ((uintptr_t)res & 15) || ((uintptr_t)gamma & 15) ||
+      ((uintptr_t)beta & 15) || ((uintptr_t)t1 & 15) || ((uintptr_t)pair & 15))
+    return CS_EINVAL;
+  const int ch4 = c >> 2;
+  const int grid = cs_grid_for(((int64_t)m + 3) / 4, 1, 256 * 32);
+  hipStream_t s = (hipStream_t)stream;
+  _Float16* po = (_Float16*)pair;
+  if (ch4 <= 64 * 2)
+    CS_LAUNCH(twin_ln_pair_kernel<2>, dim3(grid), dim3(256), 0, s, y, rowvec, res, gamma, beta, t1, po, m, c, ldy, ldrv, rv_rows,
+              ldr, ldt, ldp, eps, a_scale, status);
+  else if (ch4 <= 64 * 4)
+    CS_LAUNCH(twin_ln_pair_kernel<4>, dim3(grid), dim3(256), 0, s, y, rowvec, res, gamma, beta, t1, po, m, c, ldy, ldrv, rv_rows,
+              ldr, ldt, ldp, eps, a_scale, status);
+  else if (ch4 <= 64 * 8)
+    CS_LAUNCH(twin_ln_pair_kernel<8>, dim3(grid), dim3(256), 0, s, y, rowvec, res, gamma, beta, t1, po, m, c, ldy, ldrv, rv_rows,
+              ldr, ldt, ldp, eps, a_scale, status);
+  else
+    return CS_EINVAL;
+  CS_CHECK_LAUNCH();
+  return CS_OK;
+}
diff --git a/commonscenes_amd/csrc/cs_unet.hip b/commonscenes_amd/csrc/cs_unet.hip
--- a/commonscenes_amd/csrc/cs_unet.hip
+++ b/commonscenes_amd/csrc/cs_unet.hip
@@ -354,17 +354,18 @@
     return o;
   }
 
-  Act attn_block(const Layer& l, const Act& x, const float* ctxvec) {
+  Act attn_block(const Layer& l, const Act& x, const float* ctxvec, bool twin = false) {
     const int c = l.cin, heads = u.cfg.num_heads, dh = c / heads;
     const int n = x.d * x.h * x.w;
-    const int64_t rows = (int64_t)x.nb * n;
+    const int nbo = twin ? 2 * x.nb : x.nb;
+    const int64_t rows = (int64_t)nbo * n;
     Buf xn = groupnorm(x.b, l.n[0], x.nb, 1e-6f, CS_ACT_NONE);
     Buf t0 = linear(xn, l.g[0]);
     release(xn);
     Buf n1 = layernorm(t0, l.n[1]);
     Buf qkv = linear(n1, l.g[1]);
     release(n1);
-    Buf a = alloc(rows, c);
+    Buf a = alloc(t0.rows, c);
     float ss[12];
     const Norm& gnn = pl.norms[l.n[0]];
     const bool stat = l.has_ts && u.cfg.math == CS_MATH_F16X3 && !cs_debug()->no_static_scales && ctxvec &&
@@ -372,10 +373,28 @@
     self_attention(qkv, a, x.nb, n, heads, dh, c, (float)std::pow((double)dh, -0.5), stat ? ss : nullptr);
     if (stat) a.a_scale = ss[3];
     release(qkv);
-    Buf t1 = linear(a, l.g[2], GemmOpts().row_vector(ctxvec ? ctxvec + l.ctx_off : nullptr, u.ctx_total, n).residual(t0, c));
-    release(a);
-    release(t0);
-    Buf n3 = layernorm(t1, l.n[3]);
+    const float* rv = ctxvec ? ctxvec + l.ctx_off : nullptr;
+    Buf t1, n3;
+    if (twin) {
+      Buf y = linear(a, l.g[2]);
+      cs_conv_plan_copies(1);
+      release(a);
+      const Norm& nm = pl.norms[l.n[3]];
+      t1 = alloc(rows, c);
+      n3 = alloc(rows, c);
+      n3.pair = true;
+      n3.a_scale = norm_a_scale(nm.gmax, nm.bmax, c);
+      if (ok() && !dry)
+        chk(cs_twin_layernorm_pair16(p(y), rv, p(t0), wf(nm.g_off), wf(nm.b_off), p(t1), p(n3), (int)y.rows, c, c, u.ctx_total, n, c,
+                                     c, c, 1e-5f, n3.a_scale, status, st));
+      release(y);
+      release(t0);
+    } else {
+      t1 = linear(a, l.g[2], GemmOpts().row_vector(rv, u.ctx_total, n).residual(t0, c));
+      release(a);
+      release(t0);
+      n3 = layernorm(t1, l.n[3]);
+    }
     Buf gg;
     const float pairs = u.cfg.math == CS_MATH_F16X3 ? 16.f : 0.f;
     const float pair_gg = (pairs > 0.f && stat) ? ss[4] : pairs, pair_t2 = (pairs > 0.f && stat) ? ss[5] : pairs;
@@ -394,8 +413,16 @@
     release(gg);
     release(t1);
     Act o = x;
-    o.b = gemm(t2, l.g[7], x.nb, n, 1, 1, GemmOpts().residual(x.b, c).stats());
+    o.nb = nbo;
+    Buf x2;
+    if (twin) {
+      x2 = alloc(rows, c);
+      for (int g = 0; g < 2 && ok() && !dry; ++g)
+        chk(cs_copy_rows(p(x.b), p(x2) + (int64_t)g * x.b.rows * c, x.b.rows, c, c, c, st));
+    }
+    o.b = gemm(t2, l.g[7], nbo, n, 1, 1, GemmOpts().residual(twin ? x2 : x.b, c).stats());
     release(t2);
+    release(x2);
     return o;
   }
 
@@ -420,8 +447,9 @@
   }
 
   Act run(const std::vector<Layer>& layers, Act h, const Buf& semb, const float* ctxvec, bool keep_in,
-          const Act* split_skip = nullptr) {
+          const Act* split_skip = nullptr, bool twin = false) {
     bool owned = !keep_in;
+    if (twin) cs_conv_plan_copies(2);
     for (const Layer& l : layers) {
       Act o;
       if (l.kind == RES && l.ks > 0 && split_skip && &l == &layers[0]) {
@@ -440,7 +468,7 @@
           o = res_block(l, h, semb);
           break;
         case ATTN:
-          o = attn_block(l, h, ctxvec);
+          o = attn_block(l, h, ctxvec, twin && &l == &layers.back());
           break;
         case ATTNBLOCK:
           o = attnblock(l, h);
@@ -468,7 +496,16 @@
       h = o;
       owned = true;
     }
+    if (twin) cs_conv_plan_copies(1);
     return h;
+  }
+
+  bool late_split(const std::vector<Layer>& layers) const {
+    if (u.cfg.math != CS_MATH_F16X3 || cs_debug()->no_cfg_late_split || cs_debug()->no_pair16) return false;
+    if (layers.size() < 2 || layers.back().kind != ATTN || layers.back().cin % 16) return false;
+    for (size_t i = 0; i + 1 < layers.size(); ++i)
+      if (layers[i].kind != RES) return false;
+    return true;
   }
 
   Buf duplicate(const Buf& a) {
@@ -524,11 +561,21 @@
   bool first = true;
   for (const auto& layers : u.inp) {
     bool keep = !first;
+    bool twin = false;
     if (shared && has_attn(layers)) {
-      split(!first);
-      keep = false;
-    }
-    h = e.run(layers, h, semb, ctxvec, keep);
+      twin = e.late_split(layers);
+      if (!twin) {
+        split(!first);
+        keep = false;
+      }
+    }
+    h = e.run(layers, h, semb, ctxvec, keep, nullptr, twin);
+    if (twin) {
+      Buf s2 = e.duplicate(semb);
+      e.release(semb);
+      semb = s2;
+      shared = false;
+    }
     hs.push_back(h);
     first = false;
     if (!e.ok()) return e.rc;
diff --git a/commonscenes_amd/lib.py b/commonscenes_amd/lib.py
--- a/commonscenes_amd/lib.py
+++ b/commonscenes_amd/lib.py
@@ -65,7 +65,8 @@
         "plan_pow2", "slice_tile2", "no_gn_parts", "no_pair_epilogue", "no_dyn_scale", "no_tok_rules", "no_fused_reduce",
         "no_gn_fold", "no_kwave", "no_static_scales", "no_wino", "wino_min_rows", "no_wino43", "wino43_min_rows",
         "no_wino_tail")] + [
-        ("split16_min_rows", C.c_int64), ("cfg_split_min_rows", C.c_int64), ("gn_small_group", C.c_int64)]
+        ("split16_min_rows", C.c_int64), ("cfg_split_min_rows", C.c_int64), ("gn_small_group", C.c_int64),
+        ("no_cfg_late_split", C.c_int32)]
 
 
 class CsUnetConfig(C.Structure):
@@ -95,6 +96,7 @@
     "cs_conv_gemm_epilogue_caps": (_i, [C.POINTER(CsConvGemm), C.POINTER(C.c_int32), C.POINTER(C.c_int32)]),
     "cs_conv_wino_ok": (_i, [C.POINTER(CsConvGemm)]),
     "cs_conv_wino_plan": (_i, [C.POINTER(CsConvGemm), C.POINTER(C.c_int32), C.POINTER(C.c_int64)]),
+    "cs_conv_plan_copies": (_i, [_i]),
     "cs_conv_wino_plan_info": (_i, [C.POINTER(CsConvGemm), C.POINTER(C.c_int32), C.POINTER(C.c_int32), C.POINTER(C.c_int32)]),
     "cs_conv_wino_positions": (_i, [C.POINTER(CsConvGemm), _s]),
     "cs_conv_wino_output": (_i, [C.POINTER(CsConvGemm), _s]),
@@ -133,6 +135,7 @@
     "cs_groupnorm_apply_wino16_range": (_i, [_f, _f, _f, _f, _f, _f, _i, _i, _i, _i, _i, _i, _i, _i, _i, _i, _i, _fl, _f, _s]),
     "cs_groupnorm_apply_wino_range": (_i, [_f, _f, _f, _f, _f, _f, _i, _i, _i, _i, _i, _i, _i, _i, _i, _i, _i, _fl, _i, _f, _s]),
     "cs_layernorm_pair16": (_i, [_f, _f, _f, _f, _i, _i, _i, _i, _fl, _fl, _f, _s]),
+    "cs_twin_layernorm_pair16": (_i, [_f, _f, _f, _f, _f, _f, _f, _i, _i, _i, _i, _i, _i, _i, _i, _fl, _fl, _f, _s]),
     "cs_groupnorm_apply_range": (_i, [_f, _f, _f, _f, _f, _i, _i, _i, _i, _i, _i, _i, _i, _i, _s]),
     "cs_groupnorm_apply_split16_range": (_i, [_f, _f, _f, _f, _f, _f, _i, _i, _i, _i, _i, _i, _i, _i, _i, _fl, _f, _s]),
     "cs_groupnorm": (_i, [_f, _f, _f, _f, _i, _i, _i, _i, _i, _i, _fl, _i, _f, _f, _s]),
diff --git a/commonscenes_amd/ops.py b/commonscenes_amd/ops.py
--- a/commonscenes_amd/ops.py
+++ b/commonscenes_amd/ops.py
@@ -991,6 +991,42 @@
     return out
 
 
+def twin_layernorm(y: Tensor, rowvec: Tensor, rv_rows: int, res: Tensor, gamma: Tensor, beta: Tensor, pair_scale: float,
+                   eps: float = 1e-5) -> Tuple[Tensor, "Pair16"]:
+    _chk(y, "y")
+    _chk(res, "res")
+    _chk(rowvec, "rowvec")
+    m, c, ldy = rows_ld(y, "y")
+    rm, rc, ldr = rows_ld(res, "res")
+    vm, vc, ldrv = rows_ld(rowvec, "rowvec")
+    if (rm, rc) != (m, c) or vc != c or vm * rv_rows < 2 * m or c % 16:
+        raise L.CsError("twin_layernorm: shape mismatch")
+    shape = (2 * y.shape[0], *y.shape[1:])
+    t1 = torch.empty(shape, dtype=torch.float32, device=y.device)
+    pair = torch.empty(shape, dtype=torch.float32, device=y.device)
+    L.check(L.load().cs_twin_layernorm_pair16(y.data_ptr(), rowvec.data_ptr(), res.data_ptr(), gamma.data_ptr(), beta.data_ptr(),
+                                              t1.data_ptr(), pair.data_ptr(), m, c, ldy, ldrv, int(rv_rows), ldr, c, c, eps,
+                                              float(pair_scale), status_word(y.device).data_ptr(), _stream()),
+            "cs_twin_layernorm_pair16")
+    return t1, Pair16(pair, float(pair_scale))
+
+
+class plan_copies:
+
+    def __init__(self, copies: int):
+        self.copies = int(copies)
+
+    def __enter__(self):
+        self.prev = L.load().cs_conv_plan_copies(self.copies)
+        if self.prev < 1:
+            raise L.CsError("cs_conv_plan_copies failed: invalid argument")
+        return self
+
+    def __exit__(self, *exc):
+        L.load().cs_conv_plan_copies(self.prev)
+        return False
+
+
 def bound_a_scale(bound: float) -> float:
     return float(L.load().cs_bound_a_scale(float(bound)))
 
diff --git a/commonscenes_amd/unet.py b/commonscenes_amd/unet.py
--- a/commonscenes_amd/unet.py
+++ b/commonscenes_amd/unet.py
@@ -555,7 +555,13 @@
                          spatial=(nb, n, 1, 1), a_scale=ss[3] if ss is not None else None)
         return ops.attach_stats(out.view(nb, d, h, w, c), getattr(out, "cs_stats", None))
 
-    def _attn(self, p: str, l: dict, x: Tensor, ctx, out_fn=None) -> Tensor:
+    def _late_split(self, layers, ctx) -> bool:
+        return (self.math == L.MATH_F16X3 and not L.debug().no_cfg_late_split and ops._sw("PAIR16_PRODUCERS")
+                and isinstance(ctx, tuple) and self.cfg["use_spatial_transformer"] and len(layers) >= 2
+                and layers[-1]["kind"] == "attn" and layers[-1]["cin"] % 16 == 0
+                and all(l["kind"] == "res" for l in layers[:-1]))
+
+    def _attn(self, p: str, l: dict, x: Tensor, ctx, out_fn=None, twin: bool = False) -> Tensor:
         sd, pk = self._sd, self._packed
         heads = self.cfg["num_heads"]
         nb, d, h, w, c = x.shape
@@ -571,7 +577,14 @@
         amath = self.attn_math if self.attn_math is not None else self.math
         a = ops.attention(qkv[..., 0:c], qkv[..., c:2 * c], qkv[..., 2 * c:3 * c], heads, dh ** -0.5, math=amath,
                           scales=ss["attn"] if (ss is not None and amath == L.MATH_F16X3) else None)
-        if isinstance(ctx, tuple):
+        s3 = self._nas(t + ".norm3", c)
+        n3 = None
+        if twin:
+            y = ops.linear(a, pk[t + ".attn1.to_out.0"], math=self.math, a_scale=ss["a"] if ss is not None else None)
+            L.load().cs_conv_plan_copies(1)
+            t1, n3 = ops.twin_layernorm(y, ctx[1][t], n, t0, sd[t + ".norm3.weight"], sd[t + ".norm3.bias"], s3)
+            nb *= 2
+        elif isinstance(ctx, tuple):
             t1 = ops.linear(a, pk[t + ".attn1.to_out.0"], res=t0, rowvec=ctx[1][t], rv_rows=n, math=self.math,
                             a_scale=ss["a"] if ss is not None else None)
         else:
@@ -582,8 +595,8 @@
             vv2 = ops.linear(ctx, pk[t + ".attn2.to_v"], math=self.math)
             a2 = ops.attention(q2, k2, vv2, heads, dh ** -0.5, math=self.attn_math if self.attn_math is not None else self.math)
             t1 = ops.linear(a2, pk[t + ".attn2.to_out.0"], res=t1a, math=self.math)
-        s3 = self._nas(t + ".norm3", c)
-        n3 = ops.layernorm(t1, sd[t + ".norm3.weight"], sd[t + ".norm3.bias"], pair_scale=s3)
+        if n3 is None:
+            n3 = ops.layernorm(t1, sd[t + ".norm3.weight"], sd[t + ".norm3.bias"], pair_scale=s3)
         on = self.math == L.MATH_F16X3 and ops._sw("PAIR_EPILOGUES")
         pair_gg = (ss["gg"] if ss is not None else ops.A_SCALE) if on else None
         pair_t2 = (ss["t2"] if ss is not None else ops.A_SCALE) if on else None
@@ -595,11 +608,23 @@
         t2 = ops.linear(gg, pk[t + ".ff.net.2"], res=t1, math=self.math, out_pair=pair_t2,
                         a_scale=None if isinstance(gg, ops.Pair16) or ss is None else ss["gg"])
         dst = out_fn((nb, d, h, w, c)).view(nb, n, c) if out_fn is not None else None
-        out = ops.linear(t2, pk[p + ".proj_out"], res=x.view(nb, n, c), math=self.math, out=dst, stats=True,
+        xr = x.view(x.shape[0], n, c)
+        if twin:
+            xr = torch.empty((nb, n, c), dtype=torch.float32, device=x.device)
+            for g in range(2):
+                ops.copy_rows(x.view(nb // 2, n, c), xr[g * (nb // 2):(g + 1) * (nb // 2)])
+        out = ops.linear(t2, pk[p + ".proj_out"], res=xr, math=self.math, out=dst, stats=True,
                          spatial=(nb, n, 1, 1), a_scale=None if isinstance(t2, ops.Pair16) or ss is None else ss["t2"])
         return ops.attach_stats(out.view(nb, d, h, w, c), getattr(out, "cs_stats", None))
 
-    def _run(self, bp: str, layers, h: Tensor, semb: Tensor, ctx: Tensor, out_fn=None, split_skip=None) -> Tensor:
+    def _run(self, bp: str, layers, h: Tensor, semb: Tensor, ctx: Tensor, out_fn=None, split_skip=None,
+             twin: bool = False) -> Tensor:
+        if twin:
+            with ops.plan_copies(2):
+                return self._run_layers(bp, layers, h, semb, ctx, out_fn, split_skip, True)
+        return self._run_layers(bp, layers, h, semb, ctx, out_fn, split_skip, False)
+
+    def _run_layers(self, bp: str, layers, h: Tensor, semb: Tensor, ctx: Tensor, out_fn, split_skip, twin: bool) -> Tensor:
         pk = self._packed
         for li, l in enumerate(layers):
             p = f"{bp}.{l['idx']}"
@@ -613,8 +638,8 @@
                 else:
                     h = self._res(p, l, h, semb, of)
             elif k == "attn":
-                h = (self._attn(p, l, h, ctx, of) if self.cfg["use_spatial_transformer"]
-                     else self._attnblock(p, l, h, of))
+                h = (self._attn(p, l, h, ctx, of, twin=twin and li == len(layers) - 1)
+                     if self.cfg["use_spatial_transformer"] else self._attnblock(p, l, h, of))
             elif k == "down":
                 h = ops.conv_gemm(h, pk[p + ".op"], stride=(1, 2, 2) if self.cfg["dims"] == 3 else (2, 2, 2),
                                   math=self.math, out_fn=of, stats=True, x_bound=ops.range_bound(h, self._slot()))
@@ -662,14 +687,20 @@
 
         shared = cfg_pairs
         for i, layers in enumerate(inp):
+            twin = False
             if shared and any(l["kind"] == "attn" for l in layers):
-                st = getattr(h, "cs_stats", None)
-                h = torch.cat([h, h], dim=0)
-                ops.attach_stats(h, st)
-                semb = torch.cat([semb, semb], dim=0)
+                twin = self._late_split(layers, ctx)
+                if not twin:
+                    st = getattr(h, "cs_stats", None)
+                    h = torch.cat([h, h], dim=0)
+                    ops.attach_stats(h, st)
+                    semb = torch.cat([semb, semb], dim=0)
                 shared = False
             direct = nocopy and not shared
-            h = self._run(f"{P}input_blocks.{i}", layers, h, semb, ctx, slot(nout - 1 - i, False) if direct else None)
+            h = self._run(f"{P}input_blocks.{i}", layers, h, semb, ctx, slot(nout - 1 - i, False) if direct else None,
+                          twin=twin)
+            if twin:
+                semb = torch.cat([semb, semb], dim=0)
             hs.append(None if direct else h)
             seg_r[nout - 1 - i] = getattr(h, "cs_stats", None)
             if tr is not None:
diff --git a/commonscenes_amd/unet_native.py b/commonscenes_amd/unet_native.py
--- a/commonscenes_amd/unet_native.py
+++ b/commonscenes_amd/unet_native.py
@@ -130,7 +130,7 @@
         return n
 
     def _workspace(self, nb_x: int, cfg_pairs: bool) -> Tensor:
-        key = (nb_x, cfg_pairs)
+        key = (nb_x, cfg_pairs, int(L.debug().no_cfg_late_split))
         if self._ws_key != key:
             need = int(L.load().cs_unet_workspace_bytes(self._h, nb_x, 1 if cfg_pairs else 0))
             if need < 0:
diff --git a/include/commonscenes_hip.h b/include/commonscenes_hip.h
--- a/include/commonscenes_hip.h
+++ b/include/commonscenes_hip.h
@@ -59,6 +59,7 @@
   int64_t split16_min_rows;
   int64_t cfg_split_min_rows;
   int64_t gn_small_group;
+  int32_t no_cfg_late_split;
 } CsDebug;
 const CsDebug* cs_debug(void);
 void cs_debug_set(const CsDebug* d);
@@ -133,6 +134,7 @@
 int cs_conv_gemm_plan(const CsConvGemm* desc, int32_t* splitk, int64_t* splitk_ws_bytes);
 int cs_conv_wino_ok(const CsConvGemm* desc);
 int cs_conv_wino_plan(const CsConvGemm* desc, int32_t* splitk, int64_t* ws_bytes);
+int cs_conv_plan_copies(int copies);
 int cs_conv_wino_plan_info(const CsConvGemm* desc, int32_t* slices, int32_t* units_main, int32_t* units);
 int cs_conv_wino_positions(const CsConvGemm* desc, cs_stream_t stream);
 int cs_conv_wino_output(const CsConvGemm* desc, cs_stream_t stream);
@@ -220,6 +222,10 @@
 int cs_layernorm_pair16(const float* x, const float* gamma, const float* beta, void* y, int m, int c, int ldx, int ldy,
                         float eps, float a_scale, int32_t* status, cs_stream_t stream);
 
+int cs_twin_layernorm_pair16(const float* y, const float* rowvec, const float* res, const float* gamma, const float* beta,
+                             float* t1, void* pair, int m, int c, int ldy, int ldrv, int rv_rows, int ldr, int ldt, int ldp,
+                             float eps, float a_scale, int32_t* status, cs_stream_t stream);
+
 int cs_attn_selfattn(const float* q, const float* k, const float* v, float* out, int nb, int nq,
                      int nk, int heads, int dh, int ldq, int ldk, int ldv, int ldo, float scale,
                      cs_stream_t stream);
```

Measured after the change: 16.08, median of 6. 1.7% higher.
